# atlas-jj/ORB-SLAM-free-space-carving

Hardware: AMD Instinct MI355X
Metric: Mpix*KF/s fused (640x480xN_KF) (higher is better)
Workload: dtype f32

## Files before the change

include/sdm_c.h:

```cpp
#ifndef SDM_C_H
#define SDM_C_H

#include <stddef.h>
#include <stdint.h>

#ifdef __cplusplus
extern "C" {
#endif

#define SDM_OK 0
#define SDM_EINVAL 1
#define SDM_EHIP 2
#define SDM_ENODEV 3
#define SDM_ESTATE 4
#define SDM_ECOMM 5

#define SDM_MAX_NEIGHBOURS 64
#define SDM_MAX_OBSERVATIONS 8192

typedef struct sdm_ctx sdm_ctx;

typedef struct {
    float lambdaG;
    float lambdaL;
// ... 26 lines not shown
    long long table_stagings;
} sdm_stats;

void sdm_default_params(sdm_params *p);
void sdm_default_config(sdm_config *c);
size_t sdm_depth_pool_bytes(int W, int H, int max_keyframes);
int sdm_create(sdm_ctx **out, const sdm_config *cfg);
void sdm_destroy(sdm_ctx *ctx);
const char *sdm_last_error(void);
int sdm_set_params(sdm_ctx *ctx, const sdm_params *p);
int sdm_get_params(sdm_ctx *ctx, sdm_params *out);
int sdm_set_stream(sdm_ctx *ctx, void *hip_stream);
int sdm_synchronize(sdm_ctx *ctx);
int sdm_device_count(void);

int sdm_upload_keyframe(sdm_ctx *ctx, int slot, const uint8_t *im, const float *grad,
                        const float *theta, float I_stddev, const float K[4], const float Tcw[12]);
int sdm_upload_image(sdm_ctx *ctx, int slot, const uint8_t *im, const float K[4],
                     const float Tcw[12]);
#define SDM_ORDER_RGB 0
#define SDM_ORDER_BGR 1
#define SDM_ORDER_RGBA 2
#define SDM_ORDER_BGRA 3
#define SDM_ORDER_GRAY 4
int sdm_upload_image_rgb(sdm_ctx *ctx, int slot, const uint8_t *pixels, int order, const float K[4],
                         const float dist[5], const float Tcw[12]);
int sdm_upload_images_batch(sdm_ctx *ctx, int n, const int *slots, const uint8_t *const *images,
                            const float *K, const float *Tcw);
int sdm_upload_images_rgb_batch(sdm_ctx *ctx, int n, const int *slots, const uint8_t *const *pixels,
                                int order, const float *K, const float dist[5], const float *Tcw);
void *sdm_host_alloc(size_t bytes);
void sdm_host_free(void *p);
int sdm_upload_image_device(sdm_ctx *ctx, int slot, const void *d_im, const float K[4],
                            const float Tcw[12]);
int sdm_set_pose(sdm_ctx *ctx, int slot, const float Tcw[12]);
int sdm_download_inputs(sdm_ctx *ctx, int slot, uint8_t *im, float *grad, float *theta,
                        float *I_stddev);

int sdm_search_fuse(sdm_ctx *ctx, int n_ref, const int *ref_slots, int n, const int *nbr_slots,
                    const float *rot_deg, const float *min_depth,
                    const float *max_depth);
int sdm_intra_check(sdm_ctx *ctx, int n_ref, const int *ref_slots);
int sdm_intra_grow(sdm_ctx *ctx, int n_ref, const int *ref_slots);
int sdm_recon(sdm_ctx *ctx, int n_ref, const int *ref_slots, int n, const int *nbr_slots,
              const float *rot_deg, const float *min_depth, const float *max_depth);

int sdm_upload_observations(sdm_ctx *ctx, int slot, int n_kp, const int *map_point_ids, const float *angles,
                            int n_depths, const float *depths);
int sdm_upload_observations_batch(sdm_ctx *ctx, int n, const int *slots, const int *n_kp,
                                  const int *const *map_point_ids, const float *const *angles, const int *n_depths,
                                  const float *const *depths);
int sdm_search_priors(sdm_ctx *ctx, int n_ref, const int *ref_slots, int n, const int *nbr_slots, float *rot_deg,
                      float *min_depth, float *max_depth);
int sdm_recon_observed(sdm_ctx *ctx, int n_ref, const int *ref_slots, int n, const int *nbr_slots);

#define SDM_COVIS_MIN_WEIGHT 15

int sdm_covisibility(sdm_ctx *ctx, int n_ref, const int *ref_slots, int n_cand, const int *cand_slots, int *weights);

int sdm_covisible_neighbours(sdm_ctx *ctx, int n_ref, const int *ref_slots, int n_cand, const int *cand_slots,
                             int n, int min_weight, int *nbr_slots, int *nbr_weights, int *counts);

int sdm_recon_covisible(sdm_ctx *ctx, int n_ref, const int *ref_slots, int n_cand, const int *cand_slots,
                        int n, int min_weight, int *nbr_slots_out, unsigned char *done);

int sdm_inter_check(sdm_ctx *ctx, int n_ref, const int *ref_slots, int n, const int *nbr_slots,
                    int commit);


int sdm_pointset(sdm_ctx *ctx, int n_ref, const int *ref_slots, int source);
int sdm_inter_check_pointset(sdm_ctx *ctx, int n_ref, const int *ref_slots, int n, const int *nbr_slots,
                             int commit);

int sdm_upload_depth(sdm_ctx *ctx, int slot, const float *rho, const float *sigma);
int sdm_download_depth(sdm_ctx *ctx, int slot, float *rho, float *sigma);
int sdm_download_checked(sdm_ctx *ctx, int slot, float *rho);
int sdm_download_pointset(sdm_ctx *ctx, int slot, float *xyz);
typedef struct {
    float *xyz;
    unsigned *pixel;
    float *rho_sigma;
    uint8_t *intensity;
    long long capacity;
    int on_device;
} sdm_point_buffers;

int sdm_extract_points(sdm_ctx *ctx, int n, const int *slots, int source, double max_sigma, double min_rho,
                       sdm_point_buffers *out, long long *offsets);
int sdm_extract_points_support(sdm_ctx *ctx, int n, const int *slots, int n_nbr, const int *nbr_slots ,
                               int source, double max_sigma, double min_rho, sdm_point_buffers *out,
                               unsigned long long *support , long long *offsets);
typedef struct {
    unsigned *multiplicity;
    unsigned *source_index;
    unsigned *representative;
    long long rep_capacity;
    long long plain_total;
} sdm_voxel_buffers;
int sdm_extract_points_voxel(sdm_ctx *ctx, int n, const int *slots, int source, double max_sigma, double min_rho,
                             float voxel_size, sdm_point_buffers *out, sdm_voxel_buffers *vox ,
                             long long *offsets);
int sdm_extract_bound(sdm_ctx *ctx, int n, const int *slots, int source, double min_rho, long long *bound);
void *sdm_depth_pool_ptr(sdm_ctx *ctx);
int sdm_assume_pipeline_maps(sdm_ctx *ctx, int n, const int *slots);

int sdm_mark_depth_present(sdm_ctx *ctx, int n, const int *slots);

#define SDM_COMM_ID_BYTES 128
int sdm_comm_unique_id(unsigned char id[SDM_COMM_ID_BYTES]);
int sdm_comm_init(sdm_ctx *ctx, const unsigned char id[SDM_COMM_ID_BYTES], int world, int rank);
int sdm_comm_attach(sdm_ctx *ctx, void *nccl_comm);
int sdm_comm_destroy(sdm_ctx *ctx);
int sdm_comm_info(sdm_ctx *ctx, int *world, int *rank);
int sdm_exchange_halo_begin(sdm_ctx *ctx, int n_send, const int *send_peer, const int *send_slot,
                            int n_recv, const int *recv_peer, const int *recv_slot);
int sdm_exchange_wait(sdm_ctx *ctx);
int sdm_exchange_halo(sdm_ctx *ctx, int n_send, const int *send_peer, const int *send_slot,
                      int n_recv, const int *recv_peer, const int *recv_slot);
int sdm_allgather_depth(sdm_ctx *ctx, int first_slot, int count, int n_fetch, const int *fetch_index,
                        const int *dst_slot);
int sdm_allgather_begin(sdm_ctx *ctx, int maps_per_rank);
int sdm_allgather_piece(sdm_ctx *ctx, int count, const int *slots);
int sdm_allgather_finish(sdm_ctx *ctx, int n_fetch, const int *fetch_index, const int *dst_slot);
int sdm_exchange_compact(sdm_ctx *ctx, int entries_per_map);
int sdm_exchange_mismatches(sdm_ctx *ctx, int *count);
int sdm_compact_pack_host(sdm_ctx *ctx, int slot, float *out);
int sdm_compact_unpack_host(sdm_ctx *ctx, int slot, const float *in, int *refused);
int sdm_compact_sources_ready(sdm_ctx *ctx, int n, const int *slots, int *ready);
int sdm_active_count(sdm_ctx *ctx, int slot, int *count);
int sdm_download_active_list(sdm_ctx *ctx, int slot, unsigned *list, int capacity, int *count,
                             unsigned long long *hash);
int sdm_comm_all_ok(sdm_ctx *ctx, int local_ok, int *all_ok);
int sdm_comm_all_max(sdm_ctx *ctx, int local_value, int *all_max);

int sdm_intra_check_maps(sdm_ctx *ctx, float *rho, float *sigma, const float *grad);
int sdm_intra_grow_maps(sdm_ctx *ctx, float *rho, float *sigma, const float *grad);

int sdm_epipolar_search(sdm_ctx *ctx, int ref_slot, int nbr_slot, int x, int y, float min_depth,
                        float max_depth, float rot_deg, float out[5]);
int sdm_search_range(sdm_ctx *ctx, int ref_slot, int nbr_slot, int x, int y, float mind,
                     float maxd, float *umin, float *umax);
int sdm_fuse(sdm_ctx *ctx, const float *rho, const float *sigma, int n, float out[3]);
int sdm_pair_geometry(sdm_ctx *ctx, int ref_slot, int nbr_slot, float F12[9], float R21[9],
                      float t21[3]);

int sdm_stereo_search_constraints(const float *orb_depths, int n, float *min_depth,
                                  float *max_depth);
float sdm_median_rot_in_plane(const int *mp1, const float *angle1, int n1, const int *mp2,
                              const float *angle2, int n2);

int sdm_enable_stats(sdm_ctx *ctx, int on);
int sdm_get_stats(sdm_ctx *ctx, sdm_stats *out, int reset);
int sdm_set_scan_mode(sdm_ctx *ctx, int mode);
int sdm_set_ingest_overlap(sdm_ctx *ctx, int on);
#define SDM_STAGE_SEARCH_FUSE 0
#define SDM_STAGE_INTRA 1
#define SDM_STAGE_INTER 2
#define SDM_STAGE_POINTSET 3
#define SDM_NUM_STAGES 4
int sdm_enable_timing(sdm_ctx *ctx, int on);
int sdm_get_timing(sdm_ctx *ctx, double ms_total[SDM_NUM_STAGES], long long launches[SDM_NUM_STAGES],
                   int reset);
int sdm_selftest(sdm_ctx *ctx, int which, unsigned long long out[2]);
const char *sdm_device_arch(sdm_ctx *ctx);

#ifdef __cplusplus
}
#endif
#endif
```

orb-slam-free-space-carving_amd/binding.py:

```python
import ctypes as C
import os

import numpy as np

_HERE = os.path.dirname(os.path.abspath(__file__))
MAX_NEIGHBOURS = 64
MAX_OBSERVATIONS = 8192


class SdmError(RuntimeError):
    def __init__(self, code, msg):
        super().__init__("sdm error %d: %s" % (code, msg))
        self.code = code


class Params(C.Structure):
    _fields_ = [("lambdaG", C.c_float), ("lambdaL", C.c_float), ("lambdaTheta", C.c_float),
                ("lambdaN", C.c_int), ("theta_var", C.c_double)]


class Config(C.Structure):
    _fields_ = [("device", C.c_int), ("W", C.c_int), ("H", C.c_int), ("max_keyframes", C.c_int),
                ("max_neighbours", C.c_int), ("batch_capacity", C.c_int), ("with_pointset", C.c_int),
                ("ext_depth_pool", C.c_void_p), ("stream", C.c_void_p)]


class Stats(C.Structure):
    _fields_ = [("searches", C.c_longlong), ("candidates", C.c_longlong), ("gate_pass", C.c_longlong),
                ("hypotheses", C.c_longlong), ("fused", C.c_longlong), ("mask_waves", C.c_longlong),
                ("mask_steps", C.c_longlong), ("mask_row_mismatch", C.c_longlong), ("open_pixels", C.c_longlong),
                ("table_stagings", C.c_longlong)]


class PointBuffers(C.Structure):
    _fields_ = [("xyz", C.c_void_p), ("pixel", C.c_void_p), ("rho_sigma", C.c_void_p), ("intensity", C.c_void_p),
                ("capacity", C.c_longlong), ("on_device", C.c_int)]


class VoxelBuffers(C.Structure):
    _fields_ = [("multiplicity", C.c_void_p), ("source_index", C.c_void_p), ("representative", C.c_void_p),
                ("rep_capacity", C.c_longlong), ("plain_total", C.c_longlong)]


POINT_FIELDS = {"xyz": (np.float32, 3), "pixel": (np.uint32, 1), "rho_sigma": (np.float32, 2), "intensity": (np.uint8, 1)}


def lib_path():
    return os.environ.get("SDM_LIB_PATH") or os.path.join(_HERE, "lib", "libsdm_hip.so")


_lib = None

_f32p, _u8p, _ip = C.POINTER(C.c_float), C.POINTER(C.c_uint8), C.POINTER(C.c_int)
_ctx = C.c_void_p
SYMBOLS = [
    ("sdm_default_params", None, [C.POINTER(Params)]),
    ("sdm_default_config", None, [C.POINTER(Config)]),
    ("sdm_depth_pool_bytes", C.c_size_t, [C.c_int, C.c_int, C.c_int]),
    ("sdm_create", C.c_int, [C.POINTER(_ctx), C.POINTER(Config)]),
    ("sdm_destroy", None, [_ctx]),
    ("sdm_last_error", C.c_char_p, []),
    ("sdm_set_params", C.c_int, [_ctx, C.POINTER(Params)]),
    ("sdm_set_stream", C.c_int, [_ctx, C.c_void_p]),
    ("sdm_synchronize", C.c_int, [_ctx]),
    ("sdm_device_count", C.c_int, []),
    ("sdm_upload_keyframe", C.c_int, [_ctx, C.c_int, _u8p, _f32p, _f32p, C.c_float, _f32p, _f32p]),
    ("sdm_upload_image", C.c_int, [_ctx, C.c_int, _u8p, _f32p, _f32p]),
    ("sdm_upload_image_rgb", C.c_int, [_ctx, C.c_int, _u8p, C.c_int, _f32p, _f32p, _f32p]),
    ("sdm_upload_image_device", C.c_int, [_ctx, C.c_int, C.c_void_p, _f32p, _f32p]),
    ("sdm_upload_images_batch", C.c_int, [_ctx, C.c_int, _ip, C.POINTER(C.c_void_p), _f32p, _f32p]),
    ("sdm_upload_images_rgb_batch", C.c_int, [_ctx, C.c_int, _ip, C.POINTER(C.c_void_p), C.c_int, _f32p, _f32p, _f32p]),
    ("sdm_host_alloc", C.c_void_p, [C.c_size_t]),
    ("sdm_host_free", None, [C.c_void_p]),
    ("sdm_set_pose", C.c_int, [_ctx, C.c_int, _f32p]),
    ("sdm_download_inputs", C.c_int, [_ctx, C.c_int, _u8p, _f32p, _f32p, _f32p]),
    ("sdm_search_fuse", C.c_int, [_ctx, C.c_int, _ip, C.c_int, _ip, _f32p, _f32p, _f32p]),
    ("sdm_intra_check", C.c_int, [_ctx, C.c_int, _ip]),
    ("sdm_intra_grow", C.c_int, [_ctx, C.c_int, _ip]),
    ("sdm_recon", C.c_int, [_ctx, C.c_int, _ip, C.c_int, _ip, _f32p, _f32p, _f32p]),
    ("sdm_upload_observations", C.c_int, [_ctx, C.c_int, C.c_int, _ip, _f32p, C.c_int, _f32p]),
    ("sdm_upload_observations_batch", C.c_int, [_ctx, C.c_int, _ip, _ip, C.POINTER(C.c_void_p), C.POINTER(C.c_void_p), _ip,
                                                C.POINTER(C.c_void_p)]),
    ("sdm_search_priors", C.c_int, [_ctx, C.c_int, _ip, C.c_int, _ip, _f32p, _f32p, _f32p]),
    ("sdm_recon_observed", C.c_int, [_ctx, C.c_int, _ip, C.c_int, _ip]),
    ("sdm_covisibility", C.c_int, [_ctx, C.c_int, _ip, C.c_int, _ip, _ip]),
    ("sdm_covisible_neighbours", C.c_int, [_ctx, C.c_int, _ip, C.c_int, _ip, C.c_int, C.c_int, _ip, _ip, _ip]),
    ("sdm_recon_covisible", C.c_int, [_ctx, C.c_int, _ip, C.c_int, _ip, C.c_int, C.c_int, _ip, _u8p]),
    ("sdm_inter_check", C.c_int, [_ctx, C.c_int, _ip, C.c_int, _ip, C.c_int]),
    ("sdm_pointset", C.c_int, [_ctx, C.c_int, _ip, C.c_int]),
    ("sdm_inter_check_pointset", C.c_int, [_ctx, C.c_int, _ip, C.c_int, _ip, C.c_int]),
    ("sdm_upload_depth", C.c_int, [_ctx, C.c_int, _f32p, _f32p]),
    ("sdm_download_depth", C.c_int, [_ctx, C.c_int, _f32p, _f32p]),
    ("sdm_download_checked", C.c_int, [_ctx, C.c_int, _f32p]),
    ("sdm_download_pointset", C.c_int, [_ctx, C.c_int, _f32p]),
    ("sdm_extract_points", C.c_int, [_ctx, C.c_int, _ip, C.c_int, C.c_double, C.c_double, C.POINTER(PointBuffers),
                                     C.POINTER(C.c_longlong)]),
    ("sdm_extract_points_support", C.c_int, [_ctx, C.c_int, _ip, C.c_int, _ip, C.c_int, C.c_double, C.c_double,
                                             C.POINTER(PointBuffers), C.POINTER(C.c_ulonglong), C.POINTER(C.c_longlong)]),
    ("sdm_extract_points_voxel", C.c_int, [_ctx, C.c_int, _ip, C.c_int, C.c_double, C.c_double, C.c_float,
                                           C.POINTER(PointBuffers), C.POINTER(VoxelBuffers), C.POINTER(C.c_longlong)]),
    ("sdm_extract_bound", C.c_int, [_ctx, C.c_int, _ip, C.c_int, C.c_double, C.POINTER(C.c_longlong)]),
    ("sdm_depth_pool_ptr", C.c_void_p, [_ctx]),
    ("sdm_assume_pipeline_maps", C.c_int, [_ctx, C.c_int, _ip]),
    ("sdm_mark_depth_present", C.c_int, [_ctx, C.c_int, _ip]),
    ("sdm_comm_unique_id", C.c_int, [C.POINTER(C.c_ubyte)]),
    ("sdm_comm_init", C.c_int, [_ctx, C.POINTER(C.c_ubyte), C.c_int, C.c_int]),
    ("sdm_comm_attach", C.c_int, [_ctx, C.c_void_p]),
    ("sdm_comm_destroy", C.c_int, [_ctx]),
    ("sdm_comm_info", C.c_int, [_ctx, _ip, _ip]),
    ("sdm_exchange_halo_begin", C.c_int, [_ctx, C.c_int, _ip, _ip, C.c_int, _ip, _ip]),
    ("sdm_exchange_wait", C.c_int, [_ctx]),
    ("sdm_exchange_halo", C.c_int, [_ctx, C.c_int, _ip, _ip, C.c_int, _ip, _ip]),
    ("sdm_allgather_depth", C.c_int, [_ctx, C.c_int, C.c_int, C.c_int, _ip, _ip]),
    ("sdm_allgather_begin", C.c_int, [_ctx, C.c_int]),
    ("sdm_allgather_piece", C.c_int, [_ctx, C.c_int, _ip]),
    ("sdm_allgather_finish", C.c_int, [_ctx, C.c_int, _ip, _ip]),
    ("sdm_comm_all_ok", C.c_int, [_ctx, C.c_int, _ip]),
    ("sdm_comm_all_max", C.c_int, [_ctx, C.c_int, _ip]),
    ("sdm_exchange_compact", C.c_int, [_ctx, C.c_int]),
    ("sdm_exchange_mismatches", C.c_int, [_ctx, _ip]),
    ("sdm_compact_sources_ready", C.c_int, [_ctx, C.c_int, _ip, _ip]),
    ("sdm_compact_pack_host", C.c_int, [_ctx, C.c_int, _f32p]),
    ("sdm_compact_unpack_host", C.c_int, [_ctx, C.c_int, _f32p, _ip]),
    ("sdm_active_count", C.c_int, [_ctx, C.c_int, _ip]),
    ("sdm_download_active_list", C.c_int, [_ctx, C.c_int, C.POINTER(C.c_uint), C.c_int, _ip, C.POINTER(C.c_ulonglong)]),
    ("sdm_intra_check_maps", C.c_int, [_ctx, _f32p, _f32p, _f32p]),
    ("sdm_intra_grow_maps", C.c_int, [_ctx, _f32p, _f32p, _f32p]),
    ("sdm_epipolar_search", C.c_int, [_ctx, C.c_int, C.c_int, C.c_int, C.c_int, C.c_float, C.c_float,
                                      C.c_float, _f32p]),
    ("sdm_search_range", C.c_int, [_ctx, C.c_int, C.c_int, C.c_int, C.c_int, C.c_float, C.c_float,
                                   _f32p, _f32p]),
    ("sdm_fuse", C.c_int, [_ctx, _f32p, _f32p, C.c_int, _f32p]),
    ("sdm_pair_geometry", C.c_int, [_ctx, C.c_int, C.c_int, _f32p, _f32p, _f32p]),
    ("sdm_stereo_search_constraints", C.c_int, [_f32p, C.c_int, _f32p, _f32p]),
    ("sdm_median_rot_in_plane", C.c_float, [_ip, _f32p, C.c_int, _ip, _f32p, C.c_int]),
    ("sdm_enable_stats", C.c_int, [_ctx, C.c_int]),
    ("sdm_get_stats", C.c_int, [_ctx, C.POINTER(Stats), C.c_int]),
    ("sdm_set_scan_mode", C.c_int, [_ctx, C.c_int]),
    ("sdm_get_params", C.c_int, [_ctx, C.POINTER(Params)]),
    ("sdm_set_ingest_overlap", C.c_int, [_ctx, C.c_int]),
    ("sdm_selftest", C.c_int, [_ctx, C.c_int, C.POINTER(C.c_ulonglong)]),
    ("sdm_enable_timing", C.c_int, [_ctx, C.c_int]),
    ("sdm_get_timing", C.c_int, [_ctx, C.POINTER(C.c_double), C.POINTER(C.c_longlong), C.c_int]),
    ("sdm_device_arch", C.c_char_p, [_ctx]),
]


def load_library():
    global _lib
    if _lib is not None:
        return _lib
    p = lib_path()
    if not os.path.exists(p):
        raise OSError("%s not built: run `python orb-slam-free-space-carving_amd/build.py` "
                      "(there is no CPU fallback)" % p)
    lib = C.CDLL(p)
    for name, res, args in SYMBOLS:
        fn = getattr(lib, name)
        fn.restype = res
        fn.argtypes = args
    _lib = lib
    return lib


def _f32(a):
    a = np.ascontiguousarray(a, dtype=np.float32)
    return a, a.ctypes.data_as(_f32p)


def _i32(a):
    a = np.ascontiguousarray(a, dtype=np.int32)
    return a, a.ctypes.data_as(_ip)


def stereo_search_constraints(depths):
    lib = load_library()
    d, dp = _f32(depths)
    mn, mx = C.c_float(), C.c_float()
    rc = lib.sdm_stereo_search_constraints(dp, len(d), C.byref(mn), C.byref(mx))
    if rc:
        raise SdmError(rc, lib.sdm_last_error().decode())
    return float(mn.value), float(mx.value)


def median_rot_in_plane(mp1, ang1, mp2, ang2):
    lib = load_library()
    m1, m1p = _i32(mp1)
    m2, m2p = _i32(mp2)
    a1, a1p = _f32(ang1)
    a2, a2p = _f32(ang2)
    return float(lib.sdm_median_rot_in_plane(m1p, a1p, len(m1), m2p, a2p, len(m2)))


class Engine:

    def __init__(self, W, H, max_keyframes, max_neighbours=7, device=0, batch_capacity=0,
                 with_pointset=True, ext_depth_pool=None, stream=None):
        self.lib = load_library()
        cfg = Config()
        self.lib.sdm_default_config(C.byref(cfg))
        cfg.device, cfg.W, cfg.H = device, W, H
        cfg.max_keyframes, cfg.max_neighbours = max_keyframes, max_neighbours
        cfg.batch_capacity = batch_capacity
        cfg.with_pointset = 1 if with_pointset else 0
        cfg.ext_depth_pool = ext_depth_pool
        cfg.stream = stream
        self.W, self.H, self.max_keyframes, self.max_neighbours = W, H, max_keyframes, max_neighbours
        self.device = device
        self.ctx = _ctx()
        self._check(self.lib.sdm_create(C.byref(self.ctx), C.byref(cfg)))

    def _check(self, rc):
        if rc:
            raise SdmError(rc, self.lib.sdm_last_error().decode())

    def close(self):
        if getattr(self, "ctx", None):
            self.lib.sdm_destroy(self.ctx)
            self.ctx = None

    def __del__(self):
        try:
            self.close()
        except Exception:
            pass

    def arch(self):
        return self.lib.sdm_device_arch(self.ctx).decode()

    def set_params(self, **kw):
        p = Params()
        self.lib.sdm_default_params(C.byref(p))
        for k, v in kw.items():
            setattr(p, k, v)
        self._check(self.lib.sdm_set_params(self.ctx, C.byref(p)))

    def get_params(self):
        p = Params()
        self._check(self.lib.sdm_get_params(self.ctx, C.byref(p)))
        return {k: getattr(p, k) for k, _ in Params._fields_}

    def set_stream(self, stream_ptr):
        self._check(self.lib.sdm_set_stream(self.ctx, stream_ptr))

    def synchronize(self):
        self._check(self.lib.sdm_synchronize(self.ctx))

    def depth_pool_ptr(self):
        return self.lib.sdm_depth_pool_ptr(self.ctx)

    def upload_keyframe(self, slot, im, grad, theta, I_stddev, K, Tcw):
        im = np.ascontiguousarray(im, dtype=np.uint8)
        assert im.shape == (self.H, self.W)
        g, gp = _f32(grad)
        t, tp = _f32(theta)
        k, kp = _f32(K)
        T, Tp = _f32(np.asarray(Tcw).reshape(12))
        self._check(self.lib.sdm_upload_keyframe(self.ctx, slot, im.ctypes.data_as(_u8p), gp, tp,
                                                 float(I_stddev), kp, Tp))

    def upload_image(self, slot, im, K, Tcw):
        im = np.ascontiguousarray(im, dtype=np.uint8)
        assert im.shape == (self.H, self.W)
        k, kp = _f32(K)
        T, Tp = _f32(np.asarray(Tcw).reshape(12))
        self._check(self.lib.sdm_upload_image(self.ctx, slot, im.ctypes.data_as(_u8p), kp, Tp))

    ORDER = dict(rgb=0, bgr=1, rgba=2, bgra=3, gray=4)
    compact_entries = 0

    def upload_image_rgb(self, slot, pixels, order, K, dist, Tcw):
        px = np.ascontiguousarray(pixels, dtype=np.uint8)
        ch = {0: 3, 1: 3, 2: 4, 3: 4, 4: 1}[self.ORDER[order]]
        assert px.size == self.H * self.W * ch, (px.shape, ch)
        k, kp = _f32(K)
        T, Tp = _f32(np.asarray(Tcw).reshape(12))
        dp = None
        if dist is not None:
            d, dp = _f32(dist)
            assert len(d) == 5
        self._check(self.lib.sdm_upload_image_rgb(self.ctx, slot, px.ctypes.data_as(_u8p), self.ORDER[order], kp, dp, Tp))

    def _upload_args(self, slots, images, K, Tcw, nbytes):
        n = len(slots)
        assert len(images) == n
        ims = [np.ascontiguousarray(im, dtype=np.uint8) for im in images]
        for im in ims:
            assert im.size == nbytes, (im.shape, nbytes)
        ptrs = (C.c_void_p * n)(*[im.ctypes.data for im in ims])
        sl = (C.c_int * n)(*[int(x) for x in slots])
        k = np.ascontiguousarray(np.broadcast_to(np.asarray(K, np.float32).reshape(-1, 4), (n, 4)), dtype=np.float32)
# ... 363 lines not shown
    def comm_init(self, uid, world, rank):
        buf = (C.c_ubyte * self.COMM_ID_BYTES).from_buffer_copy(uid) if uid is not None else None
        self._check(self.lib.sdm_comm_init(self.ctx, buf, world, rank))

    def comm_destroy(self):
        self.compact_entries = 0
        self._check(self.lib.sdm_comm_destroy(self.ctx))

    def comm_info(self):
        w, r = C.c_int(), C.c_int()
        self._check(self.lib.sdm_comm_info(self.ctx, C.byref(w), C.byref(r)))
        return int(w.value), int(r.value)

    def _xchg_args(self, send, recv):
        sp, ss = _i32([p for p, _ in send]), _i32([s for _, s in send])
        rp, rs = _i32([p for p, _ in recv]), _i32([s for _, s in recv])
        return (len(send), sp[1], ss[1], len(recv), rp[1], rs[1]), (sp, ss, rp, rs)

    def exchange_halo_begin(self, send, recv):
        args, keep = self._xchg_args(send, recv)
        self._check(self.lib.sdm_exchange_halo_begin(self.ctx, *args))

    def exchange_wait(self):
        self._check(self.lib.sdm_exchange_wait(self.ctx))

    def exchange_halo(self, send, recv):
        args, keep = self._xchg_args(send, recv)
        self._check(self.lib.sdm_exchange_halo(self.ctx, *args))

    def allgather_depth(self, first_slot, count, fetch=None):
        if fetch is None:
            self._check(self.lib.sdm_allgather_depth(self.ctx, first_slot, count, -1, None, None))
            return
        fi, fip = _i32([i for i, _ in fetch])
        ds, dsp = _i32([s for _, s in fetch])
        self._check(self.lib.sdm_allgather_depth(self.ctx, first_slot, count, len(fetch), fip, dsp))

    def allgather_begin(self, maps_per_rank):
        self._check(self.lib.sdm_allgather_begin(self.ctx, maps_per_rank))

    def allgather_piece(self, slots):
        s, sp = _i32(np.asarray(slots).reshape(-1))
        self._check(self.lib.sdm_allgather_piece(self.ctx, len(s), sp))

    def allgather_finish(self, fetch):
        fi, fip = _i32([i for i, _ in fetch])
        ds, dsp = _i32([s for _, s in fetch])
        self._check(self.lib.sdm_allgather_finish(self.ctx, len(fetch), fip, dsp))

    def comm_all_max(self, value):
        out = C.c_int()
        self._check(self.lib.sdm_comm_all_max(self.ctx, int(value), C.byref(out)))
        return int(out.value)

    def exchange_compact(self, entries_per_map):
        self._check(self.lib.sdm_exchange_compact(self.ctx, int(entries_per_map)))
        self.compact_entries = int(entries_per_map)

    COMPACT_HEADER = 8

    def compact_pack_host(self, slot):
        out = np.empty((self.compact_entries + self.COMPACT_HEADER, 2), np.float32)
        self._check(self.lib.sdm_compact_pack_host(self.ctx, int(slot), out.ctypes.data_as(_f32p)))
        return out

    def compact_unpack_host(self, slot, payload):
        p = np.ascontiguousarray(payload, np.float32)
        assert p.size == 2 * (self.compact_entries + self.COMPACT_HEADER)
        ref = C.c_int()
        self._check(self.lib.sdm_compact_unpack_host(self.ctx, int(slot), p.ctypes.data_as(_f32p), C.byref(ref)))
        return bool(ref.value)

    def exchange_mismatches(self):
        out = C.c_int()
        self._check(self.lib.sdm_exchange_mismatches(self.ctx, C.byref(out)))
        return int(out.value)

    def compact_sources_ready(self, slots):
        arr = (C.c_int * max(len(slots), 1))(*[int(x) for x in slots])
        out = C.c_int()
        self._check(self.lib.sdm_compact_sources_ready(self.ctx, len(slots), arr, C.byref(out)))
        return bool(out.value)

    def active_count(self, slot):
        out = C.c_int()
        self._check(self.lib.sdm_active_count(self.ctx, int(slot), C.byref(out)))
        return int(out.value)

    def active_list(self, slot):
        n = self.active_count(slot)
        lst = np.empty(max(n, 1), np.uint32)
        cnt, h = C.c_int(), C.c_ulonglong()
        self._check(self.lib.sdm_download_active_list(self.ctx, int(slot), lst.ctypes.data_as(C.POINTER(C.c_uint)), int(lst.size),
                                                      C.byref(cnt), C.byref(h)))
        return lst[:cnt.value].copy(), int(h.value)

    def comm_all_ok(self, local_ok=True):
        out = C.c_int()
        self._check(self.lib.sdm_comm_all_ok(self.ctx, 1 if local_ok else 0, C.byref(out)))
        return bool(out.value)

    def assume_pipeline_maps(self, slots):
        r, rp = _i32(np.asarray(slots).reshape(-1))
        self._check(self.lib.sdm_assume_pipeline_maps(self.ctx, len(r), rp))

    def intra_check_maps(self, rho, sigma, grad=None):
        r = np.array(rho, dtype=np.float32, order="C")
        s = np.array(sigma, dtype=np.float32, order="C")
        gp = None
        if grad is not None:
            g, gp = _f32(grad)
        self._check(self.lib.sdm_intra_check_maps(self.ctx, r.ctypes.data_as(_f32p), s.ctypes.data_as(_f32p), gp))
        return r, s

    def intra_grow_maps(self, rho, sigma, grad):
        r = np.array(rho, dtype=np.float32, order="C")
        s = np.array(sigma, dtype=np.float32, order="C")
        g, gp = _f32(grad)
        self._check(self.lib.sdm_intra_grow_maps(self.ctx, r.ctypes.data_as(_f32p), s.ctypes.data_as(_f32p), gp))
        return r, s

    def epipolar_search(self, ref, nbr, x, y, min_depth, max_depth, rot=0.0):
        out = (C.c_float * 5)()
        self._check(self.lib.sdm_epipolar_search(self.ctx, ref, nbr, x, y, min_depth, max_depth, rot, out))
        return dict(rho=float(out[0]), sigma=float(out[1]), supported=int(out[2]), best_u=float(out[3]),
                    best_v=float(out[4]))

    def search_range(self, ref, nbr, x, y, mind, maxd):
        a, b = C.c_float(), C.c_float()
        self._check(self.lib.sdm_search_range(self.ctx, ref, nbr, x, y, mind, maxd, C.byref(a), C.byref(b)))
        return float(a.value), float(b.value)

    def fuse(self, rho, sigma):
        r, rp = _f32(rho)
        s, sp = _f32(sigma)
        out = (C.c_float * 3)()
        self._check(self.lib.sdm_fuse(self.ctx, rp, sp, len(r), out))
        return float(out[0]), float(out[1]), int(out[2])

    def pair_geometry(self, ref, nbr):
        F = np.empty(9, np.float32)
        R = np.empty(9, np.float32)
        t = np.empty(3, np.float32)
        self._check(self.lib.sdm_pair_geometry(self.ctx, ref, nbr, F.ctypes.data_as(_f32p),
                                               R.ctypes.data_as(_f32p), t.ctypes.data_as(_f32p)))
        return F, R, t

    def set_ingest_overlap(self, on=True):
        self._check(self.lib.sdm_set_ingest_overlap(self.ctx, 1 if on else 0))

    def set_scan_mode(self, mode):
        self._check(self.lib.sdm_set_scan_mode(self.ctx, int(mode)))

    def enable_stats(self, on=True):
        self._check(self.lib.sdm_enable_stats(self.ctx, 1 if on else 0))

    def selftest(self, which):
        out = (C.c_ulonglong * 2)()
        self._check(self.lib.sdm_selftest(self.ctx, which, out))
        return int(out[0]), int(out[1])

    STAGES = ("search_fuse", "intra", "inter", "pointset")

    def enable_timing(self, on=True):
        self._check(self.lib.sdm_enable_timing(self.ctx, 1 if on else 0))

    def get_timing(self, reset=True):
        ms = (C.c_double * 4)()
        cnt = (C.c_longlong * 4)()
        self._check(self.lib.sdm_get_timing(self.ctx, ms, cnt, 1 if reset else 0))
        return {s: (float(ms[i]), int(cnt[i])) for i, s in enumerate(self.STAGES)}

    def get_stats(self, reset=True):
        s = Stats()
        self._check(self.lib.sdm_get_stats(self.ctx, C.byref(s), 1 if reset else 0))
        return {k: int(getattr(s, k)) for k, _ in Stats._fields_}
```

orb-slam-free-space-carving_amd/csrc/sdm_device.h:

```cpp
#pragma once
#include <hip/hip_runtime.h>
#include <float.h>
#include <stddef.h>
#include <stdint.h>

#include "sdm_c.h"

namespace sdm {

struct KfMeta {
    float fx, fy, cx, cy;
    float Tcw[12];
    float I_stddev;
    int uploaded;
    int pad[2];
};

struct RefConst {
    int slot;
    float fx, fy, cx, cy;
    float mind, maxd;
    int act_count;
};

// ... 277 lines not shown
__device__ __forceinline__ float fast_atan2_deg_x1(float y)
{
    const float scale = (float)(180.0 / 3.14159265358979323846);
    const float p1 = 0.9997878412794807f * scale;
    const float p3 = -0.3258083974640975f * scale;
    const float p5 = 0.1555786518463281f * scale;
    const float p7 = -0.04432655554792128f * scale;
    float ay = fabsf(y);
    float a, c, c2;
    if (1.0f >= ay) {
        c = ay;
        c2 = c * c;
        a = (((p7 * c2 + p5) * c2 + p3) * c2 + p1) * c;
    } else {
#if SDM_K1_OPT_ATAN_RCP
        c = rcp_exact(ay + (float)DBL_EPSILON);
#else
        c = 1.0f / (ay + (float)DBL_EPSILON);
#endif
        c2 = c * c;
        a = 90.f - (((p7 * c2 + p5) * c2 + p3) * c2 + p1) * c;
    }
    if (y < 0) a = 360.f - a;
    return a;
}

#ifndef SDM_K1_OPT
#define SDM_K1_OPT 0x3a27f
#endif

constexpr int PCV_FLOATS = 20;
constexpr int CV_RX = 9, CV_RZ = 12, CV_TX = 15, CV_TZ = 16, CV_ROT = 17, CV_ISTD = 18;
static_assert(offsetof(PairConst, Rx) == 4 * CV_RX && offsetof(PairConst, Rz) == 4 * CV_RZ && offsetof(PairConst, tx) == 4 * CV_TX &&
                  offsetof(PairConst, tz) == 4 * CV_TZ && offsetof(PairConst, rot) == 4 * CV_ROT &&
                  offsetof(PairConst, istd) == 4 * CV_ISTD && offsetof(PairConst, Ry) == 4 * PCV_FLOATS,
              "the CV_* indices follow PairConst");

__device__ __forceinline__ float match_cost1(float pe2, float ge2, const DevParams& prm)
{
    double s = (double)pe2 + (double)ge2 * prm.inv_theta;
    const unsigned lo = (unsigned)__double2loint(s), hi = (unsigned)__double2hiint(s);
    const bool risky = (((lo & 0x1FFFFFFFu) - 0x0FFFFF00u) <= 0x200u) | ((hi - 0x39C00000u) >= (0x46200000u - 0x39C00000u));
    if (__builtin_expect(risky, 0)) s = (double)pe2 + (double)ge2 / prm.theta_var;
    return (float)s;
}

constexpr float INV_THETA_DEFAULT_F = (float)(1.0 / 0.23);
constexpr unsigned COST_BAND = 16u;
__device__ __forceinline__ float match_cost_ref(float pe2, float ge2, const DevParams& prm)
{
    return (float)((double)pe2 + (double)ge2 / prm.theta_var);
}
__device__ __forceinline__ float match_cost_approx(float pe2, float ge2) { return __builtin_fmaf(ge2, INV_THETA_DEFAULT_F, pe2); }

__device__ __forceinline__ float lerp_w0(float yf)
{
#if SDM_K1_OPT & 0x10
    return 1.0f - __builtin_amdgcn_fractf(yf);
#else
    return (floorf(yf) + 1.0f) - yf;
#endif
}
__device__ __forceinline__ float rec_lerp_im_w(const float4& r, float y0w)
{
    unsigned w = __float_as_uint(r.w);
    float y1w = 1.0f - y0w;
    float v0 = (float)(int)(w & 0xffu), v1 = (float)(int)((w >> 8) & 0xffu);
    return v0 * y0w + v1 * y1w;
}
__device__ __forceinline__ float rec_lerp_grad_w(const float4& r, float y0w)
{
    float y1w = 1.0f - y0w;
    return r.x * y0w + r.z * y1w;
}

__device__ __forceinline__ int cvt_i32_sat(float x)
{
    int r;
    asm("v_cvt_i32_f32 %0, %1" : "=v"(r) : "v"(x));
    return r;
}
__device__ __forceinline__ bool search_range_int1(float fx, float cx, float rxxp, float rzxp, float tx, float tz,
                                                  float mind, float maxd, int W, int& lo, int& hi)
{
    float x_min = rxxp * mind + tx, z_min = rzxp * mind + tz;
    float x_max = rxxp * maxd + tx, z_max = rzxp * maxd + tz;
    const float u1 = fx * x_min / z_min + cx;
    const float u2 = fx * x_max / z_max + cx;
    const float mn = __builtin_amdgcn_fmed3f(u1, u2, -__builtin_inff());
    const float mx = __builtin_amdgcn_fmed3f(u1, u2, __builtin_inff());
    lo = min(max(cvt_i32_sat(ceilf(mn)), 0), W);
    hi = min(max(cvt_i32_sat(floorf(mx)), 0), W - 1);
    return !__builtin_isunordered(u1, u2);
}

__device__ __forceinline__ float wrap_once_360_ref(float a)
{
    if (a >= 360) a -= 360;
    if (a < 0) a += 360;
    return a;
}
__device__ __forceinline__ float wrap_once_360(float a)
{
#if SDM_K1_OPT & 0x40
    a = a + 0.0f;
    const unsigned bits = __float_as_uint(a);
    const unsigned lt360 = (unsigned)((int)(bits - 0x43B40000u) >> 31);
    const unsigned neg = (unsigned)((int)bits >> 31);
    unsigned keep = lt360 | neg;
    asm("" : "+v"(keep));
    a = a + __uint_as_float(~keep & 0xC3B40000u);
    return wrap_neg360(a);
#else
    return wrap_once_360_ref(a);
#endif
}

constexpr unsigned QUOT_MAG_LO = 87u << 23;
constexpr unsigned QUOT_MAG_HI = (168u << 23) - 1u;
__device__ __forceinline__ unsigned absbits(float x) { return __float_as_uint(x) & 0x7FFFFFFFu; }
__device__ __forceinline__ float rcp_fast(float b)
{
    const float r = __builtin_amdgcn_rcpf(b);
    const float e = __builtin_fmaf(-b, r, 1.0f);
    return __builtin_fmaf(e, r, r);
}
__device__ __forceinline__ float quot_fast(float a, float b, float r)
{
    float q0 = a * r;
    float e0 = __builtin_fmaf(-q0, b, a);
    float q1 = __builtin_fmaf(e0, r, q0);
    float e1 = __builtin_fmaf(-q1, b, a);
    return __builtin_fmaf(e1, r, q1);
}
__device__ __forceinline__ bool quot_window_ok(float a, float b)
{
    const unsigned ua = absbits(a), ub = absbits(b);
    return (ua >= QUOT_MAG_LO) & (ua <= QUOT_MAG_HI) & (ub >= QUOT_MAG_LO) & (ub <= QUOT_MAG_HI);
}

__device__ __forceinline__ float sqrt_exact(float x)
{
#if SDM_K1_OPT & 0x10000
    if (__builtin_expect((__float_as_uint(x) - (27u << 23)) >= ((254u - 27u) << 23), 0)) return sqrtf(x);
    const float r = __builtin_amdgcn_rsqf(x);
    const float y0 = x * r, h = 0.5f * r;
    const float e = __builtin_fmaf(-y0, y0, x);
    return __builtin_fmaf(e, h, y0);
#else
    return sqrtf(x);
#endif
}

__device__ __forceinline__ bool line_quot_safe(const float* F)
{
    bool ok = true;
    for (int i = 0; i < 9; i++) {
        const unsigned u = __float_as_uint(F[i]), mag = u & 0x7FFFFFFFu;
        ok = ok && (u == 0u || (mag >= ((127u - 36u) << 23) && mag <= ((127u + 20u) << 23)));
    }
    return ok;
}

struct ScanState {
    float old_err, best_pe, best_ge;
    int best_pixel;
};

struct ScanConst {
    const char* nbase;
    unsigned W16;
    float hlim_b;
    float ab, cb, pixel, grad1, th_line, ang_pi_rot, gate_lim;
    int hi;
};
template <bool STATS, bool CLEAN>
__device__ __forceinline__ void scan_candidate(const ScanConst& q, int uj, float yf, const float4& r, const DevParams& prm,
                                               ScanState& S, SearchStats* st)
{
    if (r.x < prm.lambdaG) return;
#if SDM_ABLATE == 4
    if (r.z > S.old_err) { S.best_pixel = uj; S.old_err = r.z; }
    return;
#endif
    const float d2 = r.y - q.th_line;
    const float d3 = r.y - q.ang_pi_rot;
    bool fail;
    if (CLEAN) {
#if SDM_K1_OPT & 0x04
        fail = gate2_fails_fast1(d2) | gate3_fails_fast1(d3);
#else
        fail = gate2_fails_fast(d2) | gate3_fails_fast(d3);
#endif
    } else {
        fail = gate2_fails_k(d2, prm.g2c) | gate3_fails_k(d3, prm.g3lo, prm.g3span);
        if (__builtin_expect(!((d2 < q.gate_lim) & (d3 < q.gate_lim)), 0))
            fail = gate2_fails_ref(d2, prm.lambdaL) || gate3_fails_ref(d3, prm.lambdaTheta);
    }
    if (fail) return;
    if (STATS) st->gate_pass++;
#if SDM_ABLATE == 3 || SDM_ABLATE == 4
    if (r.z > S.old_err) { S.best_pixel = uj; S.old_err = r.z; }
    return;
#endif
    const float y0w = lerp_w0(yf);
    float pe = q.pixel - rec_lerp_im_w(r, y0w);
    float ge = q.grad1 - rec_lerp_grad_w(r, y0w);
#if SDM_K1_OPT & 0x2000
    if (CLEAN || prm.approx_ok) {
        const float e = CLEAN ? match_cost_approx(pe * pe, ge * ge) : __builtin_fmaf(ge * ge, prm.inv_theta_f, pe * pe);
        bool better = e < S.old_err;
        if (__builtin_expect((__float_as_uint(e) - __float_as_uint(S.old_err) + COST_BAND) <= 2u * COST_BAND, 0))
            better = match_cost_ref(pe * pe, ge * ge, prm) < match_cost_ref(S.best_pe * S.best_pe, S.best_ge * S.best_ge, prm);
        if (better) {
#if SDM_K1_OPT & 0x4000
            asm volatile("" ::: "memory");
#endif
            S.best_pixel = uj;
            S.old_err = e;
            S.best_pe = pe;
            S.best_ge = ge;
        }
        return;
    }
#endif
#if SDM_K1_OPT & 0x08
    float err = match_cost1(pe * pe, ge * ge, prm);
#else
    float err = match_cost(pe * pe, ge * ge, prm);
#endif
    if (err < S.old_err) {
        S.best_pixel = uj;
        S.old_err = err;
        S.best_pe = pe;
        S.best_ge = ge;
    }
}

template <bool STATS, bool CLEAN, int NB>
__device__ __forceinline__ void scan_batch(const ScanConst& q, int u0, float u0f, const DevParams& prm, ScanState& S,
                                           SearchStats* st)
{
    float yfs[NB];
    unsigned long long rowok[NB];
    v4f rs[NB];
    const unsigned c0 = (unsigned)u0 << 4;
#if !(SDM_K1_OPT & 0x01)
    const unsigned hi16 = (unsigned)max(q.hi, 0) << 4;
#endif
#pragma unroll
    for (int k = 0; k < NB; k++) {
        float yf = -(q.ab * (u0f + (float)k) + q.cb);
        float yc = __builtin_amdgcn_fmed3f(yf, 1.0f, q.hlim_b);
#if SDM_K1_OPT & 0x01
        const unsigned off = __umul24((unsigned)(int)yc, q.W16) + c0;
        const char* __restrict__ nb_k = q.nbase + 16 * k;
#else
        unsigned uc16 = min(c0 + 16u * k, hi16);
        unsigned off = __umul24((unsigned)(int)yc, q.W16) + uc16;
        const char* __restrict__ nb_k = q.nbase;
#endif
        yfs[k] = yf;
        rowok[k] = __builtin_amdgcn_fcmpf(yc, yf, 1 );
#if SDM_ABLATE == 5
        rs[k] = v4f{20.0f + (float)(off & 15u), 10.0f, 21.0f, __uint_as_float(0x6040u)};
#else
        rs[k] = *reinterpret_cast<const v4f*>(nb_k + off);
#endif
    }
#pragma unroll
    for (int k = 0; k < NB; k++)
        asm volatile("" : "+v"(rs[k]));
#pragma unroll
    for (int k = 0; k < NB; k++) {
        const int uj = u0 + k;
        if (STATS && uj <= q.hi) st->candidates++;
        const float4 r = make_float4(rs[k].x, rs[k].y, rs[k].z, rs[k].w);
        if (!((uj <= q.hi) & __builtin_amdgcn_inverse_ballot_w64(rowok[k]))) continue;
        scan_candidate<STATS, CLEAN>(q, uj, yfs[k], r, prm, S, st);
    }
}

template <bool STATS, bool CLEAN>
__device__ __forceinline__ void scan_segment(const ScanConst& q, int lo, const DevParams& prm, ScanState& S, SearchStats* st)
{
    float u0f = (float)lo;
    for (int u0 = lo; u0 <= q.hi; u0 += SCAN_UNROLL, u0f += (float)SCAN_UNROLL)
        scan_batch<STATS, CLEAN, SCAN_UNROLL>(q, u0, u0f, prm, S, st);
}

#ifndef SDM_MASK_MIN_L
#define SDM_MASK_MIN_L 24
#endif
#ifndef SDM_MASK_MIN_L_UNION
#define SDM_MASK_MIN_L_UNION 48
#endif
#ifndef SDM_MASK_MAX_SLOPE
#define SDM_MASK_MAX_SLOPE 0.25f
#endif
#ifndef SDM_MASK_NB
#define SDM_MASK_NB 2
#endif
#ifndef SDM_MASK_BINS
#define SDM_MASK_BINS 1
#endif
constexpr int MASK_BINS = 16;
constexpr int MASK_WINDOW = 6;
constexpr int MASK_UNION = MASK_BINS + MASK_WINDOW - 1;
constexpr int MASK_PLANES = MASK_UNION + 1;
constexpr unsigned MASK_WORD_BYTES = 4u * MASK_PLANES;
constexpr float MASK_EPS = 0x1p-6f;
constexpr int MASK_HINT_L = SDM_MASK_MIN_L * 3 / 4;
#ifndef SDM_MASK_CALL_MEAN_L
#define SDM_MASK_CALL_MEAN_L 32
#endif
constexpr int MASK_CALL_MEAN_L = SDM_MASK_CALL_MEAN_L;
constexpr float MASK_ANG_MARGIN = 0.01f;
constexpr float MASK_MAX_LAMBDA_THETA = 56.0f;
constexpr float MASK_BIN_SCALE = (float)MASK_BINS / 360.0f;
__host__ __device__ __forceinline__ int mask_bin(float t)
{
    const int b = (int)(t * MASK_BIN_SCALE);
    return b < MASK_BINS - 1 ? b : MASK_BINS - 1;
}
struct MaskStats {
    unsigned long long waves, steps, row_mismatch;
};
struct MaskView {
    const char* base;
    unsigned row_pitch;
};
template <bool STATS, bool CLEAN, bool BINNED>
__device__ __forceinline__ void scan_masked(const ScanConst& q, const MaskView& mv, int lo, const DevParams& prm, ScanState& S,
                                            SearchStats* st, MaskStats* ms)
{
    const float yh = -(q.ab * (float)q.hi + q.cb);
    const float inv_s = __builtin_amdgcn_rcpf(fabsf(q.ab)) * 0.998046875f;
    const bool falling = q.ab > 0.0f;
    unsigned pl0 = 4u * (unsigned)MASK_UNION;
    if (BINNED) {
        float w0 = q.ang_pi_rot - (prm.lambdaTheta + MASK_ANG_MARGIN);
        if (w0 < 0.0f) w0 += 360.0f;
        pl0 = 4u * (unsigned)mask_bin(w0);
    }
    for (int base = lo; base <= q.hi; base += 64) {
        const int chi = min(q.hi, base + 63);
        unsigned long long cand = 0ull;
        bool ended = false;
        int u = base;
        while (u <= chi) {
            const float yf = -(q.ab * (float)u + q.cb);
            const float yc = __builtin_amdgcn_fmed3f(yf, 1.0f, q.hlim_b);
            if (!(yc == yf)) {
                const bool out_lo = (yf < 1.0f) & (yh < 1.0f), out_hi = (yf > q.hlim_b) & (yh > q.hlim_b);
                if (!(yf == yf) | out_lo | out_hi) {
                    if (STATS) st->candidates += (unsigned long long)(q.hi - u + 1);
                    ended = true;
                    break;
                }
                if (STATS) st->candidates++;
                u++;
                continue;
            }
            const float fr = __builtin_amdgcn_fractf(yf);
            const float room = (falling ? fr : 1.0f - fr) - MASK_EPS;
            const int n = max(cvt_i32_sat(room * inv_s), 0);
            const int cover = min(min(n, chi - u), 32);
            const char* __restrict__ mp = mv.base + (__umul24((unsigned)(int)yc, mv.row_pitch) + __umul24((unsigned)u >> 5, MASK_WORD_BYTES) + pl0);
            unsigned mlo, mhi;
            if (BINNED) {
                typedef unsigned mword4 __attribute__((ext_vector_type(4), aligned(4)));
                typedef unsigned mword2 __attribute__((ext_vector_type(2), aligned(4)));
                const mword4 a0 = *reinterpret_cast<const mword4*>(mp);
                const mword2 a1 = *reinterpret_cast<const mword2*>(mp + 16);
                const mword4 b0 = *reinterpret_cast<const mword4*>(mp + MASK_WORD_BYTES);
                const mword2 b1 = *reinterpret_cast<const mword2*>(mp + MASK_WORD_BYTES + 16);
                mlo = (a0.x | a0.y | a0.z) | (a0.w | a1.x | a1.y);
                mhi = (b0.x | b0.y | b0.z) | (b0.w | b1.x | b1.y);
            } else {
                mlo = *reinterpret_cast<const unsigned*>(mp);
                mhi = *reinterpret_cast<const unsigned*>(mp + MASK_WORD_BYTES);
            }
            unsigned long long bits = (((unsigned long long)mhi << 32) | (unsigned long long)mlo) >> ((unsigned)u & 31u);
            bits &= (2ull << cover) - 1ull;
            cand |= bits << (unsigned)(u - base);
            if (STATS) {
                st->candidates += (unsigned long long)(cover + 1);
                ms->steps++;
            }
            u += cover + 1;
        }
        if (STATS) {
            for (int k = 0; base + k <= (ended ? u - 1 : chi); k++) {
                const float yk = -(q.ab * (float)(base + k) + q.cb);
                if (!(__builtin_amdgcn_fmed3f(yk, 1.0f, q.hlim_b) == yk)) continue;
                const v4f r = *reinterpret_cast<const v4f*>(q.nbase + (__umul24((unsigned)(int)yk, q.W16) + ((unsigned)(base + k) << 4)));
                if (r.x < prm.lambdaG) continue;
                const bool fail = gate2_fails_ref(r.y - q.th_line, prm.lambdaL) || gate3_fails_ref(r.y - q.ang_pi_rot, prm.lambdaTheta);
                if (!fail && !((cand >> k) & 1ull)) ms->row_mismatch++;
            }
        }
        while (cand != 0ull) {
            int ujs[SDM_MASK_NB];
            float yfs[SDM_MASK_NB];
            v4f rs[SDM_MASK_NB];
            unsigned long long okm[SDM_MASK_NB];
#pragma unroll
            for (int k = 0; k < SDM_MASK_NB; k++) {
                okm[k] = __builtin_amdgcn_ballot_w64(cand != 0ull);
                const int uj = base + (cand != 0ull ? (int)__builtin_ctzll(cand) : 0);
                cand &= cand - 1ull;
                const float yfj = -(q.ab * (float)uj + q.cb);
                const float ycj = __builtin_amdgcn_fmed3f(yfj, 1.0f, q.hlim_b);
                ujs[k] = uj;
                yfs[k] = yfj;
                rs[k] = *reinterpret_cast<const v4f*>(q.nbase + (__umul24((unsigned)(int)ycj, q.W16) + ((unsigned)uj << 4)));
            }
#pragma unroll
            for (int k = 0; k < SDM_MASK_NB; k++)
                asm volatile("" : "+v"(rs[k]));
#pragma unroll
            for (int k = 0; k < SDM_MASK_NB; k++) {
                if (!__builtin_amdgcn_inverse_ballot_w64(okm[k])) continue;
                scan_candidate<STATS, CLEAN>(q, ujs[k], yfs[k], make_float4(rs[k].x, rs[k].y, rs[k].z, rs[k].w), prm, S, st);
            }
        }
        if (ended) break;
    }
}

__device__ __forceinline__ int wave_max_nonneg(int v)
{
    v = max(v, __builtin_amdgcn_update_dpp(0, v, 0x111, 0xf, 0xf, false));
    v = max(v, __builtin_amdgcn_update_dpp(0, v, 0x112, 0xf, 0xf, false));
    v = max(v, __builtin_amdgcn_update_dpp(0, v, 0x114, 0xf, 0xf, false));
    v = max(v, __builtin_amdgcn_update_dpp(0, v, 0x118, 0xf, 0xf, false));
    v = max(v, __builtin_amdgcn_update_dpp(0, v, 0x142, 0xa, 0xf, false));
    v = max(v, __builtin_amdgcn_update_dpp(0, v, 0x143, 0xc, 0xf, false));
    return __builtin_amdgcn_readlane(v, 63);
}
template <bool STATS, bool CLEAN>
__device__ __forceinline__ void scan_planned(const ScanConst& q, int lo, int Lmax, const DevParams& prm, ScanState& S,
                                             SearchStats* st)
{
    int n3 = (-Lmax) & 3;
    if (Lmax <= 3) n3 = 1;
    if (Lmax == 5) n3 = 2;
    const int n4 = max(Lmax - 3 * n3, 0) >> 2;
    int u0 = lo;
    float u0f = (float)lo;
    for (int i = 0; i < n4; i++, u0 += 4, u0f += 4.0f)
        if (u0 <= q.hi) scan_batch<STATS, CLEAN, 4>(q, u0, u0f, prm, S, st);
    for (int i = 0; i < n3; i++, u0 += 3, u0f += 3.0f)
        if (u0 <= q.hi) scan_batch<STATS, CLEAN, 3>(q, u0, u0f, prm, S, st);
}

template <bool STATS, bool PLAN = false, bool MASK = false>
__device__ __forceinline__ bool epipolar_search(const float4* __restrict__ nrec, int W, int H,
                                                const float* __restrict__ cv, const float* __restrict__ rcv, int clean,
                                                bool on, int x, int y, float pixel, float grad1,
                                                float th_pi, float xp0, float xp1, const DevParams& prm, float& rho_o,
                                                float& sigma_o, float& best_u, float& best_v,
                                                SearchStats* st, const MaskView mv = MaskView{nullptr, 0u}, MaskStats* ms = nullptr)
{
    float fx = rcv[0], cx = rcv[1];
    const float mind = rcv[2], maxd = rcv[3];
    rho_o = 0.f;
    sigma_o = 0.f;
    best_u = 0.f;
    best_v = 0.f;
    if (STATS && on) st->searches++;
    const float* F = cv;
    float a = (float)x * F[0] + (float)y * F[3] + F[6];
    float b = (float)x * F[1] + (float)y * F[4] + F[7];
    float c = (float)x * F[2] + (float)y * F[5] + F[8];
#if SDM_K1_OPT & 0x8000
    float ab, cb;
    if (clean & 2) {
        const float rb = rcp_fast(b);
        ab = quot_fast(a, b, rb);
        cb = quot_fast(c, b, rb);
    } else {
        ab = a / b;
        cb = c / b;
    }
    bool live = on & (ab >= -4) & (ab <= 4);
    if (!PLAN && !live) return false;
#else
    float ab = a / b;
    bool live = on & (ab >= -4) & (ab <= 4);
    if (!PLAN && !live) return false;
    float cb = c / b;
#endif

    float rxxp = row_dot_xp(cv + CV_RX, xp0, xp1);
    float rzxp = row_dot_xp(cv + CV_RZ, xp0, xp1);
    float tx = cv[CV_TX], tz = cv[CV_TZ];
    int lo, hi;
#if SDM_K1_OPT & 0x20
    live &= search_range_int1(fx, cx, rxxp, rzxp, tx, tz, mind, maxd, W, lo, hi);
#else
    live &= search_range_int(fx, cx, rxxp, rzxp, tx, tz, mind, maxd, W, lo, hi);
    if (hi > W - 1) hi = W - 1;
#endif
    if (!PLAN && !live) return false;

    float th_line = fast_atan2_deg_x1(-ab);
    float ang_pi_rot = wrap_once_360(th_pi + cv[CV_ROT]);

    const float gate_lim = prm.closed_ok ? 360.0f : -__builtin_inff();
    ScanState S = {1000000.0f, 1000.0f, 0.f, -1};
    const float hlim2 = (float)(H - 2);
    const char* __restrict__ nbase = reinterpret_cast<const char*>(nrec);
#if SDM_ABLATE == 10
    if (ang_pi_rot + th_line + (float)(hi - lo) != 12345.678f) live = false;
#endif
#if SDM_ABLATE == 11
    if (ab + cb + rxxp + rzxp != 12345.678f) live = false;
#endif
#if SDM_ABLATE == 6
    hi = lo - 1;
    S.old_err = ab;
    S.best_pixel = lo + 2;
#endif
    if (PLAN && !live) hi = lo - 1;
    ScanConst sc;
    sc.nbase = nbase;
    sc.W16 = (unsigned)W << 4;
    sc.hlim_b = __uint_as_float(__float_as_uint((float)(H - 1)) - 1u);
    sc.ab = ab;
    sc.cb = cb;
    sc.pixel = pixel;
    sc.grad1 = grad1;
    sc.th_line = th_line;
    sc.ang_pi_rot = ang_pi_rot;
    sc.gate_lim = gate_lim;
    sc.hi = hi;
    if (PLAN) {
        const int Lmax = wave_max_nonneg(max(hi - lo + 1, 0));
        if (Lmax > 0) {
#if SDM_K1_OPT & 0x02
            if ((clean & 1) && prm.default_gates && prm.fast_theta_div)
                scan_planned<STATS, true>(sc, lo, Lmax, prm, S, st);
            else
#endif
                scan_planned<STATS, false>(sc, lo, Lmax, prm, S, st);
        }
        if (!live) return false;
    } else {
        bool masked = false;
        const unsigned long long here = __builtin_amdgcn_ballot_w64(true);
#ifndef SDM_MASK_DISABLE
        if (MASK && mv.base != nullptr && prm.scan_mode != 1 && ((clean & 4) || prm.scan_mode == 2)) {
            const bool binned = (clean & 1) && prm.bins_ok && SDM_MASK_BINS;
            const int min_l = binned ? SDM_MASK_MIN_L : SDM_MASK_MIN_L_UNION;
            const unsigned long long lng = __builtin_amdgcn_ballot_w64(hi - lo + 1 >= min_l);
            const unsigned long long steep = __builtin_amdgcn_ballot_w64(fabsf(ab) > SDM_MASK_MAX_SLOPE);
            masked = prm.scan_mode == 2 || (2 * __popcll(lng) >= __popcll(here) && steep == 0ull);
        }
#endif
        if (MASK && masked) {
            if (STATS && (int)__builtin_amdgcn_mbcnt_hi(~0u, __builtin_amdgcn_mbcnt_lo(~0u, 0u)) == (int)__builtin_ctzll(here)) ms->waves++;
#if SDM_K1_OPT & 0x02
            if ((clean & 1) && prm.default_gates && prm.fast_theta_div)
                scan_masked<STATS, true, SDM_MASK_BINS != 0>(sc, mv, lo, prm, S, st, ms);
            else
#endif
                if ((clean & 1) && prm.bins_ok && SDM_MASK_BINS)
                scan_masked<STATS, false, true>(sc, mv, lo, prm, S, st, ms);
            else
                scan_masked<STATS, false, false>(sc, mv, lo, prm, S, st, ms);
        } else {
#if SDM_K1_OPT & 0x02
            if ((clean & 1) && prm.default_gates && prm.fast_theta_div)
                scan_segment<STATS, true>(sc, lo, prm, S, st);
            else
#endif
                scan_segment<STATS, false>(sc, lo, prm, S, st);
        }
    }
    const float best_pe = S.best_pe, best_ge = S.best_ge;
    const int best_pixel = S.best_pixel;
    if (best_pixel < 0) return false;
#if SDM_ABLATE == 2
    rho_o = S.old_err + best_pe + (float)best_pixel;
    sigma_o = best_ge + 1.0f;
    return true;
#endif


    int up = best_pixel + 1, um = best_pixel - 1;
    if (um < 0 || up > W - 1) return false;
    float yfp = -(ab * (float)up + cb);
    float yfm = -(ab * (float)um + cb);
    float fyp = floorf(yfp), fym = floorf(yfm);
    if (!(fyp >= 0.0f && fyp <= hlim2)) return false;
    if (!(fym >= 0.0f && fym <= hlim2)) return false;
    int y0p = (int)fyp, y0m = (int)fym;
#if SDM_K1_OPT & 0x20000
    v4f vp = *reinterpret_cast<const v4f*>(nbase + ((__umul24((unsigned)y0p, (unsigned)W) + (unsigned)up) << 4));
    v4f vm = *reinterpret_cast<const v4f*>(nbase + ((__umul24((unsigned)y0m, (unsigned)W) + (unsigned)um) << 4));
    asm volatile("" : "+v"(vp));
    asm volatile("" : "+v"(vm));
    const float4 rp = make_float4(vp.x, vp.y, vp.z, vp.w), rm = make_float4(vm.x, vm.y, vm.z, vm.w);
#else
    float4 rp = *reinterpret_cast<const float4*>(nbase + ((__umul24((unsigned)y0p, (unsigned)W) + (unsigned)up) << 4));
    float4 rm = *reinterpret_cast<const float4*>(nbase + ((__umul24((unsigned)y0m, (unsigned)W) + (unsigned)um) << 4));
#endif
    const float y1p = fyp + 1.0f, y1m = fym + 1.0f;
    float g = (rec_lerp_im(rp, y1p, yfp) - rec_lerp_im(rm, y1m, yfm)) / 2;
    float q = (rec_lerp_grad(rp, y1p, yfp) - rec_lerp_grad(rm, y1m, yfm)) / 2;
    const double inv_theta = prm.inv_theta;
    float gg = g * g;
    float denom = (float)((double)gg + inv_theta * (double)q * (double)q);
    float gpe = g * best_pe;
    float ustar = (float)((double)best_pixel +
                          ((double)gpe + inv_theta * (double)q * (double)best_ge) / (double)denom);
    float ustar_var = 2 * cv[CV_ISTD] * cv[CV_ISTD] / denom;
    best_u = ustar;
    best_v = -(ab * ustar + cb);

    float d0 = pixel_depth(ustar, fx, cx, rzxp, rxxp, tx, tz);
    float s = sqrt_exact(ustar_var);
    float dmin = pixel_depth(ustar - s, fx, cx, rzxp, rxxp, tx, tz);
    float dmax = pixel_depth(ustar + s, fx, cx, rzxp, rxxp, tx, tz);
    float e1 = fabsf(dmax - d0), e2 = fabsf(dmin - d0);
    rho_o = d0;
    sigma_o = (e1 < e2) ? e2 : e1;
    return true;
}

__device__ __forceinline__ bool chi_test(float a, float b, float sa, float sb)
{
    float d = a - b;
    float num = d * d;
    float chi = num / (sa * sa) + num / (sb * sb);
    return (double)chi < 5.99;
}

__device__ __forceinline__ double div_by_with_rcp(double a, double b, double r)
{
    double q0 = a * r;
    double e0 = __builtin_fma(-q0, b, a);
    double q1 = __builtin_fma(e0, r, q0);
    double e1 = __builtin_fma(-q1, b, a);
    return __builtin_fma(e1, r, q1);
}
__device__ __forceinline__ void fusion_terms(float rho, float sg, double& t_rho, double& t_one)
{
    double s2 = (double)sg * (double)sg;
    const float ar = fabsf(rho);
#if SDM_K1_OPT & 512
    const unsigned hi = (unsigned)__double2hiint(s2);
    const bool safe = ((hi - 0x39B00000u) < (0x46400000u - 0x39B00000u)) & (ar > 1.0e-30f) & (ar < 1.0e30f);
    if (safe) {
        double y = (double)__builtin_amdgcn_rcpf(sg * sg);
        double e = __builtin_fma(-s2, y, 1.0);
        y = __builtin_fma(e, y, y);
        e = __builtin_fma(-s2, y, 1.0);
        y = __builtin_fma(e, y, y);
        e = __builtin_fma(-s2, y, 1.0);
        t_one = __builtin_fma(e, y, y);
        t_rho = div_by_with_rcp((double)rho, s2, t_one);
    } else {
        t_one = 1.0 / s2;
        t_rho = (double)rho / s2;
    }
#else
    t_one = 1.0 / s2;
    const bool safe = (s2 > 1.0e-60) & (s2 < 1.0e60) & (ar > 1.0e-30f) & (ar < 1.0e30f);
    t_rho = safe ? div_by_with_rcp((double)rho, s2, t_one) : (double)rho / s2;
#endif
}
__device__ __forceinline__ void fusion_accum(float rho, float sg, float& pjsj, float& rsj)
{
    double t_rho, t_one;
    fusion_terms(rho, sg, t_rho, t_one);
    pjsj = (float)((double)pjsj + t_rho);
    rsj = (float)((double)rsj + t_one);
}

__device__ __forceinline__ bool gt_1em6(float x) { return x > __uint_as_float(0x358637bdu); }
__device__ __forceinline__ bool lt_1em6(float x) { return x <= __uint_as_float(0x358637bdu); }

__device__ __forceinline__ float safe_rcp_sq(float s)
{
    float s2 = s * s;
    bool ok = (s2 >= 1.0e-30f) && (s2 <= 1.0e30f);
    return ok ? __builtin_amdgcn_rcpf(s2) : __builtin_nanf("");
}

// ... 53 lines not shown
```

orb-slam-free-space-carving_amd/csrc/sdm_engine.hip:

```cpp
#include <hip/hip_runtime.h>

#include <algorithm>
#include <atomic>
#include <chrono>
#include <cmath>
#include <condition_variable>
#include <cstdio>
#include <cstdlib>
#include <cstring>
#include <limits>
#include <map>
#include <mutex>
#include <string>
#include <thread>
#include <vector>

#include "sdm_c.h"
#include "sdm_kernels.h"
#include "sdm_extract.h"
#include "sdm_support.h"
#include "sdm_priors.h"
#include "sdm_covis.h"
#include "sdm_voxel.h"

using namespace sdm;

namespace {

thread_local std::string g_err;

int fail(int code, const std::string& msg)
{
    g_err = msg;
    return code;
}

#define HIP_TRY(expr)                                                                         \
    do {                                                                                      \
        hipError_t e__ = (expr);                                                              \
        if (e__ != hipSuccess)                                                                \
            return fail(SDM_EHIP, std::string(#expr) + ": " + hipGetErrorString(e__));        \
    } while (0)

}

struct sdm_ctx {
    sdm_config cfg{};
    int W = 0, H = 0;
    long long P = 0;
    TileGeom geom{};
    hipStream_t stream = nullptr;
    bool own_stream = false;
    std::string arch;

    float4* rec = nullptr;
    float2* pool = nullptr;
    bool own_pool = false;
    float2* scratch = nullptr;
    float* chk = nullptr;
    float* xyz = nullptr;

    KfMeta* d_meta = nullptr;
    std::vector<KfMeta> h_meta;
    std::vector<char> has_depth, has_chk;
    unsigned* d_act = nullptr;
    int* d_act_count = nullptr;
    int* d_theta_bad = nullptr;
    unsigned* d_open_ctr = nullptr;
    long long* d_open_pix = nullptr;
    unsigned long long* d_open_vm = nullptr;
    float2* d_open_hyp = nullptr;
    unsigned open_capacity = 0;
    unsigned open_quota = 512;
    unsigned open_inplace_min = 40;
    unsigned open_grid = 2048;
    unsigned open_launch = 0;
    unsigned* d_grow_ctr = nullptr;
    long long* d_grow_pix = nullptr;
    float2* d_grow_val = nullptr;
    unsigned grow_capacity = 0;
    unsigned grow_launch = 0;
    unsigned k4_lds_pad = 0;
    int* h_act_count = nullptr;
    std::vector<float> act_lambdaG;
    std::vector<char> chk_sparse, xyz_sparse;
    std::vector<float> recon_lambdaG;

    uint8_t* d_im = nullptr;
    int ing_cap = 0;
    struct IngestBuf {
        uint8_t* d_img = nullptr;
        uint8_t* h_ring = nullptr;
        uint8_t* d_src = nullptr;
        uint8_t* h_src = nullptr;
        IngestItem* h_items = nullptr;
        IngestItem* d_items = nullptr;
        hipEvent_t copied = nullptr;
        hipEvent_t consumed = nullptr;
        bool copied_pending = false, consumed_pending = false;
        int consumed_from = -1;
    } ing[12];
    static constexpr int ING_BUFS_MAX = 12;
    int ing_bufs = 4;
    int ing_next = 0;
    size_t src_bytes = 0;
    hipStream_t up_stream = nullptr;
    static constexpr int ING_GROUP = 4;
    static_assert(ING_GROUP == CHUNK_TABLES, "one merged launch covers a group");
    unsigned long long* d_part = nullptr;
    unsigned long long* d_seg_mask = nullptr;
    int* d_seg_off = nullptr;
    IngestItem* d_gitems = nullptr;
    int nseg = 0;
    unsigned long long* d_act_hash = nullptr;
    unsigned* d_gmask = nullptr;
    int mrow = 0;
    int scan_mode = 0;
    bool ingest_overlap = false;
    static constexpr int CNT_RING = 16;
    hipEvent_t cnt_ev[CNT_RING] = {};
    unsigned long long cnt_next = 1, cnt_done = 0;
    std::vector<unsigned long long> slot_cnt;
    bool validated = false;
    sdm_params validated_prm{};
    int validated_closed = 0, validated_approx = 0;
    float* d_grad = nullptr;
    float* d_theta = nullptr;
    float* d_small = nullptr;

    int cap_refs = 0;
    size_t tab_bytes = 0;
    struct TableKey {
        bool valid = false, has_consts = false;
        bool long_ranges = false;
        int n_ref = 0, n = 0;
        unsigned long long epoch = 0;
        std::vector<int> refs, nbrs;
        std::vector<float> rot, mind, maxd;
    };
    static constexpr int TABLE_SETS = 8;
    struct TableSet {
        unsigned char *d_tab = nullptr, *h_tab = nullptr;
        RefConst* d_refs = nullptr;
        PairConst* d_pairs = nullptr;
        TableKey key;
        hipEvent_t free_ev = nullptr;
        bool pending = false;
        unsigned long long last_use = 0;
    } sets[TABLE_SETS];
    int cur_set = 0;
    unsigned long long use_tick = 0;
    unsigned char *d_tab = nullptr, *h_tab = nullptr;
    int *d_ref_slots = nullptr, *d_nbr_slots = nullptr;
    float *d_rot = nullptr, *d_mind = nullptr, *d_maxd = nullptr;
    long long *d_off = nullptr, *h_off = nullptr;
    unsigned long long epoch = 1;
    long long table_stagings = 0;
    RefConst* d_refs = nullptr;
    PairConst* d_pairs = nullptr;

    float2* h_f2 = nullptr;

    sdm_params prm{};
    DevParams dprm{};
    bool stats_on = false;
    unsigned long long* d_stats = nullptr;

    struct Span {
        hipEvent_t a, b;
        int stage;
    };
    bool timing_on = false;
    std::vector<Span> spans;
    size_t spans_used = 0;

    void* comm = nullptr;
    bool own_comm = false;
    int world = 1, rank = 0;
    hipStream_t comm_stream = nullptr;
    hipEvent_t ev_maps_ready = nullptr, ev_xchg_done = nullptr;
    bool xchg_pending = false;
    float2* gather_buf = nullptr;
    long long gather_slots = 0;
    struct AgPiece {
        int offset, count;
    };
    bool ag_open = false;
    int ag_count = 0, ag_covered = 0;
    std::vector<AgPiece> ag_pieces;
    std::vector<char> ag_contributed;
    float2* stage_buf = nullptr;
    int stage_slots = 0;
    int* d_agree = nullptr;
    int xchg_entries = 0;
    unsigned* d_xchg_mismatch = nullptr;

    unsigned char* d_ext = nullptr;
    size_t ext_bytes = 0;
    unsigned char* h_ext = nullptr;
    size_t ext_host_bytes = 0;
    unsigned char* d_ext_stage = nullptr;
    size_t ext_stage_bytes = 0;
    unsigned char* d_vox = nullptr;
    size_t vox_bytes = 0;
    unsigned char* d_vox_out = nullptr;
    size_t vox_out_bytes = 0;

    ObsStore obs{};
    std::vector<char> has_obs;
    std::vector<int> obs_kp, obs_nd;
    unsigned char *d_obs_stage = nullptr, *h_obs_stage = nullptr;
    size_t obs_dev_bytes = 0, obs_host_bytes = 0;
    unsigned char *d_pri = nullptr, *h_pri = nullptr;
    size_t pri_dev_bytes = 0, pri_host_bytes = 0;
    unsigned char *d_cov = nullptr, *h_cov = nullptr;
    size_t cov_dev_bytes = 0, cov_host_bytes = 0;
};

namespace {

void set_dev_params(sdm_ctx* c)
{
    c->dprm.lambdaG = c->prm.lambdaG;
    c->dprm.lambdaL = c->prm.lambdaL;
    c->dprm.lambdaTheta = c->prm.lambdaTheta;
    c->dprm.lambdaN = c->prm.lambdaN;
    c->dprm.theta_var = c->prm.theta_var;
    c->dprm.inv_theta = 1 / c->prm.theta_var;
    c->dprm.fast_theta_div = (c->prm.theta_var == 0.23) ? 1 : 0;
    c->dprm.default_gates = (c->prm.lambdaL == 80.0f && c->prm.lambdaTheta == 45.0f) ? 1 : 0;
    c->dprm.scan_mode = c->scan_mode;
    auto round_up = [](double v) {
        float f = (float)v;
        if ((double)f < v) f = std::nextafterf(f, std::numeric_limits<float>::infinity());
        return f;
    };
    const float lL = c->prm.lambdaL, lT = c->prm.lambdaTheta;
    c->dprm.g2c = (lL == lL) ? round_up(90.0 - (double)lL) : 0.0f;
    if (lT >= 0.0f && lT < 180.0f) {
        unsigned lo, hi;
        const float t_up = round_up(360.0 - (double)lT);
        memcpy(&lo, &lT, 4);
        memcpy(&hi, &t_up, 4);
        c->dprm.g3lo = lo + 1u;
        c->dprm.g3span = hi - (lo + 1u);
    } else if (lT < 0.0f) {
        c->dprm.g3lo = 0u;
        c->dprm.g3span = 0x7F800001u;
    } else {
        c->dprm.g3lo = 0u;
        c->dprm.g3span = 0u;
    }
    c->dprm.inv_theta_f = (float)(1.0 / c->prm.theta_var);
    c->dprm.bins_ok = (lT >= 0.0f && lT <= MASK_MAX_LAMBDA_THETA) ? 1 : 0;
    const bool defaults = c->dprm.default_gates && c->dprm.fast_theta_div;
    c->dprm.closed_ok = c->dprm.default_gates;
    c->dprm.approx_ok = defaults ? 1 : 0;
}

int validate_params(sdm_ctx* c)
{
    if (c->dprm.default_gates && c->dprm.fast_theta_div) return SDM_OK;
    if (c->validated && memcmp(&c->validated_prm, &c->prm, sizeof(sdm_params)) == 0) {
        c->dprm.closed_ok = c->validated_closed;
        c->dprm.approx_ok = c->validated_approx;
        return SDM_OK;
    }
    HIP_TRY(hipSetDevice(c->cfg.device));
    unsigned long long out[4] = {0, 0, 0, 0};
    HIP_TRY(hipMemsetAsync(c->d_stats, 0, sizeof(unsigned long long) * STATS_WORDS, c->stream));
    hipLaunchKernelGGL(k_selftest_gates, dim3(4096), dim3(BLOCK), 0, c->stream, c->dprm, c->d_stats + 4, c->d_stats + 5);
    hipLaunchKernelGGL(k_selftest_cost, dim3(256), dim3(BLOCK), 0, c->stream, c->dprm, 256, c->d_stats + 6, c->d_stats + 7);
    HIP_TRY(hipGetLastError());
    HIP_TRY(hipMemcpyAsync(out, c->d_stats + 4, sizeof(out), hipMemcpyDeviceToHost, c->stream));
    HIP_TRY(hipMemsetAsync(c->d_stats, 0, sizeof(unsigned long long) * STATS_WORDS, c->stream));
    HIP_TRY(hipStreamSynchronize(c->stream));
    const double th = c->prm.theta_var;
    c->validated_closed = (out[0] == 0 && out[1] > 0) ? 1 : 0;
    c->validated_approx = (out[2] == 0 && th >= 1.0e-6 && th <= 1.0e6) ? 1 : 0;
    c->validated_prm = c->prm;
    c->validated = true;
    c->dprm.closed_ok = c->validated_closed;
    c->dprm.approx_ok = c->validated_approx;
    return SDM_OK;
}

int blocks_for(long long n) { return (int)((n + BLOCK - 1) / BLOCK); }

int ingest_acquire(sdm_ctx* c, int b, hipStream_t copy_stream)
{
    sdm_ctx::IngestBuf& B = c->ing[b];
    if (B.copied_pending) {
        HIP_TRY(hipEventSynchronize(B.copied));
        B.copied_pending = false;
    }
    if (B.consumed_pending) {
        HIP_TRY(hipStreamWaitEvent(copy_stream, B.consumed_from >= 0 ? c->ing[B.consumed_from].consumed : B.consumed, 0));
        B.consumed_pending = false;
    }
    return SDM_OK;
}
int ingest_publish(sdm_ctx* c, int b, int m, hipStream_t copy_stream, bool compute_waits = true)
{
    const hipStream_t ks = c->stream;
    sdm_ctx::IngestBuf& B = c->ing[b];
    HIP_TRY(hipMemcpyAsync(B.d_items, B.h_items, sizeof(IngestItem) * (size_t)m, hipMemcpyHostToDevice, copy_stream));
    HIP_TRY(hipEventRecord(B.copied, copy_stream));
    B.copied_pending = true;
    if (copy_stream != ks && compute_waits) HIP_TRY(hipStreamWaitEvent(ks, B.copied, 0));
    return SDM_OK;
}
int counts_queued(sdm_ctx* c, int n, const int* slots)
{
    const unsigned long long g = c->cnt_next++;
    HIP_TRY(hipEventRecord(c->cnt_ev[g % sdm_ctx::CNT_RING], c->stream));
    for (int i = 0; i < n; i++) c->slot_cnt[(size_t)slots[i]] = g;
    return SDM_OK;
}
int ingest_launch_chunk(sdm_ctx* c, int b, int m, int kf0, bool from_images, const IngestParams* q)
{
    const hipStream_t ks = c->stream;
    sdm_ctx::IngestBuf& B = c->ing[b];
    const int tiles_x = c->geom.tiles_x, ntiles = c->geom.ntiles;
    if (kf0 < 0 || kf0 + m > sdm_ctx::ING_GROUP * c->ing_cap) return fail(SDM_EINVAL, "ingest group overflow (internal)");
    if (q) hipLaunchKernelGGL(k_ingest_batch, dim3(blocks_for(c->P), m), dim3(BLOCK), 0, ks, B.d_items, c->W, c->H, *q);
    if (from_images) {
        ChunkTables tabs;
        for (int i = 0; i < CHUNK_TABLES; i++) tabs.p[i] = B.d_items;
        tabs.per = std::max(m, 1);
        hipLaunchKernelGGL(k_prepass_batch<true>, dim3(ntiles, m), dim3(BLOCK), 0, ks, tabs, c->W, c->H, tiles_x, c->P, c->rec,
                           c->pool, c->chk, c->xyz, c->dprm.lambdaG, c->d_part, c->d_seg_mask, c->nseg, c->d_gmask, c->mrow, kf0,
                           c->d_gitems);
    } else {
        hipLaunchKernelGGL(k_gate_batch, dim3(ntiles, m), dim3(BLOCK), 0, ks, B.d_items, c->W, c->H, tiles_x, c->P, c->rec,
                           c->dprm.lambdaG, c->d_part, c->d_seg_mask, c->nseg, c->d_gmask, c->mrow, kf0, c->d_gitems);
    }
    HIP_TRY(hipGetLastError());
    HIP_TRY(hipEventRecord(B.consumed, ks));
    B.consumed_pending = true;
    B.consumed_from = -1;
    return SDM_OK;
}
int ingest_launch_chunks_merged(sdm_ctx* c, int n_chunks, const int* bufs, int per, int total)
{
    const hipStream_t ks = c->stream;
    if (n_chunks < 1 || n_chunks > CHUNK_TABLES || total > sdm_ctx::ING_GROUP * c->ing_cap || per < 1 ||
        total <= (n_chunks - 1) * per || total > n_chunks * per)
        return fail(SDM_EINVAL, "merged ingest launch: bad chunk shape (internal)");
    ChunkTables tabs;
    for (int i = 0; i < CHUNK_TABLES; i++) tabs.p[i] = c->ing[bufs[std::min(i, n_chunks - 1)]].d_items;
    tabs.per = per;
    HIP_TRY(hipStreamWaitEvent(ks, c->ing[bufs[n_chunks - 1]].copied, 0));
    hipLaunchKernelGGL(k_prepass_batch<true>, dim3(c->geom.ntiles, total), dim3(BLOCK), 0, ks, tabs, c->W, c->H, c->geom.tiles_x,
                       c->P, c->rec, c->pool, c->chk, c->xyz, c->dprm.lambdaG, c->d_part, c->d_seg_mask, c->nseg, c->d_gmask,
                       c->mrow, 0, c->d_gitems);
    HIP_TRY(hipGetLastError());
    HIP_TRY(hipEventRecord(c->ing[bufs[n_chunks - 1]].consumed, ks));
    for (int i = 0; i < n_chunks; i++) {
        c->ing[bufs[i]].consumed_pending = true;
        c->ing[bufs[i]].consumed_from = i == n_chunks - 1 ? -1 : bufs[n_chunks - 1];
    }
    return SDM_OK;
}
int ingest_launch_group(sdm_ctx* c, int n_kf, bool from_images)
{
    if (n_kf <= 0) return SDM_OK;
    const hipStream_t ks = c->stream;
    hipLaunchKernelGGL(k_prepass_finish, dim3(n_kf), dim3(FIN_BLOCK), 0, ks, c->d_gitems, c->W, c->H, c->geom.ntiles, c->nseg,
                       c->d_part, c->d_seg_mask, c->d_seg_off, c->d_meta, c->d_act_count, c->h_act_count, c->d_theta_bad,
                       c->d_act_hash, from_images ? 1 : 0);
    const int waves = (c->nseg + LIST_SEGS - 1) / LIST_SEGS;
    hipLaunchKernelGGL(k_list_write, dim3((waves + BLOCK / 64 - 1) / (BLOCK / 64), n_kf), dim3(BLOCK), 0, ks, c->d_gitems,
                       c->geom.tiles_x, c->nseg, c->P, c->d_seg_mask, c->d_seg_off, c->d_act);
    HIP_TRY(hipGetLastError());
    return SDM_OK;
}

int rebuild_lists(sdm_ctx* c, int n, const int* slots)
{
    int rc;
    int group_kfs = 0, group_chunks = 0;
    for (int i0 = 0; i0 < n; i0 += c->ing_cap) {
        const int m = std::min(c->ing_cap, n - i0);
        const int b = c->ing_next;
        c->ing_next = (c->ing_next + 1) % c->ing_bufs;
        if ((rc = ingest_acquire(c, b, c->stream))) return rc;
        for (int i = 0; i < m; i++) {
            IngestItem& it = c->ing[b].h_items[i];
            memset(&it, 0, sizeof(it));
            it.slot = slots[i0 + i];
        }
        if ((rc = ingest_publish(c, b, m, c->stream))) return rc;
        if ((rc = ingest_launch_chunk(c, b, m, group_kfs, false, nullptr))) return rc;
        group_kfs += m;
        if (++group_chunks == sdm_ctx::ING_GROUP || i0 + m >= n) {
            if ((rc = ingest_launch_group(c, group_kfs, false))) return rc;
            group_kfs = group_chunks = 0;
        }
    }
    if ((rc = counts_queued(c, n, slots))) return rc;
    for (int i = 0; i < n; i++) {
        const int slot = slots[i];
        if (c->act_lambdaG[slot] == c->act_lambdaG[slot]) {
            c->chk_sparse[slot] = 0;
            c->xyz_sparse[slot] = 0;
        }
        c->act_lambdaG[slot] = c->dprm.lambdaG;
    }
    c->epoch++;
    return SDM_OK;
}
int build_active(sdm_ctx* c, int slot) { return rebuild_lists(c, 1, &slot); }

int sync_counts(sdm_ctx* c)
{
    if (c->cnt_done + 1 < c->cnt_next) {
        HIP_TRY(hipEventSynchronize(c->cnt_ev[(c->cnt_next - 1) % sdm_ctx::CNT_RING]));
        c->cnt_done = c->cnt_next - 1;
    }
    return SDM_OK;
}
int sync_counts_for(sdm_ctx* c, int n_a, const int* a, size_t n_b, const int* b)
{
    unsigned long long g = 0;
    for (int i = 0; i < n_a; i++) g = std::max(g, c->slot_cnt[(size_t)a[i]]);
    for (size_t i = 0; i < n_b; i++) g = std::max(g, c->slot_cnt[(size_t)b[i]]);
    if (g > c->cnt_done) {
        if (c->cnt_next - g >= (unsigned long long)sdm_ctx::CNT_RING) g = c->cnt_next - 1;
        HIP_TRY(hipEventSynchronize(c->cnt_ev[g % sdm_ctx::CNT_RING]));
        c->cnt_done = g;
    }
    return SDM_OK;
}

int check_slot(sdm_ctx* c, int slot, bool need_upload)
{
    if (!c) return fail(SDM_EINVAL, "null context");
    if (slot < 0 || slot >= c->cfg.max_keyframes) return fail(SDM_EINVAL, "slot out of range");
    if (need_upload && !c->h_meta[slot].uploaded) return fail(SDM_ESTATE, "slot has no keyframe uploaded");
    return SDM_OK;
}

int wait_tables(sdm_ctx* c)
{
    sdm_ctx::TableSet& s = c->sets[c->cur_set];
    if (s.pending) {
        HIP_TRY(hipEventSynchronize(s.free_ev));
        s.pending = false;
    }
    return SDM_OK;
}

size_t select_set(sdm_ctx* c, int si, int n_ref, size_t np)
{
    sdm_ctx::TableSet& s = c->sets[si];
    c->cur_set = si;
    c->d_tab = s.d_tab;
    c->h_tab = s.h_tab;
    c->d_refs = s.d_refs;
    c->d_pairs = s.d_pairs;
    size_t words = (size_t)n_ref * 3 + np * 2;
    words = (words + 1) & ~(size_t)1;
    c->h_off = reinterpret_cast<long long*>(c->h_tab + words * 4);
    c->d_ref_slots = reinterpret_cast<int*>(c->d_tab);
    c->d_nbr_slots = c->d_ref_slots + n_ref;
    c->d_rot = reinterpret_cast<float*>(c->d_nbr_slots + np);
    c->d_mind = c->d_rot + np;
    c->d_maxd = c->d_mind + n_ref;
    c->d_off = reinterpret_cast<long long*>(c->d_tab + words * 4);
    return words;
}

template <typename F>
void for_ref_slices(int n_ref, long long blocks_per_ref, int threads, F&& fn)
{
    static const int lg = [] {
        int v = 31;
        if (const char* e = getenv("SDM_MAX_DISPATCH_LOG2")) {
#ifdef SDM_DEBUG_KNOBS
            v = std::max(20, std::min(40, atoi(e)));
#else
            v = std::max(20, std::min(31, atoi(e)));
#endif
        }
        return v;
    }();
    const long long max_blocks = (1ll << lg) / threads;
    const int per = (int)std::max<long long>(1, std::min<long long>(n_ref, max_blocks / std::max<long long>(blocks_per_ref, 1)));
    for (int first = 0; first < n_ref; first += per) fn(first, std::min(per, n_ref - first));
}

struct StageTimer {
    sdm_ctx* c;
    sdm_ctx::Span* sp = nullptr;
    StageTimer(sdm_ctx* ctx, int stage) : c(ctx)
    {
        if (!c->timing_on) return;
        if (c->spans_used == c->spans.size()) {
            if (c->spans.size() >= 65536) return;
            sdm_ctx::Span n{};
            if (hipEventCreate(&n.a) != hipSuccess || hipEventCreate(&n.b) != hipSuccess) return;
            c->spans.push_back(n);
        }
        sp = &c->spans[c->spans_used++];
        sp->stage = stage;
        (void)hipEventRecord(sp->a, c->stream);
    }
    ~StageTimer()
    {
        if (sp) (void)hipEventRecord(sp->b, c->stream);
    }
};

int stage_tables(sdm_ctx* c, int n_ref, const int* ref_slots, int n, const int* nbr_slots, const float* rot,
                 const float* mind, const float* maxd, bool need_consts = false, bool rebuild_stale = true)
{
    if (n_ref <= 0 || !ref_slots) return fail(SDM_EINVAL, "n_ref <= 0 or null ref_slots");
    if (n_ref > c->cap_refs) return fail(SDM_EINVAL, "n_ref exceeds max_keyframes");
    if (n < 0 || n > c->cfg.max_neighbours) return fail(SDM_EINVAL, "n exceeds max_neighbours");
    if (n > 0 && !nbr_slots) return fail(SDM_EINVAL, "null nbr_slots");
    for (int r = 0; r < n_ref; r++) {
        int rc = check_slot(c, ref_slots[r], true);
        if (rc) return rc;
        for (int j = 0; j < n; j++) {
            rc = check_slot(c, nbr_slots[r * n + j], true);
            if (rc) return rc;
        }
    }
    HIP_TRY(hipSetDevice(c->cfg.device));
    int rc;
    if (rebuild_stale) {
        std::vector<int> stale;
        std::vector<char> seen((size_t)c->cfg.max_keyframes, 0);
        auto look = [&](int slot) {
            if (!(c->act_lambdaG[slot] == c->dprm.lambdaG) && !seen[slot]) {
                seen[slot] = 1;
                stale.push_back(slot);
            }
        };
        for (int r = 0; r < n_ref; r++) look(ref_slots[r]);
        if (need_consts)
            for (size_t i = 0; i < (size_t)n_ref * (size_t)n; i++) look(nbr_slots[i]);
        if (!stale.empty() && (rc = rebuild_lists(c, (int)stale.size(), stale.data()))) return rc;
    }
    static const bool dbg_st = getenv("SDM_DEBUG_STAGE_TIMING") != nullptr;
    auto now_ms = [] { return std::chrono::duration<double, std::milli>(std::chrono::steady_clock::now().time_since_epoch()).count(); };
    const double t_s0 = dbg_st ? now_ms() : 0.0;
    if ((rc = sync_counts_for(c, n_ref, ref_slots, (size_t)n_ref * (size_t)n, nbr_slots))) return rc;
    if (dbg_st && now_ms() - t_s0 > 0.2)
        fprintf(stderr, "[sdm stage] waited %.3f ms for list lengths (slot %d: read-back %llu, done %llu, next %llu)\n",
                now_ms() - t_s0, ref_slots[0], c->slot_cnt[(size_t)ref_slots[0]], c->cnt_done, c->cnt_next);

    const size_t np = (size_t)n_ref * (size_t)n;
    auto matches = [&](const sdm_ctx::TableKey& k) {
        bool hit = k.valid && k.epoch == c->epoch && k.n_ref == n_ref &&
                   memcmp(k.refs.data(), ref_slots, sizeof(int) * n_ref) == 0;
        if (hit && n > 0) hit = (k.n == n) && memcmp(k.nbrs.data(), nbr_slots, sizeof(int) * np) == 0;
        if (hit && need_consts) {
            hit = k.has_consts && memcmp(k.mind.data(), mind, sizeof(float) * n_ref) == 0 &&
                  memcmp(k.maxd.data(), maxd, sizeof(float) * n_ref) == 0;
            if (hit) {
                if (rot)
                    hit = memcmp(k.rot.data(), rot, sizeof(float) * np) == 0;
                else
                    for (size_t i = 0; i < np && hit; i++) hit = (k.rot[i] == 0.0f);
            }
        }
        return hit;
    };
    for (int si = 0; si < sdm_ctx::TABLE_SETS; si++) {
        if (!matches(c->sets[si].key)) continue;
        select_set(c, si, n_ref, (size_t)n_ref * (size_t)c->sets[si].key.n);
        c->sets[si].last_use = ++c->use_tick;
        return SDM_OK;
    }
    int victim = 0;
    for (int si = 0; si < sdm_ctx::TABLE_SETS; si++) {
        if (!c->sets[si].key.valid) {
            victim = si;
            break;
        }
        if (c->sets[si].last_use < c->sets[victim].last_use) victim = si;
    }
    const size_t words = select_set(c, victim, n_ref, np);
    c->table_stagings++;
    const double t_w0 = dbg_st ? now_ms() : 0.0;
    if ((rc = wait_tables(c))) return rc;
    if (dbg_st && now_ms() - t_w0 > 0.2) fprintf(stderr, "[sdm stage] waited %.3f ms for table set %d\n", now_ms() - t_w0, victim);
    sdm_ctx::TableKey& k = c->sets[victim].key;
    k.valid = false;
    const size_t bytes = words * 4 + sizeof(long long) * 3 * (size_t)n_ref;
    if (bytes > c->tab_bytes) return fail(SDM_EINVAL, "table staging overflow");
    int* h_refs = reinterpret_cast<int*>(c->h_tab);
    int* h_nbrs = h_refs + n_ref;
    float* h_rot = reinterpret_cast<float*>(h_nbrs + np);
    float* h_mind = h_rot + np;
    float* h_maxd = h_mind + n_ref;
    memcpy(h_refs, ref_slots, sizeof(int) * n_ref);
    if (np) memcpy(h_nbrs, nbr_slots, sizeof(int) * np);
    for (size_t i = 0; i < np; i++) h_rot[i] = rot ? rot[i] : 0.0f;
    const int cap = c->cfg.batch_capacity;
    for (int r = 0; r < n_ref; r++) {
        h_mind[r] = mind ? mind[r] : 0.f;
        h_maxd[r] = maxd ? maxd[r] : 0.f;
        c->h_off[r] = (long long)ref_slots[r] * c->P;
        c->h_off[n_ref + r] = (long long)(r % cap) * c->P;
        c->h_off[2 * n_ref + r] = (long long)ref_slots[r] * c->P * 4;
    }
    HIP_TRY(hipMemcpyAsync(c->d_tab, c->h_tab, bytes, hipMemcpyHostToDevice, c->stream));
    if (n > 0) {
        hipLaunchKernelGGL(k_pair_setup, dim3(blocks_for((long long)np)), dim3(BLOCK), 0, c->stream, c->d_meta,
                           c->d_ref_slots, c->d_nbr_slots, c->d_rot, c->d_mind, c->d_maxd, c->d_act_count, c->d_theta_bad,
                           n_ref, n, c->W, c->H, c->d_refs, c->d_pairs);
    } else {
        hipLaunchKernelGGL(k_ref_setup, dim3(blocks_for(n_ref)), dim3(BLOCK), 0, c->stream, c->d_meta, c->d_ref_slots,
                           c->d_act_count, n_ref, c->d_refs);
    }
    HIP_TRY(hipGetLastError());
    k.valid = true;
    k.has_consts = (n > 0) && mind && maxd;
    k.n_ref = n_ref;
    k.n = n;
    k.epoch = c->epoch;
    k.refs.assign(ref_slots, ref_slots + n_ref);
    k.nbrs.assign(nbr_slots, nbr_slots + np);
    k.rot.assign(h_rot, h_rot + np);
    k.mind.assign(h_mind, h_mind + n_ref);
    k.maxd.assign(h_maxd, h_maxd + n_ref);
    k.long_ranges = false;
    if (k.has_consts) {
        double sum = 0.0;
        for (size_t i = 0; i < np; i++) {
            const KfMeta& m1 = c->h_meta[ref_slots[i / (size_t)n]];
            const KfMeta& m2 = c->h_meta[nbr_slots[i]];
            float F[9], R21[9], t21[3];
            pair_geometry(m1, m2, F, R21, t21);
            const float d0 = h_mind[i / (size_t)n], d1 = h_maxd[i / (size_t)n];
            float u0 = m1.fx * (R21[2] * d0 + t21[0]) / (R21[8] * d0 + t21[2]) + m1.cx;
            float u1 = m1.fx * (R21[2] * d1 + t21[0]) / (R21[8] * d1 + t21[2]) + m1.cx;
            const float cols = (float)c->W;
            u0 = u0 < 0 ? 0 : (u0 > cols ? cols : u0);
            u1 = u1 < 0 ? 0 : (u1 > cols ? cols : u1);
            const float len = std::fabs(u1 - u0);
            sum += (len == len) ? (double)len : (double)cols;
        }
        k.long_ranges = np > 0 && sum / (double)np >= (double)MASK_CALL_MEAN_L;
    }
    HIP_TRY(hipEventRecord(c->sets[victim].free_ev, c->stream));
    c->sets[victim].pending = true;
    c->sets[victim].last_use = ++c->use_tick;
    return SDM_OK;
}

int tables_staged(sdm_ctx* c)
{
    (void)c;
    return SDM_OK;
}

int push_meta(sdm_ctx* c, int slot, bool keep_istd)
{
    c->epoch++;
    hipLaunchKernelGGL(k_set_meta, dim3(1), dim3(1), 0, c->stream, c->d_meta + slot, c->h_meta[slot], keep_istd ? 1 : 0);
    HIP_TRY(hipGetLastError());
    return SDM_OK;
}

void reset_slot_state(sdm_ctx* c, int slot)
{
    c->epoch++;
    c->has_depth[slot] = 0;
    c->has_chk[slot] = 0;
    c->recon_lambdaG[slot] = std::nanf("");
    c->act_lambdaG[slot] = std::nanf("");
    c->chk_sparse[slot] = 1;
    c->xyz_sparse[slot] = 1;
    if (!c->has_obs.empty()) c->has_obs[slot] = 0;
}
int reset_slot(sdm_ctx* c, int slot)
{
    reset_slot_state(c, slot);
    HIP_TRY(hipMemsetAsync(c->pool + (long long)slot * c->P, 0, sizeof(float2) * c->P, c->stream));
    HIP_TRY(hipMemsetAsync(c->chk + (long long)slot * c->P, 0, sizeof(float) * c->P, c->stream));
    HIP_TRY(hipMemsetAsync(c->d_theta_bad + slot, 0, sizeof(int), c->stream));
    if (c->xyz) HIP_TRY(hipMemsetAsync(c->xyz + (long long)slot * c->P * 3, 0, sizeof(float) * 3 * c->P, c->stream));
    return SDM_OK;
}

void fill_meta(KfMeta& m, const float K[4], const float Tcw[12])
{
    m.fx = K[0];
    m.fy = K[1];
    m.cx = K[2];
    m.cy = K[3];
    memcpy(m.Tcw, Tcw, sizeof(float) * 12);
}

int pack_staged(sdm_ctx* c, int slot)
{
    hipLaunchKernelGGL(k_pack, dim3(blocks_for(c->P)), dim3(BLOCK), 0, c->stream, c->d_im, c->d_grad, c->d_theta,
                       c->W, c->H, c->rec + (long long)slot * c->P, c->d_theta_bad + slot);
    HIP_TRY(hipGetLastError());
    return SDM_OK;
}

template <typename T>
int dev_alloc(T** p, size_t count)
{
    HIP_TRY(hipMalloc((void**)p, sizeof(T) * std::max<size_t>(count, 1)));
    return SDM_OK;
}
template <typename T>
int host_alloc(T** p, size_t count)
{
    HIP_TRY(hipHostMalloc((void**)p, sizeof(T) * std::max<size_t>(count, 1), hipHostMallocDefault));
    return SDM_OK;
}

int alloc_ingest_bufs(sdm_ctx* c, int want)
{
    int rc;
    for (int b = 0; b < want; b++) {
        sdm_ctx::IngestBuf& B = c->ing[b];
        if (B.d_img) continue;
        if ((rc = dev_alloc(&B.d_img, (size_t)c->ing_cap * c->P)) || (rc = host_alloc(&B.h_ring, (size_t)c->ing_cap * c->P)) ||
            (rc = dev_alloc(&B.d_items, (size_t)c->ing_cap)) || (rc = host_alloc(&B.h_items, (size_t)c->ing_cap)))
            return rc;
        if (hipEventCreateWithFlags(&B.copied, hipEventDisableTiming) != hipSuccess ||
            hipEventCreateWithFlags(&B.consumed, hipEventDisableTiming) != hipSuccess)
            return fail(SDM_EHIP, "hipEventCreate failed");
    }
    return SDM_OK;
}

}

#include "sdm_comm.h"

extern "C" {

void sdm_default_params(sdm_params* p)
{
    p->lambdaG = 8.0f;
    p->lambdaL = 80.0f;
    p->lambdaTheta = 45.0f;
    p->lambdaN = 3;
    p->theta_var = 0.23;
}

void sdm_default_config(sdm_config* c)
{
    memset(c, 0, sizeof(*c));
    c->W = 640;
    c->H = 480;
    c->max_keyframes = 16;
    c->max_neighbours = 7;
    c->with_pointset = 1;
}

size_t sdm_depth_pool_bytes(int W, int H, int max_keyframes)
{
    return sizeof(float2) * (size_t)W * (size_t)H * (size_t)max_keyframes;
}

const char* sdm_last_error(void) { return g_err.c_str(); }

int sdm_device_count(void)
{
    int n = 0;
    if (hipGetDeviceCount(&n) != hipSuccess) return 0;
    return n;
}

int sdm_create(sdm_ctx** out, const sdm_config* cfg)
{
    if (!out || !cfg) return fail(SDM_EINVAL, "null argument");
    *out = nullptr;
    if (cfg->W < 8 || cfg->H < 8 || cfg->W > 16384 || cfg->H > 16384) return fail(SDM_EINVAL, "bad image size");
    if ((long long)cfg->W * cfg->H > (1ll << 27)) return fail(SDM_EINVAL, "image too large (more than 2^27 pixels)");
    if (cfg->max_keyframes < 1) return fail(SDM_EINVAL, "max_keyframes < 1");
    if (cfg->max_neighbours < 1 || cfg->max_neighbours > SDM_MAX_NEIGHBOURS)
        return fail(SDM_EINVAL, "max_neighbours out of range");
    int ndev = 0;
    if (hipGetDeviceCount(&ndev) != hipSuccess || ndev <= 0)
        return fail(SDM_ENODEV, "no HIP device visible: this engine has no CPU fallback");
    if (cfg->device < 0 || cfg->device >= ndev) return fail(SDM_EINVAL, "device ordinal out of range");
    HIP_TRY(hipSetDevice(cfg->device));
    hipDeviceProp_t prop;
    HIP_TRY(hipGetDeviceProperties(&prop, cfg->device));

    sdm_ctx* c = new sdm_ctx();
    c->cfg = *cfg;
    c->arch = prop.gcnArchName;
    c->W = cfg->W;
    c->H = cfg->H;
    c->P = (long long)cfg->W * cfg->H;
    c->geom = make_geom(cfg->W, cfg->H);
    if (c->cfg.batch_capacity <= 0) c->cfg.batch_capacity = std::min(cfg->max_keyframes, 64);
    c->cfg.batch_capacity = std::max(2, std::min(c->cfg.batch_capacity, std::max(cfg->max_keyframes, 2)));
    sdm_default_params(&c->prm);
    set_dev_params(c);
    const int K = cfg->max_keyframes;
    c->cap_refs = K;
    c->h_meta.assign(K, KfMeta{});
    c->has_depth.assign(K, 0);
    c->has_chk.assign(K, 0);
    c->act_lambdaG.assign(K, std::nanf(""));
    c->recon_lambdaG.assign(K, std::nanf(""));
    c->chk_sparse.assign(K, 1);
    c->xyz_sparse.assign(K, 1);
    c->slot_cnt.assign(K, 0);

    int rc = SDM_OK;
    auto bail = [&](int code) {
        std::string keep = g_err;
        sdm_destroy(c);
        g_err = keep;
        return code;
    };
    if (cfg->stream) {
        c->stream = (hipStream_t)cfg->stream;
    } else {
        if (hipStreamCreateWithFlags(&c->stream, hipStreamNonBlocking) != hipSuccess)
            return bail(fail(SDM_EHIP, "hipStreamCreate failed"));
        c->own_stream = true;
    }
    if ((rc = dev_alloc(&c->rec, (size_t)c->P * K))) return bail(rc);
    if (cfg->ext_depth_pool) {
        c->pool = (float2*)cfg->ext_depth_pool;
    } else {
        if ((rc = dev_alloc(&c->pool, (size_t)c->P * K))) return bail(rc);
        c->own_pool = true;
    }
    if ((rc = dev_alloc(&c->scratch, (size_t)c->P * c->cfg.batch_capacity))) return bail(rc);
    if ((rc = dev_alloc(&c->chk, (size_t)c->P * K))) return bail(rc);

    if (cfg->with_pointset)
        if ((rc = dev_alloc(&c->xyz, (size_t)c->P * 3 * K))) return bail(rc);
    if ((rc = dev_alloc(&c->d_meta, (size_t)K))) return bail(rc);
    if ((rc = dev_alloc(&c->d_act, (size_t)c->P * K))) return bail(rc);
    if ((rc = dev_alloc(&c->d_act_count, (size_t)K))) return bail(rc);
    if ((rc = dev_alloc(&c->d_theta_bad, (size_t)K))) return bail(rc);
    {
        long long cap = std::min<long long>(1ll << 20, std::max<long long>(K1_PX, c->P * K / 4));
        if (const char* e = getenv("SDM_K4_PAD")) c->k4_lds_pad = (unsigned)atoi(e);
        if (const char* e = getenv("SDM_OPEN_QUOTA")) c->open_quota = (unsigned)atoll(e);
        if (const char* e = getenv("SDM_OPEN_INPLACE")) c->open_inplace_min = (unsigned)atoll(e);
        if (const char* e = getenv("SDM_OPEN_GRID")) c->open_grid = (unsigned)std::max(1ll, atoll(e));
        if (const char* e = getenv("SDM_OPEN_CAPACITY"))
            cap = std::max<long long>(K1_PX, std::min<long long>(cap, atoll(e)));
        c->open_capacity = (unsigned)(cap / K1_PX * K1_PX);
        if ((rc = dev_alloc(&c->d_open_ctr, 8)) || (rc = dev_alloc(&c->d_open_pix, (size_t)c->open_capacity)) ||
            (rc = dev_alloc(&c->d_open_vm, (size_t)c->open_capacity)) ||
            (rc = dev_alloc(&c->d_open_hyp, (size_t)c->open_capacity * cfg->max_neighbours)))
            return bail(rc);
        const unsigned init[8] = {0u, 0xFFFFFFFFu, 0u, 0u, 0u, 0xFFFFFFFFu, 0u, 0u};
        if (hipMemcpy(c->d_open_ctr, init, sizeof(init), hipMemcpyHostToDevice) != hipSuccess)
            return bail(fail(SDM_EHIP, "open-list counter initialisation failed"));
        long long gcap = std::min<long long>(1ll << 18, c->P);
        if (const char* e = getenv("SDM_GROW_CAPACITY")) gcap = std::max<long long>(1, std::min<long long>(gcap, atoll(e)));
        c->grow_capacity = (unsigned)gcap;
        if ((rc = dev_alloc(&c->d_grow_ctr, 2)) || (rc = dev_alloc(&c->d_grow_pix, (size_t)gcap)) ||
            (rc = dev_alloc(&c->d_grow_val, (size_t)gcap)))
            return bail(rc);
        if (hipMemset(c->d_grow_ctr, 0, 2 * sizeof(unsigned)) != hipSuccess)
            return bail(fail(SDM_EHIP, "grow-list counter initialisation failed"));
    }
    {
        c->nseg = c->H * c->geom.tiles_x;
        c->ing_cap = (int)std::max<long long>(1, std::min<long long>(std::min(64, K), ((long long)32 << 20) / c->P));
        c->src_bytes = (size_t)std::max<long long>((long long)c->ing_cap * c->P, 4 * c->P);
        {
            int lo_p = 0, hi_p = 0;
            (void)hipDeviceGetStreamPriorityRange(&lo_p, &hi_p);
            if (hipStreamCreateWithPriority(&c->up_stream, hipStreamNonBlocking, hi_p) != hipSuccess)
                return bail(fail(SDM_EHIP, "hipStreamCreate failed"));
        }
        for (int i = 0; i < sdm_ctx::CNT_RING; i++)
            if (hipEventCreateWithFlags(&c->cnt_ev[i], hipEventDisableTiming) != hipSuccess)
                return bail(fail(SDM_EHIP, "hipEventCreate failed"));
        if ((rc = alloc_ingest_bufs(c, c->ing_bufs))) return bail(rc);
        const size_t gcap = (size_t)sdm_ctx::ING_GROUP * c->ing_cap;
        if ((rc = dev_alloc(&c->d_part, gcap * c->geom.ntiles * PART_WORDS)) || (rc = dev_alloc(&c->d_seg_mask, gcap * c->nseg)) ||
            (rc = dev_alloc(&c->d_seg_off, gcap * c->nseg)) || (rc = dev_alloc(&c->d_gitems, gcap)) ||
            (rc = dev_alloc(&c->d_act_hash, (size_t)K)))
            return bail(rc);
        c->mrow = 2 * (c->geom.tiles_x + 1);
        if ((rc = dev_alloc(&c->d_gmask, (size_t)K * c->H * MASK_PLANES * c->mrow))) return bail(rc);
        if (const char* e = getenv("SDM_SCAN_MODE")) c->scan_mode = std::max(0, std::min(2, atoi(e)));
        set_dev_params(c);
    }
    if ((rc = dev_alloc(&c->d_im, (size_t)c->P))) return bail(rc);
    if ((rc = dev_alloc(&c->d_grad, (size_t)c->P))) return bail(rc);
    if ((rc = dev_alloc(&c->d_theta, (size_t)c->P))) return bail(rc);
    if ((rc = dev_alloc(&c->d_small, 16))) return bail(rc);
    if ((rc = dev_alloc(&c->d_stats, STATS_WORDS))) return bail(rc);
    const size_t np = (size_t)K * cfg->max_neighbours;
    c->tab_bytes = 4 * ((size_t)K * 3 + np * 2 + 2) + sizeof(long long) * 3 * (size_t)K;
    for (int si = 0; si < sdm_ctx::TABLE_SETS; si++) {
        sdm_ctx::TableSet& s = c->sets[si];
        if ((rc = dev_alloc(&s.d_tab, c->tab_bytes)) || (rc = host_alloc(&s.h_tab, c->tab_bytes))) return bail(rc);
        if ((rc = dev_alloc(&s.d_refs, K)) || (rc = dev_alloc(&s.d_pairs, np))) return bail(rc);
        if (hipEventCreateWithFlags(&s.free_ev, hipEventDisableTiming) != hipSuccess)
            return bail(fail(SDM_EHIP, "hipEventCreate failed"));
    }
    select_set(c, 0, 1, 0);
    if ((rc = host_alloc(&c->h_f2, (size_t)c->P))) return bail(rc);
    if ((rc = host_alloc(&c->h_act_count, (size_t)K))) return bail(rc);
    memset(c->h_act_count, 0, sizeof(int) * (size_t)K);

    if (hipMemsetAsync(c->rec, 0, sizeof(float4) * c->P * K, c->stream) != hipSuccess ||
        hipMemsetAsync(c->pool, 0, sizeof(float2) * c->P * K, c->stream) != hipSuccess ||
        hipMemsetAsync(c->chk, 0, sizeof(float) * c->P * K, c->stream) != hipSuccess ||
        hipMemsetAsync(c->d_meta, 0, sizeof(KfMeta) * K, c->stream) != hipSuccess ||
        hipMemsetAsync(c->d_act_count, 0, sizeof(int) * K, c->stream) != hipSuccess ||
        hipMemsetAsync(c->d_theta_bad, 0, sizeof(int) * K, c->stream) != hipSuccess ||
        hipMemsetAsync(c->d_act_hash, 0, sizeof(unsigned long long) * K, c->stream) != hipSuccess ||
        hipMemsetAsync(c->d_gmask, 0, sizeof(unsigned) * (size_t)K * c->H * MASK_PLANES * c->mrow, c->stream) != hipSuccess ||
        hipMemsetAsync(c->d_stats, 0, sizeof(unsigned long long) * STATS_WORDS, c->stream) != hipSuccess ||
        (c->xyz && hipMemsetAsync(c->xyz, 0, sizeof(float) * 3 * c->P * K, c->stream) != hipSuccess) ||
        hipStreamSynchronize(c->stream) != hipSuccess)
        return bail(fail(SDM_EHIP, "initial memset failed"));

    const int max_lds = (int)k1_lds_bytes(cfg->max_neighbours);
    if (hipFuncSetAttribute((const void*)k_search_fuse<false, false>, hipFuncAttributeMaxDynamicSharedMemorySize, max_lds) != hipSuccess ||
        hipFuncSetAttribute((const void*)k_search_fuse<true, false>, hipFuncAttributeMaxDynamicSharedMemorySize, max_lds) != hipSuccess ||
        hipFuncSetAttribute((const void*)k_search_fuse<false, true>, hipFuncAttributeMaxDynamicSharedMemorySize, max_lds) != hipSuccess ||
        hipFuncSetAttribute((const void*)k_search_fuse<true, true>, hipFuncAttributeMaxDynamicSharedMemorySize, max_lds) != hipSuccess)
        return bail(fail(SDM_EHIP, "hipFuncSetAttribute(max dynamic LDS) failed"));
    *out = c;
    return SDM_OK;
}

void sdm_destroy(sdm_ctx* c)
{
    if (!c) return;
    (void)hipSetDevice(c->cfg.device);
    if (c->stream) (void)hipStreamSynchronize(c->stream);
    comm_release(c);
    (void)hipFree(c->rec);
    if (c->own_pool) (void)hipFree(c->pool);
    (void)hipFree(c->scratch);
    (void)hipFree(c->chk);

    (void)hipFree(c->xyz);
    (void)hipFree(c->d_meta);
    (void)hipFree(c->d_act);
    (void)hipFree(c->d_act_count);
    (void)hipFree(c->d_theta_bad);
    (void)hipFree(c->d_open_ctr);
    (void)hipFree(c->d_open_pix);
    (void)hipFree(c->d_open_vm);
    (void)hipFree(c->d_open_hyp);
    (void)hipFree(c->d_grow_ctr);
    (void)hipFree(c->d_grow_pix);
    (void)hipFree(c->d_grow_val);
    if (c->up_stream) (void)hipStreamSynchronize(c->up_stream);
    for (int b = 0; b < sdm_ctx::ING_BUFS_MAX; b++) {
        sdm_ctx::IngestBuf& B = c->ing[b];
        (void)hipFree(B.d_img);
        (void)hipFree(B.d_src);
        (void)hipFree(B.d_items);
        (void)hipHostFree(B.h_ring);
        (void)hipHostFree(B.h_src);
        (void)hipHostFree(B.h_items);
        if (B.copied) (void)hipEventDestroy(B.copied);
        if (B.consumed) (void)hipEventDestroy(B.consumed);
    }
    if (c->up_stream) (void)hipStreamDestroy(c->up_stream);
    for (int i = 0; i < sdm_ctx::CNT_RING; i++)
        if (c->cnt_ev[i]) (void)hipEventDestroy(c->cnt_ev[i]);
    (void)hipFree(c->d_part);
    (void)hipFree(c->d_seg_mask);
    (void)hipFree(c->d_seg_off);
    (void)hipFree(c->d_gitems);
    (void)hipFree(c->d_act_hash);
    (void)hipFree(c->d_gmask);
    (void)hipFree(c->d_im);
    (void)hipFree(c->d_grad);
    (void)hipFree(c->d_theta);
    (void)hipFree(c->d_small);
    (void)hipFree(c->d_stats);
    for (int si = 0; si < sdm_ctx::TABLE_SETS; si++) {
        sdm_ctx::TableSet& s = c->sets[si];
        (void)hipFree(s.d_tab);
        (void)hipFree(s.d_refs);
        (void)hipFree(s.d_pairs);
        (void)hipHostFree(s.h_tab);
        if (s.free_ev) (void)hipEventDestroy(s.free_ev);
    }
    (void)hipHostFree(c->h_f2);
    (void)hipHostFree(c->h_act_count);
    (void)hipFree(c->d_ext);
    (void)hipFree(c->d_ext_stage);
    (void)hipFree(c->d_vox);
    (void)hipFree(c->d_vox_out);
    (void)hipHostFree(c->h_ext);
    (void)hipFree(c->obs.ids);
    (void)hipFree(c->obs.ang);
    (void)hipFree(c->obs.depth);
    (void)hipFree(c->obs.cnt);
    (void)hipFree(c->obs.nd);
    (void)hipFree(c->d_obs_stage);
    (void)hipHostFree(c->h_obs_stage);
    (void)hipFree(c->d_pri);
    (void)hipHostFree(c->h_pri);
    (void)hipFree(c->obs.cov_ids);
    (void)hipFree(c->obs.cov_cnt);
    (void)hipFree(c->d_cov);
    (void)hipHostFree(c->h_cov);
    for (auto& sp : c->spans) {
        (void)hipEventDestroy(sp.a);
        (void)hipEventDestroy(sp.b);
    }
    if (c->own_stream && c->stream) (void)hipStreamDestroy(c->stream);
    delete c;
}

int sdm_set_params(sdm_ctx* c, const sdm_params* p)
{
    if (!c || !p) return fail(SDM_EINVAL, "null argument");
    if (!(p->theta_var > 0) || p->lambdaN < 0) return fail(SDM_EINVAL, "bad parameter value");
    c->prm = *p;
    set_dev_params(c);
    return validate_params(c);
}

int sdm_get_params(sdm_ctx* c, sdm_params* out)
{
    if (!c || !out) return fail(SDM_EINVAL, "null argument");
    *out = c->prm;
    return SDM_OK;
}

int sdm_set_stream(sdm_ctx* c, void* s)
{
    if (!c) return fail(SDM_EINVAL, "null context");
    HIP_TRY(hipStreamSynchronize(c->stream));
    c->cnt_done = c->cnt_next - 1;
    if (c->own_stream) {
        (void)hipStreamDestroy(c->stream);
        c->own_stream = false;
    }
    c->stream = (hipStream_t)s;
    return SDM_OK;
}

int sdm_synchronize(sdm_ctx* c)
{
    if (!c) return fail(SDM_EINVAL, "null context");
    HIP_TRY(hipStreamSynchronize(c->stream));
    return SDM_OK;
}

const char* sdm_device_arch(sdm_ctx* c) { return c ? c->arch.c_str() : ""; }

int sdm_upload_keyframe(sdm_ctx* c, int slot, const uint8_t* im, const float* grad, const float* theta, float I_stddev,
                        const float K[4], const float Tcw[12])
{
    int rc = check_slot(c, slot, false);
    if (rc) return rc;
    if (!im || !grad || !theta || !K || !Tcw) return fail(SDM_EINVAL, "null input plane");
    HIP_TRY(hipSetDevice(c->cfg.device));
    if ((rc = reset_slot(c, slot))) return rc;
    HIP_TRY(hipMemcpyAsync(c->d_im, im, (size_t)c->P, hipMemcpyHostToDevice, c->stream));
    HIP_TRY(hipMemcpyAsync(c->d_grad, grad, sizeof(float) * c->P, hipMemcpyHostToDevice, c->stream));
    HIP_TRY(hipMemcpyAsync(c->d_theta, theta, sizeof(float) * c->P, hipMemcpyHostToDevice, c->stream));
    if ((rc = pack_staged(c, slot))) return rc;
    KfMeta& m = c->h_meta[slot];
    fill_meta(m, K, Tcw);
    m.I_stddev = I_stddev;
    m.uploaded = 1;
    if ((rc = push_meta(c, slot, false))) return rc;
    if ((rc = build_active(c, slot))) return rc;
    return sync_counts(c);
}

namespace {

std::mutex g_pinned_mutex;
std::map<const uint8_t*, size_t> g_pinned_blocks;
bool host_pinned(const void* p, size_t bytes)
{
    std::lock_guard<std::mutex> lock(g_pinned_mutex);
    const uint8_t* q = (const uint8_t*)p;
    auto it = g_pinned_blocks.upper_bound(q);
    if (it == g_pinned_blocks.begin()) return false;
    --it;
    return q >= it->first && q + bytes <= it->first + it->second;
}

struct Stager {
    struct Plan {
        uint8_t* dst = nullptr;
        const uint8_t* const* src = nullptr;
        int m = 0;
        size_t bytes = 0;
    };
    int nt = 1;
    std::vector<std::thread> th;
    std::vector<Plan> plans;
    std::vector<std::atomic<int> > done;
    std::mutex mu;
    std::condition_variable cv;
    int posted = 0;
    bool quit = false;

    Stager(int threads, int chunks) noexcept
    {
        try {
            plans.resize((size_t)chunks);
            done = std::vector<std::atomic<int> >((size_t)chunks);
            for (auto& d : done) d.store(0);
            th.reserve((size_t)std::max(0, threads - 1));
            for (int t = 1; t < threads; t++)
                th.emplace_back([this, t] {
                    for (size_t k = 0; k < plans.size(); k++) {
                        {
                            std::unique_lock<std::mutex> lock(mu);
                            cv.wait(lock, [&] { return quit || posted > (int)k; });
                            if (quit) return;
                        }
                        share(plans[k], t);
                        done[k].fetch_add(1, std::memory_order_release);
                    }
                });
        } catch (...) {
        }
        nt = 1 + (int)th.size();
    }
    bool usable() const { return !plans.empty() && done.size() == plans.size(); }
    void share(const Plan& p, int t) const
    {
        for (int i = t; i < p.m; i += nt) memcpy(p.dst + (size_t)i * p.bytes, p.src[i], p.bytes);
    }
    void stage(int k, uint8_t* dst, const uint8_t* const* src, int m, size_t bytes)
    {
        Plan p;
        p.dst = dst;
        p.src = src;
        p.m = m;
        p.bytes = bytes;
        if (!usable() || nt == 1) {
            for (int i = 0; i < m; i++) memcpy(dst + (size_t)i * bytes, src[i], bytes);
            return;
// ... 1 lines not shown
        plans[(size_t)k] = p;
        {
            std::lock_guard<std::mutex> lock(mu);
            posted = k + 1;
        }
        cv.notify_all();
        share(p, 0);
        while (done[(size_t)k].load(std::memory_order_acquire) < nt - 1) std::this_thread::yield();
    }
    ~Stager()
    {
        {
            std::lock_guard<std::mutex> lock(mu);
            quit = true;
        }
        cv.notify_all();
        for (auto& x : th)
            if (x.joinable()) x.join();
    }
};

int check_batch_slots(sdm_ctx* c, int n, const int* slots)
{
    if (!c) return fail(SDM_EINVAL, "null context");
    if (n < 0 || (n > 0 && !slots)) return fail(SDM_EINVAL, "bad slot list");
    std::vector<char> seen((size_t)c->cfg.max_keyframes, 0);
    for (int i = 0; i < n; i++) {
        int rc = check_slot(c, slots[i], false);
        if (rc) return rc;
        if (seen[slots[i]]) return fail(SDM_EINVAL, "duplicate slot in one upload batch");
        seen[slots[i]] = 1;
    }
    return SDM_OK;
}

int ensure_src_buffers(sdm_ctx* c)
{
    if (c->ing[0].d_src && c->ing[c->ing_bufs - 1].d_src) return SDM_OK;
    int rc;
    for (int b = 0; b < c->ing_bufs; b++) {
        if (c->ing[b].d_src) continue;
        if ((rc = dev_alloc(&c->ing[b].d_src, c->src_bytes))) return rc;
        if ((rc = host_alloc(&c->ing[b].h_src, c->src_bytes))) return rc;
    }
    return SDM_OK;
}

int ingest_images_impl(sdm_ctx* c, int n, const int* slots, const uint8_t* const* images, bool on_device, const IngestParams* q,
                  const float* K, const float* Tcw)
{
    static const bool dbg = getenv("SDM_DEBUG_INGEST_TIMING") != nullptr;
    static const double dbg_ms = dbg && atof(getenv("SDM_DEBUG_INGEST_TIMING")) > 0 ? atof(getenv("SDM_DEBUG_INGEST_TIMING")) : 2.0;
    auto now = [] { return std::chrono::duration<double, std::milli>(std::chrono::steady_clock::now().time_since_epoch()).count(); };
    const double t_entry = dbg ? now() : 0.0;
    int rc = check_batch_slots(c, n, slots);
    if (rc) return rc;
    if (n == 0) return SDM_OK;
    if (!images || !K || !Tcw) return fail(SDM_EINVAL, "null input");
    for (int i = 0; i < n; i++)
        if (!images[i]) return fail(SDM_EINVAL, "null image");
    HIP_TRY(hipSetDevice(c->cfg.device));
    if (q && (rc = ensure_src_buffers(c))) return rc;
    const size_t bytes = (size_t)c->P * (q ? q->channels : 1);
    int cap = q ? (int)std::max<size_t>(1, std::min<size_t>((size_t)c->ing_cap, c->src_bytes / bytes)) : c->ing_cap;
    cap = std::max(1, std::min(cap, std::max(4, (n + 3) / 4)));
    bool direct = false;
    int last = -1;
    std::vector<char> pinned((size_t)n, 0);
    size_t pageable_bytes = 0;
    for (int i = 0; i < n && !on_device; i++) {
        pinned[i] = host_pinned(images[i], bytes) ? 1 : 0;
        if (!pinned[i]) pageable_bytes += bytes;
    }
    const int hw = (int)std::thread::hardware_concurrency();
    const int n_chunks = (n + cap - 1) / cap;
    static const int max_stagers = [] {
        const char* e = getenv("SDM_STAGER_THREADS");
        return e ? std::max(1, std::min(16, atoi(e))) : 4;
    }();
    Stager stager((pageable_bytes >= ((size_t)2 << 20) && hw >= 4) ? std::min(max_stagers, hw / 2) : 1, n_chunks);
    const hipStream_t cs = n_chunks > 1 ? c->up_stream : c->stream;
    double tdbg[5] = {0, 0, 0, 0, 0};
    const double t_loop = dbg ? now() : 0.0;
    int failed_from = n;
    int group_kfs = 0, group_chunks = 0;
    int group_first = 0;
    const bool merge = c->ingest_overlap && n_chunks > 1 && !q && !on_device && cs != c->stream;
    int merged_bufs[CHUNK_TABLES] = {0, 0, 0, 0};
    auto finish_group = [&]() -> int {
        const int g = group_kfs, nch = group_chunks;
        group_kfs = group_chunks = 0;
        int r = SDM_OK;
        if (merge && nch > 0) r = ingest_launch_chunks_merged(c, nch, merged_bufs, cap, g);
        if (!r) r = ingest_launch_group(c, g, true);
        return r;
    };
    auto bail = [&](int code) {
        const std::string keep = g_err;
        if (direct) (void)hipStreamSynchronize(cs);
        (void)finish_group();
        (void)counts_queued(c, failed_from, slots);
        for (int i = failed_from; i < n; i++) {
            reset_slot_state(c, slots[i]);
            c->h_meta[slots[i]].uploaded = 0;
        }
        g_err = keep;
        return code;
    };
    for (int i0 = 0, chunk = 0; i0 < n; i0 += cap, chunk++) {
        const int m = std::min(cap, n - i0);
        failed_from = i0;
        const int b = c->ing_next;
        c->ing_next = (c->ing_next + 1) % c->ing_bufs;
        sdm_ctx::IngestBuf& B = c->ing[b];
        if (dbg) tdbg[0] = now();
        if ((rc = ingest_acquire(c, b, cs))) return bail(rc);
        if (dbg) tdbg[1] = now();
        uint8_t* d_dst = q ? B.d_src : B.d_img;
        uint8_t* h_dst = q ? B.h_src : B.h_ring;
        for (int i = 0; i < m; i++) {
            IngestItem& it = B.h_items[i];
            memset(&it, 0, sizeof(it));
            it.slot = slots[i0 + i];
            it.img = on_device ? images[i0 + i] : B.d_img + (size_t)i * c->P;
            it.src = q ? B.d_src + (size_t)i * bytes : nullptr;
            fill_meta(it.meta, K + 4 * (size_t)(i0 + i), Tcw + 12 * (size_t)(i0 + i));
            it.meta.uploaded = 1;
        }
        if (!on_device) {
            int n_pinned = 0;
            for (int i = 0; i < m; i++) n_pinned += pinned[i0 + i];
            if (n_pinned == m) {
                for (int i = 0; i < m;) {
                    int r = 1;
                    while (i + r < m && images[i0 + i + r] == images[i0 + i + r - 1] + bytes) r++;
                    if (hipMemcpyAsync(d_dst + (size_t)i * bytes, images[i0 + i], (size_t)r * bytes, hipMemcpyHostToDevice, cs) != hipSuccess)
                        return bail(fail(SDM_EHIP, "hipMemcpyAsync (pinned image) failed"));
                    direct = true;
                    i += r;
                }
                direct = true;
            } else {
                stager.stage(chunk, h_dst, images + i0, m, bytes);
                if (hipMemcpyAsync(d_dst, h_dst, (size_t)m * bytes, hipMemcpyHostToDevice, cs) != hipSuccess)
                    return bail(fail(SDM_EHIP, "hipMemcpyAsync (staged images) failed"));
            }
        }
        if (dbg) tdbg[2] = now();
        if ((rc = ingest_publish(c, b, m, cs, !merge))) return bail(rc);
        if (dbg) tdbg[3] = now();
        for (int i = 0; i < m; i++) {
            const int slot = slots[i0 + i];
            reset_slot_state(c, slot);
            c->h_meta[slot] = B.h_items[i].meta;
            c->act_lambdaG[slot] = c->dprm.lambdaG;
            c->recon_lambdaG[slot] = c->dprm.lambdaG;
        }
        if (merge)
            merged_bufs[group_chunks] = b;
        else if ((rc = ingest_launch_chunk(c, b, m, group_kfs, true, q)))
            return bail(rc);
        group_kfs += m;
        group_chunks++;
        failed_from = i0 + m;
        if (group_chunks == sdm_ctx::ING_GROUP || i0 + m >= n) {
            if ((rc = finish_group())) {
                failed_from = group_first;
                return bail(rc);
            }
            group_first = i0 + m;
        }
        if (dbg) {
            tdbg[4] = now();
            if (tdbg[4] - tdbg[0] > dbg_ms)
                fprintf(stderr, "[sdm ingest] slow chunk: acquire %.3f  images %.3f  publish %.3f  launch %.3f ms\n",
                        tdbg[1] - tdbg[0], tdbg[2] - tdbg[1], tdbg[3] - tdbg[2], tdbg[4] - tdbg[3]);
        }
        last = b;
    }
    if ((rc = counts_queued(c, n, slots))) return rc;
    const double t_tail = dbg ? now() : 0.0;
    if (direct && last >= 0) {
        HIP_TRY(hipEventSynchronize(c->ing[last].copied));
        c->ing[last].copied_pending = false;
    }
    if (dbg && now() - t_entry > dbg_ms)
        fprintf(stderr, "[sdm ingest] slow call (%d keyframes): set-up %.3f  chunks %.3f  final wait %.3f ms\n", n, t_loop - t_entry,
                t_tail - t_loop, now() - t_tail);
    return SDM_OK;
}

int ingest_images(sdm_ctx* c, int n, const int* slots, const uint8_t* const* images, bool on_device, const IngestParams* q,
                  const float* K, const float* Tcw)
{
    try {
        return ingest_images_impl(c, n, slots, images, on_device, q, K, Tcw);
    } catch (const std::exception& e) {
        return fail(SDM_EHIP, std::string("ingest: ") + e.what());
    } catch (...) {
        return fail(SDM_EHIP, "ingest: unknown exception");
    }
}

int colour_order(int order, IngestParams& q)
{
    switch (order) {
        case SDM_ORDER_RGB: q.channels = 3; q.r_idx = 0; q.g_idx = 1; q.b_idx = 2; break;
        case SDM_ORDER_BGR: q.channels = 3; q.r_idx = 2; q.g_idx = 1; q.b_idx = 0; break;
        case SDM_ORDER_RGBA: q.channels = 4; q.r_idx = 0; q.g_idx = 1; q.b_idx = 2; break;
        case SDM_ORDER_BGRA: q.channels = 4; q.r_idx = 2; q.g_idx = 1; q.b_idx = 0; break;
        case SDM_ORDER_GRAY: q.channels = 1; break;
        default: return fail(SDM_EINVAL, "unknown colour order");
    }
    return SDM_OK;
}

}

int sdm_upload_images_batch(sdm_ctx* c, int n, const int* slots, const uint8_t* const* images, const float* K, const float* Tcw)
{
    return ingest_images(c, n, slots, images, false, nullptr, K, Tcw);
}

int sdm_upload_image(sdm_ctx* c, int slot, const uint8_t* im, const float K[4], const float Tcw[12])
{
    return ingest_images(c, 1, &slot, &im, false, nullptr, K, Tcw);
}

int sdm_upload_images_rgb_batch(sdm_ctx* c, int n, const int* slots, const uint8_t* const* pixels, int order, const float* K,
                                const float dist[5], const float* Tcw)
{
    if (!c) return fail(SDM_EINVAL, "null context");
    if (n > 0 && !K) return fail(SDM_EINVAL, "null input");
    IngestParams q{};
    int rc = colour_order(order, q);
    if (rc) return rc;
    if (n > 0) {
        q.fx = K[0]; q.fy = K[1]; q.cx = K[2]; q.cy = K[3];
        for (int i = 1; i < n && dist; i++)
            if (memcmp(K, K + 4 * (size_t)i, sizeof(float) * 4) != 0)
                return fail(SDM_EINVAL, "one batch undistorts with one camera: the K of its frames differ");
    }
    q.undistort = dist != nullptr;
    if (dist) { q.k1 = dist[0]; q.k2 = dist[1]; q.p1 = dist[2]; q.p2 = dist[3]; q.k3 = dist[4]; }
    if (dist && n > 0 && !(K[0] != 0.0f && K[1] != 0.0f)) return fail(SDM_EINVAL, "zero focal length");
    return ingest_images(c, n, slots, pixels, false, &q, K, Tcw);
}

int sdm_upload_image_rgb(sdm_ctx* c, int slot, const uint8_t* pixels, int order, const float K[4], const float dist[5],
                         const float Tcw[12])
{
    return sdm_upload_images_rgb_batch(c, 1, &slot, &pixels, order, K, dist, Tcw);
}

int sdm_upload_image_device(sdm_ctx* c, int slot, const void* d_im, const float K[4], const float Tcw[12])
{
    const uint8_t* im = (const uint8_t*)d_im;
    int rc = ingest_images(c, 1, &slot, &im, true, nullptr, K, Tcw);
    if (rc) return rc;
    return sync_counts(c);
}

void* sdm_host_alloc(size_t bytes)
{
    void* p = nullptr;
    if (hipHostMalloc(&p, std::max<size_t>(bytes, 1), hipHostMallocDefault) != hipSuccess) {
        (void)hipGetLastError();
        return nullptr;
    }
    std::lock_guard<std::mutex> lock(g_pinned_mutex);
    g_pinned_blocks[(const uint8_t*)p] = std::max<size_t>(bytes, 1);
    return p;
}

void sdm_host_free(void* p)
{
    if (!p) return;
    {
        std::lock_guard<std::mutex> lock(g_pinned_mutex);
        g_pinned_blocks.erase((const uint8_t*)p);
    }
    (void)hipHostFree(p);
}

int sdm_set_pose(sdm_ctx* c, int slot, const float Tcw[12])
{
    int rc = check_slot(c, slot, true);
    if (rc) return rc;
    if (!Tcw) return fail(SDM_EINVAL, "null pose");
    if (memcmp(c->h_meta[slot].Tcw, Tcw, sizeof(float) * 12) == 0) return SDM_OK;
    memcpy(c->h_meta[slot].Tcw, Tcw, sizeof(float) * 12);
    return push_meta(c, slot, true);
}

int sdm_download_inputs(sdm_ctx* c, int slot, uint8_t* im, float* grad, float* theta, float* I_stddev)
{
    int rc = check_slot(c, slot, true);
    if (rc) return rc;
    HIP_TRY(hipSetDevice(c->cfg.device));
    hipLaunchKernelGGL(k_unpack, dim3(blocks_for(c->P)), dim3(BLOCK), 0, c->stream, c->rec + (long long)slot * c->P,
                       (int)c->P, c->d_im, c->d_grad, c->d_theta);
    HIP_TRY(hipGetLastError());
    if (im) HIP_TRY(hipMemcpyAsync(im, c->d_im, (size_t)c->P, hipMemcpyDeviceToHost, c->stream));
    if (grad) HIP_TRY(hipMemcpyAsync(grad, c->d_grad, sizeof(float) * c->P, hipMemcpyDeviceToHost, c->stream));
    if (theta) HIP_TRY(hipMemcpyAsync(theta, c->d_theta, sizeof(float) * c->P, hipMemcpyDeviceToHost, c->stream));
    if (I_stddev)
        HIP_TRY(hipMemcpyAsync(I_stddev, &c->d_meta[slot].I_stddev, sizeof(float), hipMemcpyDeviceToHost, c->stream));
    HIP_TRY(hipStreamSynchronize(c->stream));
    return SDM_OK;
}

static bool all_pipeline_maps(sdm_ctx* c, int n_ref, const int* ref_slots);

static int launch_search_fuse(sdm_ctx* c, int n_ref, int n, const int* ref_slots)
{
    if (!all_pipeline_maps(c, n_ref, ref_slots)) {
        for_ref_slices(n_ref, blocks_for(c->P), BLOCK, [&](int first, int count) {
            hipLaunchKernelGGL(k_zero_maps, dim3(blocks_for(c->P * count)), dim3(BLOCK), 0, c->stream, c->pool, c->P,
                               c->d_ref_slots + first, count);
        });
        HIP_TRY(hipGetLastError());
    }
    StageTimer tm(c, SDM_STAGE_SEARCH_FUSE);
    int max_chunks = 0;
    for (int r = 0; r < n_ref; r++) max_chunks = std::max(max_chunks, (c->h_act_count[ref_slots[r]] + K1_PX - 1) / K1_PX);
    if (max_chunks == 0) return SDM_OK;
    const size_t lds = k1_lds_bytes(n);
    const int blocks_per_ref = 8 * ((max_chunks + 7) / 8);
    OpenList ol;
    ol.count = c->d_open_ctr + 4 * (c->open_launch & 1u);
    ol.next = c->d_open_ctr + 4 * ((c->open_launch + 1u) & 1u);
    ol.capacity = c->open_capacity;
    ol.quota = c->open_quota;
    ol.inplace_min = c->open_inplace_min;
    ol.pix = c->d_open_pix;
    ol.vm = c->d_open_vm;
    ol.hyp = c->d_open_hyp;
    c->open_launch++;
    const size_t lds_open = (sizeof(float2) + sizeof(float)) * (size_t)K1_PX * n + sizeof(unsigned) * (size_t)K1_PX * ((n + 3) / 4);
    const int grid_open = (int)std::min<unsigned>(c->open_capacity / K1_PX, c->open_grid);
    const bool mask = c->scan_mode == 2 || (c->scan_mode == 0 && c->sets[c->cur_set].key.long_ranges);
    auto k1 = c->stats_on ? (mask ? k_search_fuse<true, true> : k_search_fuse<true, false>)
                          : (mask ? k_search_fuse<false, true> : k_search_fuse<false, false>);
    for_ref_slices(n_ref, blocks_per_ref, K1_BLOCK, [&](int first, int count) {
        hipLaunchKernelGGL(k1, dim3(blocks_per_ref * count), dim3(K1_BLOCK), lds, c->stream, c->rec, c->P, c->d_refs + first,
                           c->d_pairs + (size_t)first * n, count, n, c->W, c->H, max_chunks, c->dprm, c->d_act, c->pool, c->d_stats,
                           ol, c->d_gmask, c->mrow);
    });
    if (c->stats_on)
        hipLaunchKernelGGL(k_fuse_open<true>, dim3(grid_open), dim3(K1_BLOCK), lds_open, c->stream, ol, n, c->dprm, c->pool,
                           c->P * c->cfg.max_keyframes, c->d_stats);
    else
        hipLaunchKernelGGL(k_fuse_open<false>, dim3(grid_open), dim3(K1_BLOCK), lds_open, c->stream, ol, n, c->dprm, c->pool,
                           c->P * c->cfg.max_keyframes, c->d_stats);
    HIP_TRY(hipGetLastError());
    return SDM_OK;
}

int sdm_active_count(sdm_ctx* c, int slot, int* count)
{
    int rc = check_slot(c, slot, true);
    if (rc) return rc;
    if (!count) return fail(SDM_EINVAL, "null argument");
    HIP_TRY(hipSetDevice(c->cfg.device));
    if (!(c->act_lambdaG[slot] == c->dprm.lambdaG))
        if ((rc = build_active(c, slot))) return rc;
    if ((rc = sync_counts(c))) return rc;
    *count = c->h_act_count[slot];
    return SDM_OK;
}

int sdm_download_active_list(sdm_ctx* c, int slot, unsigned* list, int capacity, int* count, unsigned long long* hash)
{
    int n = 0;
    int rc = sdm_active_count(c, slot, &n);
    if (rc) return rc;
    if (count) *count = n;
    if (list && capacity < n) return fail(SDM_EINVAL, "list buffer too small");
    HIP_TRY(hipStreamSynchronize(c->stream));
    if (list && n > 0)
        HIP_TRY(hipMemcpy(list, c->d_act + (long long)slot * c->P, sizeof(unsigned) * (size_t)n, hipMemcpyDeviceToHost));
    if (hash) HIP_TRY(hipMemcpy(hash, c->d_act_hash + slot, sizeof(unsigned long long), hipMemcpyDeviceToHost));
    return SDM_OK;
}

int sdm_search_fuse(sdm_ctx* c, int n_ref, const int* ref_slots, int n, const int* nbr_slots, const float* rot,
                    const float* mind, const float* maxd)
{
    if (!c) return fail(SDM_EINVAL, "null context");
    if (n < 1) return fail(SDM_EINVAL, "need at least one neighbour");
    if (!mind || !maxd) return fail(SDM_EINVAL, "null depth bounds");
    int rc = stage_tables(c, n_ref, ref_slots, n, nbr_slots, rot, mind, maxd, true);
    if (rc) return rc;
    if ((rc = launch_search_fuse(c, n_ref, n, ref_slots))) return rc;
    for (int r = 0; r < n_ref; r++) {
        c->has_depth[ref_slots[r]] = 1;
        c->recon_lambdaG[ref_slots[r]] = c->dprm.lambdaG;
    }
    return tables_staged(c);
}

static int launch_intra(sdm_ctx* c, int n_ref, int first, int count, bool check, bool grow)
{
    const int K = n_ref;
    if (check) {
        for_ref_slices(count, grid_blocks(c->geom, 1), BLOCK, [&](int f, int cn) {
            hipLaunchKernelGGL(k_intra_check, dim3(grid_blocks(c->geom, cn)), dim3(BLOCK), 0, c->stream, c->pool, c->scratch,
                               c->d_off + first + f, c->d_off + K + first + f, cn, c->geom);
        });
        HIP_TRY(hipGetLastError());
    }
    if (grow) {
        for_ref_slices(count, grid_blocks(c->geom, 1), BLOCK, [&](int f, int cn) {
            hipLaunchKernelGGL(k_intra_grow, dim3(grid_blocks(c->geom, cn)), dim3(BLOCK), 0, c->stream, c->scratch, c->pool,
                               c->d_off + K + first + f, c->d_off + first + f, (const float*)c->rec,
                               c->d_off + 2 * K + first + f, 4, cn, c->geom, c->dprm.lambdaG);
        });
        HIP_TRY(hipGetLastError());
    }
    return SDM_OK;
}

static int run_intra_lists(sdm_ctx* c, int n_ref, const int* ref_slots, bool check, bool grow)
{
    int rc = SDM_OK;
    StageTimer tm(c, SDM_STAGE_INTRA);
    const int K = n_ref, cap = c->cfg.batch_capacity;
    for (int first = 0; first < n_ref; first += cap) {
        const int count = std::min(cap, n_ref - first);
        int max_chunks = 0;
        for (int r = 0; r < count; r++)
            max_chunks = std::max(max_chunks, (c->h_act_count[ref_slots[first + r]] + BLOCK - 1) / BLOCK);
        if (max_chunks == 0) continue;
        const int per_ref = band_grid_per_ref(max_chunks, SDM_K23_GROUP, SDM_K23_BAND);
#if SDM_INTRA_COMPACT
        GrowList gl;
        gl.count = c->d_grow_ctr + (c->grow_launch & 1u);
        gl.next = c->d_grow_ctr + ((c->grow_launch + 1u) & 1u);
        gl.capacity = c->grow_capacity;
        gl.pix = c->d_grow_pix;
        gl.val = c->d_grow_val;
        for_ref_slices(count, per_ref, BLOCK, [&](int f, int cn) {
            if (check && grow)
                hipLaunchKernelGGL((k_intra_compact<true, true>), dim3(per_ref * cn), dim3(BLOCK), 0, c->stream, c->pool,
                                   c->scratch, c->d_off, c->d_off + K, c->d_refs, first + f, cn, c->W, max_chunks, c->P,
                                   c->d_act, gl);
            else if (check)
                hipLaunchKernelGGL((k_intra_compact<true, false>), dim3(per_ref * cn), dim3(BLOCK), 0, c->stream, c->pool,
                                   c->scratch, c->d_off, c->d_off + K, c->d_refs, first + f, cn, c->W, max_chunks, c->P,
                                   c->d_act, gl);
            else
                hipLaunchKernelGGL((k_intra_compact<false, true>), dim3(per_ref * cn), dim3(BLOCK), 0, c->stream, c->pool,
                                   c->scratch, c->d_off, c->d_off + K, c->d_refs, first + f, cn, c->W, max_chunks, c->P,
                                   c->d_act, gl);
        });
        HIP_TRY(hipGetLastError());
        if (check) {
            for_ref_slices(count, per_ref, BLOCK, [&](int f, int cn) {
                hipLaunchKernelGGL(k_intra_commit, dim3(per_ref * cn), dim3(BLOCK), 0, c->stream, c->pool, c->scratch, c->d_off,
                                   c->d_off + K, c->d_refs, first + f, cn, c->W, max_chunks, c->P, c->d_act);
            });
            HIP_TRY(hipGetLastError());
        }
        if (grow) {
            hipLaunchKernelGGL(k_grow, dim3(1), dim3(GROW_BLOCK), 0, c->stream, c->pool, gl, c->W, c->P, c->scratch, c->d_off,
                               c->d_off + K, c->d_refs, first, count, c->d_act);
            HIP_TRY(hipGetLastError());
            c->grow_launch++;
        }
#else
        if (check) {
            if (!grow) HIP_TRY(hipMemsetAsync(c->scratch, 0, sizeof(float2) * c->P * count, c->stream));
            for_ref_slices(count, per_ref, BLOCK, [&](int f, int cn) {
                hipLaunchKernelGGL(k_intra_list<false>, dim3(per_ref * cn), dim3(BLOCK), 0, c->stream, c->pool, c->scratch,
                                   c->d_off, c->d_off + K, c->d_refs, first + f, cn, c->W, max_chunks, c->P, c->d_act, c->rec,
                                   c->H, c->dprm.lambdaG);
            });
            HIP_TRY(hipGetLastError());
        } else {
            for (int r = 0; r < count; r++)
                HIP_TRY(hipMemcpyAsync(c->scratch + (long long)r * c->P, c->pool + c->h_off[first + r],
                                       sizeof(float2) * c->P, hipMemcpyDeviceToDevice, c->stream));
        }
        if (grow) {
            for_ref_slices(count, per_ref, BLOCK, [&](int f, int cn) {
                hipLaunchKernelGGL(k_intra_list<true>, dim3(per_ref * cn), dim3(BLOCK), 0, c->stream, c->scratch, c->pool,
                                   c->d_off + K, c->d_off, c->d_refs, first + f, cn, c->W, max_chunks, c->P, c->d_act, c->rec,
                                   c->H, c->dprm.lambdaG);
            });
            HIP_TRY(hipGetLastError());
        } else {
            for (int r = 0; r < count; r++)
                HIP_TRY(hipMemcpyAsync(c->pool + c->h_off[first + r], c->scratch + (long long)r * c->P,
                                       sizeof(float2) * c->P, hipMemcpyDeviceToDevice, c->stream));
        }
#endif
// ... 1130 lines not shown
    }
}

int sdm_covisible_neighbours(sdm_ctx* c, int n_ref, const int* ref_slots, int n_cand, const int* cand_slots, int n,
                             int min_weight, int* nbr_slots, int* nbr_weights, int* counts)
{
    try {
        if (c && !nbr_slots) return fail(SDM_EINVAL, "null nbr_slots");
        if (c && n < 1) return fail(SDM_EINVAL, "n out of [1, max_neighbours]");
        return covis_impl(c, n_ref, ref_slots, n_cand, cand_slots, n, min_weight, nullptr, nbr_slots, nbr_weights, counts);
    } catch (const std::exception& e) {
        return fail(SDM_EHIP, std::string("covisible neighbours: ") + e.what());
    }
}

int sdm_recon_covisible(sdm_ctx* c, int n_ref, const int* ref_slots, int n_cand, const int* cand_slots, int n, int min_weight,
                        int* nbr_slots_out, unsigned char* done)
{
    try {
        if (c && !done) return fail(SDM_EINVAL, "null done");
        if (c && n < 1) return fail(SDM_EINVAL, "n out of [1, max_neighbours]");
        if (c && n_ref <= 0) return fail(SDM_EINVAL, "n_ref <= 0 or null ref_slots");
        std::vector<int> nbrs((size_t)std::max(n_ref, 0) * n), counts((size_t)std::max(n_ref, 0));
        int rc = covis_impl(c, n_ref, ref_slots, n_cand, cand_slots, n, min_weight, nullptr, nbrs.data(), nullptr, counts.data());
        if (rc) return rc;
        std::vector<int> refs2, nbrs2;
        for (int r = 0; r < n_ref; r++)
            if (counts[r] == n) {
                refs2.push_back(ref_slots[r]);
                nbrs2.insert(nbrs2.end(), nbrs.begin() + (size_t)r * n, nbrs.begin() + (size_t)(r + 1) * n);
            }
        if (!refs2.empty() && (rc = sdm_recon_observed(c, (int)refs2.size(), refs2.data(), n, nbrs2.data()))) return rc;
        for (int r = 0; r < n_ref; r++) done[r] = counts[r] == n;
        if (nbr_slots_out) memcpy(nbr_slots_out, nbrs.data(), sizeof(int) * nbrs.size());
        return SDM_OK;
    } catch (const std::exception& e) {
        return fail(SDM_EHIP, std::string("recon covisible: ") + e.what());
    }
}

int sdm_enable_stats(sdm_ctx* c, int on)
{
    if (!c) return fail(SDM_EINVAL, "null context");
    c->stats_on = on != 0;
    return SDM_OK;
}

int sdm_selftest(sdm_ctx* c, int which, unsigned long long out[2])
{
    if (!c || !out) return fail(SDM_EINVAL, "null argument");
    HIP_TRY(hipSetDevice(c->cfg.device));
    HIP_TRY(hipMemsetAsync(c->d_stats, 0, sizeof(unsigned long long) * STATS_WORDS, c->stream));
    if (which == 0) {
        hipLaunchKernelGGL(k_selftest_div, dim3(4096), dim3(BLOCK), 0, c->stream, c->dprm.theta_var, c->dprm.inv_theta,
                           c->d_stats + 5);
    } else if (which == 1) {
        hipLaunchKernelGGL(k_selftest_chi, dim3(1024), dim3(BLOCK), 0, c->stream, 1024, c->d_stats + 5,
                           c->d_stats + 6);
    } else if (which == 2) {
        hipLaunchKernelGGL(k_selftest_cost, dim3(1024), dim3(BLOCK), 0, c->stream, c->dprm, 2048, c->d_stats + 5,
                           c->d_stats + 6);
    } else if (which == 4) {
        hipLaunchKernelGGL(k_selftest_fusion_terms, dim3(4096), dim3(BLOCK), 0, c->stream, 2048, c->d_stats + 5,
                           c->d_stats + 6);
    } else if (which == 5) {
        hipLaunchKernelGGL(k_selftest_quot, dim3(4096), dim3(BLOCK), 0, c->stream, 8192, c->d_stats + 5,
                           c->d_stats + 6);
    } else if (which == 7 || which == 9) {
        const int blocks = 1024;
        float2* d_patch = nullptr;
        PairConst* d_pc = nullptr;
        HIP_TRY(hipMalloc(&d_patch, sizeof(float2) * 6 * blocks * BLOCK));
        if (hipMalloc(&d_pc, sizeof(PairConst) * blocks * BLOCK) != hipSuccess) {
            (void)hipFree(d_patch);
            return fail(SDM_EHIP, "selftest scratch allocation failed");
        }
        hipLaunchKernelGGL(k_selftest_k4, dim3(blocks), dim3(BLOCK), 0, c->stream, 2048, d_patch, d_pc, c->d_stats + 5,
                           c->d_stats + 6, which == 9 ? 1 : 0);
        hipError_t e = hipGetLastError();
        if (e == hipSuccess) e = hipMemcpyAsync(out, c->d_stats + 5, sizeof(unsigned long long) * 2, hipMemcpyDeviceToHost, c->stream);
        if (e == hipSuccess) e = hipStreamSynchronize(c->stream);
        (void)hipFree(d_patch);
        (void)hipFree(d_pc);
        if (e != hipSuccess) return fail(SDM_EHIP, hipGetErrorString(e));
        HIP_TRY(hipMemsetAsync(c->d_stats, 0, sizeof(unsigned long long) * STATS_WORDS, c->stream));
        return SDM_OK;
    } else if (which == 6) {
        hipLaunchKernelGGL(k_selftest_rcp, dim3(4096), dim3(BLOCK), 0, c->stream, c->d_stats + 5, c->d_stats + 6);
    } else if (which == 8) {
        hipLaunchKernelGGL(k_selftest_scan_ids, dim3(4096), dim3(BLOCK), 0, c->stream, c->d_stats + 5, c->d_stats + 6);
    } else if (which == 10) {
        hipLaunchKernelGGL(k_selftest_atan_x1, dim3(4096), dim3(BLOCK), 0, c->stream, c->d_stats + 5, c->d_stats + 6);
    } else if (which == 3) {
        hipLaunchKernelGGL(k_selftest_gates, dim3(4096), dim3(BLOCK), 0, c->stream, c->dprm, c->d_stats + 5, c->d_stats + 6);
    } else {
        return fail(SDM_EINVAL, "unknown selftest");
    }
    HIP_TRY(hipGetLastError());
    HIP_TRY(hipMemcpyAsync(out, c->d_stats + 5, sizeof(unsigned long long) * 2, hipMemcpyDeviceToHost, c->stream));
    HIP_TRY(hipStreamSynchronize(c->stream));
    HIP_TRY(hipMemsetAsync(c->d_stats, 0, sizeof(unsigned long long) * STATS_WORDS, c->stream));
    return SDM_OK;
}

int sdm_enable_timing(sdm_ctx* c, int on)
{
    if (!c) return fail(SDM_EINVAL, "null context");
    c->timing_on = on != 0;
    return SDM_OK;
}

int sdm_get_timing(sdm_ctx* c, double ms_total[SDM_NUM_STAGES], long long launches[SDM_NUM_STAGES], int reset)
{
    if (!c || !ms_total || !launches) return fail(SDM_EINVAL, "null argument");
    HIP_TRY(hipStreamSynchronize(c->stream));
    for (int i = 0; i < SDM_NUM_STAGES; i++) {
        ms_total[i] = 0.0;
        launches[i] = 0;
    }
    for (size_t i = 0; i < c->spans_used; i++) {
        float ms = 0.f;
        HIP_TRY(hipEventElapsedTime(&ms, c->spans[i].a, c->spans[i].b));
        ms_total[c->spans[i].stage] += (double)ms;
        launches[c->spans[i].stage]++;
    }
    if (reset) c->spans_used = 0;
    return SDM_OK;
}

int sdm_set_ingest_overlap(sdm_ctx* c, int on)
{
    if (!c) return fail(SDM_EINVAL, "null context");
    HIP_TRY(hipSetDevice(c->cfg.device));
    if (on && c->ing_bufs < sdm_ctx::ING_BUFS_MAX) {
        HIP_TRY(hipStreamSynchronize(c->stream));
        if (c->up_stream) HIP_TRY(hipStreamSynchronize(c->up_stream));
        const int rc = alloc_ingest_bufs(c, sdm_ctx::ING_BUFS_MAX);
        if (rc) return rc;
        c->ing_bufs = sdm_ctx::ING_BUFS_MAX;
    }
    c->ingest_overlap = on != 0;
    return SDM_OK;
}

int sdm_set_scan_mode(sdm_ctx* c, int mode)
{
    if (!c) return fail(SDM_EINVAL, "null context");
    if (mode < 0 || mode > 2) return fail(SDM_EINVAL, "scan mode must be 0, 1 or 2");
    c->scan_mode = mode;
    set_dev_params(c);
    return SDM_OK;
}

int sdm_get_stats(sdm_ctx* c, sdm_stats* out, int reset)
{
    if (!c || !out) return fail(SDM_EINVAL, "null argument");
    unsigned long long v[STATS_WORDS];
    HIP_TRY(hipMemcpyAsync(v, c->d_stats, sizeof(v), hipMemcpyDeviceToHost, c->stream));
    HIP_TRY(hipStreamSynchronize(c->stream));
    out->searches = (long long)v[0];
    out->candidates = (long long)v[1];
    out->gate_pass = (long long)v[2];
    out->hypotheses = (long long)v[3];
    out->fused = (long long)v[4];
    out->mask_waves = (long long)v[5];
    out->mask_steps = (long long)v[6];
    out->mask_row_mismatch = (long long)v[7];
    out->open_pixels = (long long)v[8];
    out->table_stagings = c->table_stagings;
    if (reset) c->table_stagings = 0;
    if (reset) HIP_TRY(hipMemsetAsync(c->d_stats, 0, sizeof(v), c->stream));
    return SDM_OK;
}

}
```

orb-slam-free-space-carving_amd/csrc/sdm_ingest.h:

```cpp
#pragma once
#include "sdm_device.h"

namespace sdm {

constexpr int TILE_W = 64;
constexpr int TILE_H = 16;
constexpr int TILE_PX = TILE_W * TILE_H;
constexpr int BLOCK = 256;
constexpr int PX_PER_THREAD = TILE_PX / BLOCK;

struct IngestItem {
    const uint8_t* img;
    const uint8_t* src;
    int slot;
    int keep_istd;
    KfMeta meta;
};
constexpr int CHUNK_TABLES = 4;
struct ChunkTables {
    const IngestItem* p[CHUNK_TABLES];
    int per;
};
__device__ __forceinline__ const IngestItem& chunk_item(const ChunkTables& t, int kf)
{
// ... 131 lines not shown
    const unsigned long long G = __builtin_amdgcn_ballot_w64(sgate);
    const unsigned long long R = __builtin_amdgcn_ballot_w64(sgate & in_range);
    unsigned long long mine = R;
#pragma unroll
    for (int k = 0; k < 4; k++) {
        const unsigned long long Bk = __builtin_amdgcn_ballot_w64((bin >> k) & 1);
        const unsigned long long flip = ((mybin >> k) & 1) ? 0ull : ~0ull;
        mine &= Bk ^ flip;
    }
    mine |= G & ~R;
    if (lane == MASK_UNION) mine = G;
    if (store && lane < MASK_PLANES) {
        gmask[row_dword0 + (long long)(2 * tx) * MASK_PLANES + lane] = (unsigned)mine;
        gmask[row_dword0 + (long long)(2 * tx + 1) * MASK_PLANES + lane] = (unsigned)(mine >> 32);
    }
}

template <bool ZERO>
__global__ __launch_bounds__(BLOCK) void k_prepass_batch(const ChunkTables tabs, int W, int H, int tiles_x,
                                                         long long plane, float4* __restrict__ rec,
                                                         float2* __restrict__ pool, float* __restrict__ chk,
                                                         float* __restrict__ xyz, float lambdaG,
                                                         unsigned long long* __restrict__ part,
                                                         unsigned long long* __restrict__ seg_mask, int nseg,
                                                         unsigned* __restrict__ gmask, int mrow, int kf0,
                                                         IngestItem* __restrict__ gitems)
{
    __shared__ uint8_t t[PRE_HALO_H][PRE_HALO_W];
    __shared__ float gm[TILE_H + 1][TILE_W];
    __shared__ unsigned long long red[PART_WORDS * (BLOCK / 64)];
    const int kf = blockIdx.y, tile = blockIdx.x, tid = threadIdx.x;
    const int gkf = kf0 + kf;
    const IngestItem& item = chunk_item(tabs, kf);
    const uint8_t* __restrict__ im = item.img;
    const int slot = item.slot;
    if (tile == 0 && tid == 0) gitems[gkf] = item;
    const int tx = tile % tiles_x, ty = tile / tiles_x;
    const int tx0 = tx * TILE_W, ty0 = ty * TILE_H;
    const int lx = tid & (TILE_W - 1), wv = __builtin_amdgcn_readfirstlane(tid >> 6);
    for (int hy = wv; hy < PRE_HALO_H; hy += BLOCK / 64) {
        const uint8_t* __restrict__ row = im + (long long)min(max(ty0 + hy - 1, 0), H - 1) * W;
        t[hy][lx] = row[min(max(tx0 + lx - 1, 0), W - 1)];
        if (lx < PRE_HALO_W - TILE_W) t[hy][TILE_W + lx] = row[min(max(tx0 + TILE_W + lx - 1, 0), W - 1)];
    }
    __syncthreads();
    float th[PX_PER_THREAD];
    unsigned s1 = 0u, s2 = 0u;
    unsigned long long hsum = 0ull;
    bool bad = false;
#pragma unroll
    for (int i = 0; i < PX_PER_THREAD; i++) {
        const int ly = i * (BLOCK / 64) + wv;
        float gx, gy;
        int centre;
        scharr32(t, lx, ly, gx, gy, centre);
        const float xx = gx * gx, yy = gy * gy;
        gm[ly][lx] = sqrt_grad(xx + yy);
        th[i] = fast_atan2_deg(gy, gx);
        if (tx0 + lx < W && ty0 + ly < H) {
            s1 += (unsigned)centre;
            s2 += (unsigned)(centre * centre);
        }
    }
    if (wv == 0) {
        float gx, gy;
        int centre;
        scharr32(t, lx, TILE_H, gx, gy, centre);
        const float xx = gx * gx, yy = gy * gy;
        gm[TILE_H][lx] = sqrt_grad(xx + yy);
    }
    __syncthreads();
    const long long base = (long long)slot * plane;
#pragma unroll
    for (int i = 0; i < PX_PER_THREAD; i++) {
        const int ly = i * (BLOCK / 64) + wv;
        const int x = tx0 + lx, y = ty0 + ly;
        const bool in = x < W && y < H;
        bool gate = false, sgate = false, odd = false;
        if (in) {
            const bool below = y + 1 < H;
            const unsigned bits = (unsigned)t[ly + 1][lx + 1] | ((below ? (unsigned)t[ly + 2][lx + 1] : 0u) << 8);
            float4 r;
            r.x = gm[ly][lx];
            r.y = th[i];
            r.z = below ? gm[ly + 1][lx] : 0.0f;
            r.w = __uint_as_float(bits);
            const long long o = base + (long long)y * W + x;
            rec[o] = r;
            if (ZERO) {
                pool[o] = make_float2(0.f, 0.f);
                chk[o] = 0.f;
            }
            gate = act_gate(r.x, x, y, W, H, lambdaG);
            sgate = !(r.x < lambdaG);
            odd = !(r.y >= 0.0f && r.y <= 360.0f);
        }
        bad = bad || __builtin_amdgcn_ballot_w64(odd) != 0ull;
        if (ZERO && xyz && y < H) {
            float* __restrict__ z = xyz + (base + (long long)y * W + tx0) * 3;
            const int nz = 3 * min(TILE_W, W - tx0);
#pragma unroll
            for (int k = 0; k < 3; k++)
                if (lx + TILE_W * k < nz) z[lx + TILE_W * k] = 0.f;
        }
        const unsigned long long m = __builtin_amdgcn_ballot_w64(gate);
        hsum += seg_hash_term(m, (unsigned)y, (unsigned)tx0);
        if (lx == 0 && y < H) seg_mask[(long long)gkf * nseg + (long long)y * tiles_x + tx] = m;
        write_gate_planes(gmask, ((long long)slot * H + y) * MASK_PLANES * mrow, tx, sgate, th[i], y < H);
    }
    tile_partials(s1, s2, hsum, bad, red, part + ((long long)gkf * gridDim.x + tile) * PART_WORDS);
}

__global__ __launch_bounds__(BLOCK) void k_gate_batch(const IngestItem* __restrict__ items, int W, int H, int tiles_x,
                                                      long long plane, const float4* __restrict__ rec, float lambdaG,
                                                      unsigned long long* __restrict__ part,
                                                      unsigned long long* __restrict__ seg_mask, int nseg,
                                                      unsigned* __restrict__ gmask, int mrow, int kf0,
                                                      IngestItem* __restrict__ gitems)
{
    __shared__ unsigned long long red[PART_WORDS * (BLOCK / 64)];
    const int kf = blockIdx.y, tile = blockIdx.x, tid = threadIdx.x;
    const int gkf = kf0 + kf;
    const int slot = items[kf].slot;
    if (tile == 0 && tid == 0) gitems[gkf] = items[kf];
    const int tx = tile % tiles_x, ty = tile / tiles_x;
    const int lx = tid & (TILE_W - 1), wv = __builtin_amdgcn_readfirstlane(tid >> 6);
    const float4* __restrict__ r = rec + (long long)slot * plane;
    unsigned long long hsum = 0ull;
#pragma unroll
    for (int i = 0; i < PX_PER_THREAD; i++) {
        const int x = tx * TILE_W + lx, y = ty * TILE_H + i * (BLOCK / 64) + wv;
        bool gate = false, sgate = false;
        float theta = 0.0f;
        if (x < W && y < H) {
            const float4 rr = r[(long long)y * W + x];
            gate = act_gate(rr.x, x, y, W, H, lambdaG);
            sgate = !(rr.x < lambdaG);
            theta = rr.y;
        }
        const unsigned long long m = __builtin_amdgcn_ballot_w64(gate);
        hsum += seg_hash_term(m, (unsigned)y, (unsigned)(tx * TILE_W));
        if (lx == 0 && y < H) seg_mask[(long long)gkf * nseg + (long long)y * tiles_x + tx] = m;
        write_gate_planes(gmask, ((long long)slot * H + y) * MASK_PLANES * mrow, tx, sgate, theta, y < H);
    }
    tile_partials(0u, 0u, hsum, false, red, part + ((long long)gkf * gridDim.x + tile) * PART_WORDS);
}

constexpr int FIN_BLOCK = 1024;
__global__ __launch_bounds__(FIN_BLOCK) void k_prepass_finish(const IngestItem* __restrict__ items, int W, int H, int ntiles,
                                                              int nseg, const unsigned long long* __restrict__ part,
                                                              const unsigned long long* __restrict__ seg_mask,
                                                              int* __restrict__ seg_off, KfMeta* __restrict__ meta,
                                                              int* __restrict__ act_count, int* __restrict__ host_count,
                                                              int* __restrict__ theta_bad,
                                                              unsigned long long* __restrict__ act_hash, int full)
{
    __shared__ unsigned long long red[PART_WORDS][FIN_BLOCK / 64];
    __shared__ int wtot[FIN_BLOCK / 64];
    const int kf = blockIdx.x, tid = threadIdx.x, lane = tid & 63, wv = tid >> 6;
    const IngestItem it = items[kf];
    unsigned long long v[PART_WORDS] = {0ull, 0ull, 0ull, 0ull};
    for (int i = tid; i < ntiles; i += FIN_BLOCK)
#pragma unroll
        for (int k = 0; k < PART_WORDS; k++) v[k] += part[((long long)kf * ntiles + i) * PART_WORDS + k];
#pragma unroll
    for (int k = 0; k < PART_WORDS; k++) {
        for (int o = 32; o > 0; o >>= 1) v[k] += __shfl_down(v[k], o);
        if (lane == 0) red[k][wv] = v[k];
    }
    const unsigned long long* __restrict__ sm = seg_mask + (long long)kf * nseg;
    int* __restrict__ so = seg_off + (long long)kf * nseg;
    const int per = (nseg + FIN_BLOCK - 1) / FIN_BLOCK;
    const int s0 = tid * per, s1 = min(s0 + per, nseg);
    int mine = 0;
    for (int s = s0; s < s1; s++) mine += __popcll(sm[s]);
    int incl = mine;
    for (int o = 1; o < 64; o <<= 1) {
        const int up = __shfl_up(incl, o);
        if (lane >= o) incl += up;
    }
    if (lane == 63) wtot[wv] = incl;
    __syncthreads();
    int wbase = 0, total = 0;
    for (int w = 0; w < FIN_BLOCK / 64; w++) {
        if (w == wv) wbase = total;
        total += wtot[w];
    }
    int run = wbase + incl - mine;
    for (int s = s0; s < s1; s++) {
        so[s] = run;
        run += __popcll(sm[s]);
    }
    if (tid == 0) {
        unsigned long long tot[PART_WORDS];
        for (int k = 0; k < PART_WORDS; k++) {
            tot[k] = 0;
            for (int w = 0; w < FIN_BLOCK / 64; w++) tot[k] += red[k][w];
        }
        act_count[it.slot] = total;
        host_count[it.slot] = total;
        act_hash[it.slot] = tot[2];
        if (full) {
            KfMeta m = it.meta;
            if (it.keep_istd) {
                m.I_stddev = meta[it.slot].I_stddev;
            } else {
                const double n = (double)W * (double)H;
                const double mean = (double)tot[0] / n;
                double var = (double)tot[1] / n - mean * mean;
                if (var < 0) var = 0;
                m.I_stddev = (float)sqrt(var);
            }
            meta[it.slot] = m;
            theta_bad[it.slot] = tot[3] ? 1 : 0;
        }
    }
}

constexpr int LIST_SEGS = 16;
__global__ __launch_bounds__(BLOCK) void k_list_write(const IngestItem* __restrict__ items, int tiles_x, int nseg,
                                                      long long plane, const unsigned long long* __restrict__ seg_mask,
                                                      const int* __restrict__ seg_off, unsigned* __restrict__ act)
{
    const int kf = blockIdx.y;
    const int s0 = (blockIdx.x * (BLOCK / 64) + (int)(threadIdx.x >> 6)) * LIST_SEGS, lane = threadIdx.x & 63;
    if (s0 >= nseg) return;
    const int mine = min(s0 + (lane & (LIST_SEGS - 1)), nseg - 1);
    const unsigned long long mm = seg_mask[(long long)kf * nseg + mine];
    const int mo = seg_off[(long long)kf * nseg + mine];
    unsigned* __restrict__ out = act + (long long)items[kf].slot * plane;
    int y = s0 / tiles_x, tx = s0 - y * tiles_x;
#pragma unroll
    for (int j = 0; j < LIST_SEGS; j++) {
        if (s0 + j < nseg) {
            const unsigned long long m = ((unsigned long long)(unsigned)__builtin_amdgcn_readlane((int)(mm >> 32), j) << 32) |
                                         (unsigned)__builtin_amdgcn_readlane((int)mm, j);
            const int off = __builtin_amdgcn_readlane(mo, j);
            if ((m >> lane) & 1ull)
                out[off + __popcll(m & ((1ull << lane) - 1ull))] = ((unsigned)y << 16) | (unsigned)(tx * TILE_W + lane);
        }
        if (++tx == tiles_x) {
            tx = 0;
            y++;
        }
    }
}

__global__ __launch_bounds__(BLOCK) void k_pack(const uint8_t* __restrict__ im, const float* __restrict__ grad,
                                                const float* __restrict__ theta, int W, int H,
                                                float4* __restrict__ rec, int* __restrict__ theta_bad)
{
    int idx = blockIdx.x * BLOCK + threadIdx.x;
    bool bad = false;
    if (idx < W * H) {
        int y = idx / W;
        bool below = (y + 1 < H);
        unsigned bits = (unsigned)im[idx] | ((below ? (unsigned)im[idx + W] : 0u) << 8);
        float4 r;
        r.x = grad[idx];
        r.y = theta[idx];
        r.z = below ? grad[idx + W] : 0.0f;
        r.w = __uint_as_float(bits);
        rec[idx] = r;
        bad = !(r.y >= 0.0f && r.y <= 360.0f);
    }
    if (__builtin_amdgcn_ballot_w64(bad) != 0ull && (threadIdx.x & 63) == 0) atomicOr(theta_bad, 1);
}

__global__ __launch_bounds__(BLOCK) void k_unpack(const float4* __restrict__ rec, int n, uint8_t* __restrict__ im,
                                                  float* __restrict__ grad, float* __restrict__ theta)
{
    int idx = blockIdx.x * BLOCK + threadIdx.x;
    if (idx >= n) return;
    float4 r = rec[idx];
    im[idx] = (uint8_t)(__float_as_uint(r.w) & 0xffu);
    grad[idx] = r.x;
    theta[idx] = r.y;
}

__global__ void k_set_meta(KfMeta* __restrict__ dst, KfMeta m, int keep_istd)
{
    if (keep_istd) m.I_stddev = dst->I_stddev;
    *dst = m;
}

}
```

orb-slam-free-space-carving_amd/csrc/sdm_kernels.h:

```cpp
#pragma once
#include "sdm_device.h"
#include "sdm_ingest.h"

namespace sdm {

#ifndef SDM_INTRA_COMPACT
#define SDM_INTRA_COMPACT 1
#endif

struct TileGeom {
    int W, H, tiles_x, tiles_y, ntiles;
};

__host__ __device__ inline TileGeom make_geom(int W, int H)
{
    TileGeom g;
    g.W = W;
    g.H = H;
    g.tiles_x = (W + TILE_W - 1) / TILE_W;
    g.tiles_y = (H + TILE_H - 1) / TILE_H;
    g.ntiles = g.tiles_x * g.tiles_y;
    return g;
}
__host__ inline int grid_blocks(const TileGeom& g, int n_ref) { return 8 * ((g.ntiles + 7) / 8) * n_ref; }
// ... 110 lines not shown
    int r = idx / n, j = idx - r * n;
    KfMeta m1 = meta[ref_slots[r]];
    KfMeta m2 = meta[nbr_slots[idx]];
    PairConst pc;
    float R21[9], t21[3];
    pair_geometry(m1, m2, pc.F, R21, t21);
    for (int i = 0; i < 3; i++) {
        pc.Rx[i] = R21[i];
        pc.Ry[i] = R21[3 + i];
        pc.Rz[i] = R21[6 + i];
    }
    pc.tx = t21[0];
    pc.ty = t21[1];
    pc.tz = t21[2];
    pc.rot = rot ? rot[idx] : 0.0f;
    pc.istd = m2.I_stddev;
    pc.nbr_slot = nbr_slots[idx];
    pc.nfx = m2.fx;
    pc.nfy = m2.fy;
    pc.ncx = m2.cx;
    pc.ncy = m2.cy;
    pc.clean = ((theta_bad[ref_slots[r]] == 0 && theta_bad[nbr_slots[idx]] == 0 && pc.rot >= -360.0f && pc.rot <= 360.0f) ? 1 : 0) |
               (line_quot_safe(pc.F) ? 2 : 0);
    {
        float umin, umax;
        search_range(m1.fx, m1.cx, pc.Rx[2], pc.Rz[2], pc.tx, pc.tz, mind ? mind[r] : 0.f, maxd ? maxd[r] : 0.f, W, umin, umax);
        if (!(umax - umin < (float)MASK_HINT_L)) pc.clean |= 4;
    }
    {
        const float s = 1.0f + 0x1p-20f;
        const float X0 = fmaxf(fabsf(m1.cx), fabsf((float)(W - 1) - m1.cx)) / fabsf(m1.fx) * s;
        const float X1 = fmaxf(fabsf(m1.cy), fabsf((float)(H - 1) - m1.cy)) / fabsf(m1.fy) * s;
        k4_proj_bounds(pc, X0, X1);
    }
    pairs[idx] = pc;
    if (j == 0) {
        RefConst rc;
        rc.slot = ref_slots[r];
        rc.fx = m1.fx;
        rc.fy = m1.fy;
        rc.cx = m1.cx;
        rc.cy = m1.cy;
        rc.mind = mind ? mind[r] : 0.f;
        rc.maxd = maxd ? maxd[r] : 0.f;
        rc.act_count = act_counts[ref_slots[r]];
        refs[r] = rc;
    }
}

__global__ void k_ref_setup(const KfMeta* __restrict__ meta, const int* __restrict__ ref_slots,
                            const int* __restrict__ act_counts, int n_ref, RefConst* __restrict__ refs)
{
    int r = blockIdx.x * blockDim.x + threadIdx.x;
    if (r >= n_ref) return;
    KfMeta m = meta[ref_slots[r]];
    RefConst rc;
    rc.slot = ref_slots[r];
    rc.fx = m.fx;
    rc.fy = m.fy;
    rc.cx = m.cx;
    rc.cy = m.cy;
    rc.mind = 0.f;
    rc.maxd = 0.f;
    rc.act_count = act_counts[ref_slots[r]];
    refs[r] = rc;
}

__global__ __launch_bounds__(BLOCK) void k_zero_maps(float2* __restrict__ pool, long long plane,
                                                     const int* __restrict__ slots, int n_ref)
{
    long long idx = (long long)blockIdx.x * BLOCK + threadIdx.x;
    if (idx >= plane * n_ref) return;
    int r = (int)(idx / plane);
    long long p = idx - (long long)r * plane;
    pool[(long long)slots[r] * plane + p] = make_float2(0.f, 0.f);
}

#ifndef SDM_K1_WAVES
#define SDM_K1_WAVES 4
#endif
constexpr int K1_PX = 64;
constexpr int K1_WAVES = SDM_K1_WAVES;
constexpr int K1_BLOCK = K1_PX * K1_WAVES;
constexpr int K1_OUTLIER_ROWS = 4;
__host__ __device__ inline size_t k1_lds_bytes(int n)
{
    const size_t nn = (size_t)(n > 0 ? n : 1);
    const size_t cw = (nn + 3) / 4 > (size_t)K1_OUTLIER_ROWS ? (nn + 3) / 4 : (size_t)K1_OUTLIER_ROWS;
    return (sizeof(float2) + sizeof(float)) * (size_t)K1_PX * nn + sizeof(unsigned) * (size_t)K1_PX * cw +
           sizeof(unsigned long long) * K1_BLOCK + sizeof(unsigned long long) * K1_PX + sizeof(unsigned) * K1_PX + 16;
}

constexpr int STATS_WORDS = 16;
struct OpenList {
    unsigned* count;
    unsigned* next;
    unsigned capacity;
    unsigned quota;
    unsigned inplace_min;
    long long* pix;
    unsigned long long* vm;
    float2* hyp;
};

__device__ __forceinline__ void k1_count_all_pairs(const float2* hyp, const float* sgm, unsigned* cnt, unsigned long long vm,
                                                   int n, int p, int w)
{
    for (int i = 0; K1_WAVES * i < n; i++) {
        const int a = K1_WAVES * i + ((i & 1) ? (K1_WAVES - 1 - w) : w);
        if (a >= n || !((vm >> a) & 1ull)) continue;
        const float2 ha = hyp[a * K1_PX + p];
        const float sa = sgm[a * K1_PX + p];
        unsigned c = (sa * sa > 0.0f) ? 1u : 0u;
        for (int bb = a + 1; bb < n; bb++) {
            const float2 hb = hyp[bb * K1_PX + p];
            if (chi_test_lazy(ha, hb, sa, &sgm[bb * K1_PX + p])) {
                c++;
                atomicAdd(&cnt[(bb >> 2) * K1_PX + p], 1u << (8 * (bb & 3)));
            }
        }
        atomicAdd(&cnt[(a >> 2) * K1_PX + p], c << (8 * (a & 3)));
    }
}
__device__ __forceinline__ bool k1_fuse_counted(const float2* hyp, const float* sgm, const unsigned* cnt, unsigned long long vm,
                                                int n, int p, int lambdaN, float2& result)
{
    unsigned best = 0;
    int besta = 0;
    for (int a = 0; a < n; a++) {
        if (!((vm >> a) & 1ull)) continue;
        const unsigned c = (cnt[(a >> 2) * K1_PX + p] >> (8 * (a & 3))) & 0xffu;
        if (c > best) {
            best = c;
            besta = a;
        }
    }
    if ((int)best < lambdaN) return false;
    const float2 ha = hyp[besta * K1_PX + p];
    const float sa = sgm[besta * K1_PX + p];
    float pjsj = 0.f, rsj = 0.f;
    for (int bb = 0; bb < n; bb++) {
        if (!((vm >> bb) & 1ull)) continue;
        const float2 hb = hyp[bb * K1_PX + p];
        const bool in = (bb == besta) ? (sa * sa > 0.0f) : chi_test_lazy(ha, hb, sa, &sgm[bb * K1_PX + p]);
        if (in) fusion_accum(hb.x, sgm[bb * K1_PX + p], pjsj, rsj);
    }
    result = make_float2(pjsj / rsj, sqrtf(1 / rsj));
    return true;
}

#ifndef SDM_K1_EU_MIN
#define SDM_K1_EU_MIN 8
#endif
#ifndef SDM_K1_LB
#define SDM_K1_LB __launch_bounds__(K1_BLOCK) __attribute__((amdgpu_waves_per_eu(SDM_K1_EU_MIN, 8)))
#endif
template <bool STATS, bool MASK>
__global__ SDM_K1_LB void k_search_fuse(const float4* __restrict__ rec, long long plane,
                                                       const RefConst* __restrict__ refs,
                                                       const PairConst* __restrict__ pairs, int n_ref, int n,
                                                       int W, int H, int max_chunks, DevParams prm,
                                                       const unsigned* __restrict__ act, float2* __restrict__ pool,
                                                       unsigned long long* __restrict__ stats, OpenList open_list,
                                                       const unsigned* __restrict__ gmask, int mrow)
{
    extern __shared__ __align__(16) unsigned char smem_raw[];
    float2* hyp = reinterpret_cast<float2*>(smem_raw);
    float* sgm = reinterpret_cast<float*>(hyp + (size_t)n * K1_PX);
    unsigned* cnt = reinterpret_cast<unsigned*>(sgm + (size_t)n * K1_PX);
    const int cnt_words = max((n + 3) >> 2, K1_OUTLIER_ROWS);
    unsigned long long* pmask = reinterpret_cast<unsigned long long*>(cnt + (size_t)cnt_words * K1_PX);
    unsigned long long* set0 = pmask + K1_BLOCK;
    unsigned* cnt0 = reinterpret_cast<unsigned*>(set0 + K1_PX);
    unsigned* xbase = cnt0 + K1_PX;

    const int b = blockIdx.x;
    const int i8 = b >> 3;
    const int cl = i8 / n_ref;
    const int ref = i8 - cl * n_ref;
    const int chunk = cl * 8 + (b & 7);
    if (chunk >= max_chunks) return;
    const RefConst rc = refs[ref];
    if (chunk * K1_PX >= rc.act_count) return;
    const int tid = threadIdx.x, p = tid & (K1_PX - 1);
    const int w = __builtin_amdgcn_readfirstlane(tid >> 6);
    const int t = chunk * K1_PX + p;
    const bool on = t < rc.act_count;
    const float4* __restrict__ rrec = rec + (long long)rc.slot * plane;

    int x = 2, y = 2;
    float pixel = 0.f, grad1 = 0.f, th_pi = 0.f, xp0 = 0.f, xp1 = 0.f;
    if (on) {
        unsigned xy = act[(long long)rc.slot * plane + t];
        x = (int)(xy & 0xffffu);
        y = (int)(xy >> 16);
        float4 r = rrec[y * W + x];
        pixel = (float)(int)(__float_as_uint(r.w) & 0xffu);
        grad1 = r.x;
        th_pi = r.y;
        xp0 = ((float)x - rc.cx) / rc.fx;
        xp1 = ((float)y - rc.cy) / rc.fy;
    }
    SearchStats st = {0, 0, 0};
    MaskStats ms = {0, 0, 0};
    MaskView mv;
    mv.row_pitch = (unsigned)mrow * MASK_WORD_BYTES;
    const PairConst* __restrict__ pcs = pairs + (long long)ref * n;
    const float rcvb[4] = {rc.fx, rc.cx, rc.mind, rc.maxd};
    const float* __restrict__ rcv = rcvb;
    unsigned long long mymask = 0;
    for (int j = w; j < n; j += K1_WAVES) {
        const PairConst* __restrict__ pc = pcs + j;
        const float4* __restrict__ nrec = rec + (long long)pc->nbr_slot * plane;
        float2 h = make_float2(__builtin_inff(), 1.0f);
#if SDM_K1_OPT & 0x1000
        {
            float rho, sigma, bu, bv;
            const float* __restrict__ cv = reinterpret_cast<const float*>(pc);
            bool ok = epipolar_search<STATS, true>(nrec, W, H, cv, rcv, pc->clean, on, x, y, pixel, grad1, th_pi, xp0, xp1, prm,
                                                   rho, sigma, bu, bv, &st);
            if (ok && __float_as_uint(rho) < 0x7f800000u) {
                h = make_float2(rho, sigma);
                mymask |= 1ull << j;
            }
        }
#else
        if (on) {
            float rho, sigma, bu, bv;
            const float* __restrict__ cv = reinterpret_cast<const float*>(pc);
            mv.base = (MASK && gmask) ? reinterpret_cast<const char*>(gmask + (long long)pc->nbr_slot * H * MASK_PLANES * mrow) : nullptr;
            bool ok = epipolar_search<STATS, false, MASK>(nrec, W, H, cv, rcv, pc->clean, true, x, y, pixel, grad1, th_pi, xp0, xp1, prm, rho,
                                             sigma, bu, bv, &st, mv, &ms);
            if (ok && __float_as_uint(rho) < 0x7f800000u) {
                h = make_float2(rho, sigma);
                mymask |= 1ull << j;
            }
        }
#endif
        hyp[j * K1_PX + p] = make_float2(h.x, safe_rcp_sq(h.y));
        sgm[j * K1_PX + p] = h.y;
    }
    for (int q = w; q < cnt_words; q += K1_WAVES) cnt[q * K1_PX + p] = 0u;
    if (w == 0) {
        set0[p] = 0ull;
        cnt0[p] = 0u;
    }
    pmask[tid] = mymask;
    __syncthreads();

    unsigned long long vm = 0;
#pragma unroll
    for (int q = 0; q < K1_WAVES; q++) vm |= pmask[q * K1_PX + p];
#if SDM_ABLATE == 1
    const int nh = 0;
    if (vm == 0x123456789ull) pool[0] = make_float2(1.f, 1.f);
#else
    const int nh = __popcll(vm);
#endif
    const bool go = nh > prm.lambdaN;
    const int a0 = (int)__ffsll((long long)vm) - 1;
    bool self0 = false;
    if (go) {
        const float2 ha = hyp[a0 * K1_PX + p];
        const float sa = sgm[a0 * K1_PX + p];
        self0 = sa * sa > 0.0f;
        unsigned c = 0;
        for (int bb = w; bb < n; bb += K1_WAVES) {
            const float2 hb = hyp[bb * K1_PX + p];
            if (bb != a0 && chi_test_lazy(ha, hb, sa, &sgm[bb * K1_PX + p])) c++;
        }
        if (c) atomicAdd(&cnt0[p], c);
    }
    __syncthreads();
#if SDM_ABLATE == 9
    bool settled = false;
    const bool few = false;
    const unsigned long long S0 = 0ull;
    const int s0 = 0;
#else
    bool settled = go && self0 && (int)cnt0[p] + 1 == nh;
    const bool more = go && !settled && self0;
    unsigned long long S0 = settled ? vm : 0ull;
    if (__builtin_amdgcn_ballot_w64(more) != 0ull) {
        if (more) {
            const float2 ha = hyp[a0 * K1_PX + p];
            const float sa = sgm[a0 * K1_PX + p];
            unsigned long long m = 0;
            for (int bb = w; bb < n; bb += K1_WAVES) {
                const float2 hb = hyp[bb * K1_PX + p];
                if (bb != a0 && chi_test_lazy(ha, hb, sa, &sgm[bb * K1_PX + p])) m |= 1ull << bb;
            }
            if (m) atomicOr(&set0[p], m);
        }
        __syncthreads();
        if (more) S0 = set0[p] | (1ull << a0);
    }
    const int s0 = __popcll(S0);
    const unsigned long long O = vm & ~S0;
    const bool few = more && __popcll(O) <= K1_OUTLIER_ROWS;
    if (__builtin_amdgcn_ballot_w64(few) != 0ull) {
        unsigned* orow = cnt;
        unsigned long long rem = few ? O : 0ull;
        for (int i = 0; i < K1_OUTLIER_ROWS && __builtin_amdgcn_ballot_w64(rem != 0ull) != 0ull; i++) {
            if (rem != 0ull) {
                const int o = (int)__ffsll((long long)rem) - 1;
                rem &= rem - 1ull;
                const float2 ho = hyp[o * K1_PX + p];
                const float so = sgm[o * K1_PX + p];
                unsigned c = (w == 0 && so * so > 0.0f) ? 1u : 0u;
                for (int bb = w; bb < n; bb += K1_WAVES) {
                    const float2 hb = hyp[bb * K1_PX + p];
                    if (bb != o && chi_test_lazy(ho, hb, so, &sgm[bb * K1_PX + p])) c += ((S0 >> bb) & 1ull) ? 0x10001u : 1u;
                }
                if (c) atomicAdd(&orow[i * K1_PX + p], c);
            }
        }
        __syncthreads();
        if (few) {
            bool stands = true;
            const int nO = __popcll(O);
            for (int i = 0; i < K1_OUTLIER_ROWS; i++) {
                const unsigned v = orow[i * K1_PX + p];
                if (i < nO) stands = stands && (v >> 16) == 0u && (int)(v & 0xffffu) <= s0;
            }
            settled = stands;
        }
        __syncthreads();
        for (int q = w; q < K1_OUTLIER_ROWS; q += K1_WAVES) cnt[q * K1_PX + p] = 0u;
    }
#endif
    const bool open = go && !settled;
    const unsigned long long open_mask = __builtin_amdgcn_ballot_w64(open);
    bool deferred = false;
    if (open_mask != 0ull) {
        if (tid == 0) {
            const unsigned cntw = (unsigned)__popcll(open_mask);
            unsigned first = 0xFFFFFFFFu;
            if (cntw < open_list.inplace_min && atomicAdd(&open_list.count[0], cntw) >= open_list.quota) {
                const unsigned base = atomicAdd(&open_list.count[2], cntw);
                if (base <= open_list.capacity && cntw <= open_list.capacity - base)
                    first = base;
                else
                    atomicMin(&open_list.count[1], base);
            }
            xbase[0] = first;
        }
        __syncthreads();
        const unsigned base = xbase[0];
        deferred = base != 0xFFFFFFFFu;
        if (deferred) {
            if (open) {
                const unsigned e = base + (unsigned)__popcll(open_mask & ((1ull << p) - 1ull));
                float2* __restrict__ dst = open_list.hyp + ((size_t)(e >> 6) * n) * K1_PX + (e & 63u);
                for (int j = w; j < n; j += K1_WAVES) dst[(size_t)j * K1_PX] = make_float2(hyp[j * K1_PX + p].x, sgm[j * K1_PX + p]);
                if (w == 0) {
                    open_list.pix[e] = (long long)rc.slot * plane + y * W + x;
                    open_list.vm[e] = vm;
                }
            }
        } else {
            if (open) k1_count_all_pairs(hyp, sgm, cnt, vm, n, p, w);
            __syncthreads();
        }
    }

    unsigned long long n_fused = 0;
    if (w == 0 && on && !(open && deferred)) {
        float2 result = make_float2(0.f, 0.f);
        if (settled) {
            if (s0 >= prm.lambdaN) {
                float pjsj = 0.f, rsj = 0.f;
                for (int bb = 0; bb < n; bb++) {
                    if (!((S0 >> bb) & 1ull)) continue;
                    fusion_accum(hyp[bb * K1_PX + p].x, sgm[bb * K1_PX + p], pjsj, rsj);
                }
                result = make_float2(pjsj / rsj, sqrtf(1 / rsj));
                n_fused = 1;
            }
        } else if (go) {
            n_fused = k1_fuse_counted(hyp, sgm, cnt, vm, n, p, prm.lambdaN, result) ? 1 : 0;
        }
        pool[(long long)rc.slot * plane + y * W + x] = result;
    }
    if (STATS) {
        unsigned long long v[9] = {st.searches, st.candidates, st.gate_pass,
// ... 1392 lines not shown
```

Before: 13730.

## Add lean search-fuse kernel variant when all pairs are host-verified clean

Computes per-pair clean bits on the host (valid theta angles, safe line quotient) and, when every pair is clean and default gates apply, launches a specialized k_search_fuse instantiation that hardcodes the clean path, skips the plan/mask branches and relaxes the waves-per-EU minimum. An optional unroll-3 variant is chosen below a mean-range threshold, which defaults to zero so it is effectively off. Host-side theta_bad mirroring, host-wait counters and debugging APIs are added. The lean path trades the occupancy hint and extra kernel instantiations for less branching and register pressure, and relies on the host bits matching the device ones.

After: 13730, median of 2. About the same (+0.0%).

```diff
diff --git a/include/sdm_c.h b/include/sdm_c.h
--- a/include/sdm_c.h
+++ b/include/sdm_c.h
@@ -202,6 +202,14 @@
 int sdm_enable_stats(sdm_ctx *ctx, int on);
 int sdm_get_stats(sdm_ctx *ctx, sdm_stats *out, int reset);
 int sdm_set_scan_mode(sdm_ctx *ctx, int mode);
+#define SDM_K1_AUTO 0
+#define SDM_K1_GENERAL 1
+#define SDM_K1_LEAN 2
+#define SDM_K1_MASK 3
+int sdm_set_k1_variant(sdm_ctx *ctx, int variant);
+int sdm_get_k1_variant(sdm_ctx *ctx, int *last);
+int sdm_host_waits(sdm_ctx *ctx, long long *count, int reset);
+int sdm_pair_clean_bits(sdm_ctx *ctx, int capacity, int *host_bits, int *device_bits, int *n_pairs);
 int sdm_set_ingest_overlap(sdm_ctx *ctx, int on);
 #define SDM_STAGE_SEARCH_FUSE 0
 #define SDM_STAGE_INTRA 1
diff --git a/orb-slam-free-space-carving_amd/binding.py b/orb-slam-free-space-carving_amd/binding.py
--- a/orb-slam-free-space-carving_amd/binding.py
+++ b/orb-slam-free-space-carving_amd/binding.py
@@ -137,6 +137,10 @@
     ("sdm_enable_stats", C.c_int, [_ctx, C.c_int]),
     ("sdm_get_stats", C.c_int, [_ctx, C.POINTER(Stats), C.c_int]),
     ("sdm_set_scan_mode", C.c_int, [_ctx, C.c_int]),
+    ("sdm_set_k1_variant", C.c_int, [_ctx, C.c_int]),
+    ("sdm_get_k1_variant", C.c_int, [_ctx, C.POINTER(C.c_int)]),
+    ("sdm_host_waits", C.c_int, [_ctx, C.POINTER(C.c_longlong), C.c_int]),
+    ("sdm_pair_clean_bits", C.c_int, [_ctx, C.c_int, C.POINTER(C.c_int), C.POINTER(C.c_int), C.POINTER(C.c_int)]),
     ("sdm_get_params", C.c_int, [_ctx, C.POINTER(Params)]),
     ("sdm_set_ingest_overlap", C.c_int, [_ctx, C.c_int]),
     ("sdm_selftest", C.c_int, [_ctx, C.c_int, C.POINTER(C.c_ulonglong)]),
@@ -806,6 +810,30 @@
     def set_scan_mode(self, mode):
         self._check(self.lib.sdm_set_scan_mode(self.ctx, int(mode)))
 
+    K1_VARIANTS = ("none", "general", "lean", "mask")
+
+    def set_k1_variant(self, variant):
+        self._check(self.lib.sdm_set_k1_variant(self.ctx, int(variant)))
+
+    def k1_variant(self):
+        v = C.c_int(0)
+        self._check(self.lib.sdm_get_k1_variant(self.ctx, C.byref(v)))
+        return self.K1_VARIANTS[v.value]
+
+    def host_waits(self, reset=True):
+        v = C.c_longlong(0)
+        self._check(self.lib.sdm_host_waits(self.ctx, C.byref(v), 1 if reset else 0))
+        return int(v.value)
+
+    def pair_clean_bits(self):
+        n = C.c_int(0)
+        self._check(self.lib.sdm_pair_clean_bits(self.ctx, 0, None, None, C.byref(n)))
+        host = np.zeros(n.value, np.int32)
+        dev = np.zeros(n.value, np.int32)
+        ip = C.POINTER(C.c_int)
+        self._check(self.lib.sdm_pair_clean_bits(self.ctx, n.value, host.ctypes.data_as(ip), dev.ctypes.data_as(ip), C.byref(n)))
+        return host, dev
+
     def enable_stats(self, on=True):
         self._check(self.lib.sdm_enable_stats(self.ctx, 1 if on else 0))
 
diff --git a/orb-slam-free-space-carving_amd/csrc/sdm_device.h b/orb-slam-free-space-carving_amd/csrc/sdm_device.h
--- a/orb-slam-free-space-carving_amd/csrc/sdm_device.h
+++ b/orb-slam-free-space-carving_amd/csrc/sdm_device.h
@@ -453,11 +453,11 @@
 #endif
 }
 
-__device__ __forceinline__ bool line_quot_safe(const float* F)
+__host__ __device__ __forceinline__ bool line_quot_safe(const float* F)
 {
     bool ok = true;
     for (int i = 0; i < 9; i++) {
-        const unsigned u = __float_as_uint(F[i]), mag = u & 0x7FFFFFFFu;
+        const unsigned u = __builtin_bit_cast(unsigned, F[i]), mag = u & 0x7FFFFFFFu;
         ok = ok && (u == 0u || (mag >= ((127u - 36u) << 23) && mag <= ((127u + 20u) << 23)));
     }
     return ok;
@@ -582,12 +582,12 @@
     }
 }
 
-template <bool STATS, bool CLEAN>
+template <bool STATS, bool CLEAN, int NB = SCAN_UNROLL>
 __device__ __forceinline__ void scan_segment(const ScanConst& q, int lo, const DevParams& prm, ScanState& S, SearchStats* st)
 {
     float u0f = (float)lo;
-    for (int u0 = lo; u0 <= q.hi; u0 += SCAN_UNROLL, u0f += (float)SCAN_UNROLL)
-        scan_batch<STATS, CLEAN, SCAN_UNROLL>(q, u0, u0f, prm, S, st);
+    for (int u0 = lo; u0 <= q.hi; u0 += NB, u0f += (float)NB)
+        scan_batch<STATS, CLEAN, NB>(q, u0, u0f, prm, S, st);
 }
 
 #ifndef SDM_MASK_MIN_L
@@ -756,7 +756,7 @@
         if (u0 <= q.hi) scan_batch<STATS, CLEAN, 3>(q, u0, u0f, prm, S, st);
 }
 
-template <bool STATS, bool PLAN = false, bool MASK = false>
+template <bool STATS, bool PLAN = false, bool MASK = false, bool LEAN = false, int NB = SCAN_UNROLL>
 __device__ __forceinline__ bool epipolar_search(const float4* __restrict__ nrec, int W, int H,
                                                 const float* __restrict__ cv, const float* __restrict__ rcv, int clean,
                                                 bool on, int x, int y, float pixel, float grad1,
@@ -777,7 +777,7 @@
     float c = (float)x * F[2] + (float)y * F[5] + F[8];
 #if SDM_K1_OPT & 0x8000
     float ab, cb;
-    if (clean & 2) {
+    if (LEAN || (clean & 2)) {
         const float rb = rcp_fast(b);
         ab = quot_fast(a, b, rb);
         cb = quot_fast(c, b, rb);
@@ -837,7 +837,10 @@
     sc.ang_pi_rot = ang_pi_rot;
     sc.gate_lim = gate_lim;
     sc.hi = hi;
-    if (PLAN) {
+    if (LEAN) {
+        static_assert(!LEAN || (!STATS && !PLAN && !MASK), "the lean search has no statistics, no plan and no mask scan");
+        scan_segment<false, true, NB>(sc, lo, prm, S, st);
+    } else if (PLAN) {
         const int Lmax = wave_max_nonneg(max(hi - lo + 1, 0));
         if (Lmax > 0) {
 #if SDM_K1_OPT & 0x02
diff --git a/orb-slam-free-space-carving_amd/csrc/sdm_engine.hip b/orb-slam-free-space-carving_amd/csrc/sdm_engine.hip
--- a/orb-slam-free-space-carving_amd/csrc/sdm_engine.hip
+++ b/orb-slam-free-space-carving_amd/csrc/sdm_engine.hip
@@ -82,6 +82,8 @@
     unsigned grow_launch = 0;
     unsigned k4_lds_pad = 0;
     int* h_act_count = nullptr;
+    int* h_theta_bad = nullptr;
+    std::vector<char> theta_known;
     std::vector<float> act_lambdaG;
     std::vector<char> chk_sparse, xyz_sparse;
     std::vector<float> recon_lambdaG;
@@ -116,6 +118,11 @@
     unsigned* d_gmask = nullptr;
     int mrow = 0;
     int scan_mode = 0;
+    int k1_variant = 0;
+    int k1_last = 0;
+    int k1_last_unroll = 0;
+    float k1_unroll3_below = K1_UNROLL3_BELOW;
+    long long host_waits = 0;
     bool ingest_overlap = false;
     static constexpr int CNT_RING = 16;
     hipEvent_t cnt_ev[CNT_RING] = {};
@@ -133,6 +140,9 @@
     struct TableKey {
         bool valid = false, has_consts = false;
         bool long_ranges = false;
+        bool all_clean = false;
+        float mean_range = 0.0f;
+        std::vector<unsigned char> clean_host;
         int n_ref = 0, n = 0;
         unsigned long long epoch = 0;
         std::vector<int> refs, nbrs;
@@ -368,7 +378,7 @@
     const hipStream_t ks = c->stream;
     hipLaunchKernelGGL(k_prepass_finish, dim3(n_kf), dim3(FIN_BLOCK), 0, ks, c->d_gitems, c->W, c->H, c->geom.ntiles, c->nseg,
                        c->d_part, c->d_seg_mask, c->d_seg_off, c->d_meta, c->d_act_count, c->h_act_count, c->d_theta_bad,
-                       c->d_act_hash, from_images ? 1 : 0);
+                       c->h_theta_bad, c->d_act_hash, from_images ? 1 : 0);
     const int waves = (c->nseg + LIST_SEGS - 1) / LIST_SEGS;
     hipLaunchKernelGGL(k_list_write, dim3((waves + BLOCK / 64 - 1) / (BLOCK / 64), n_kf), dim3(BLOCK), 0, ks, c->d_gitems,
                        c->geom.tiles_x, c->nseg, c->P, c->d_seg_mask, c->d_seg_off, c->d_act);
@@ -416,6 +426,7 @@
 {
     if (c->cnt_done + 1 < c->cnt_next) {
         HIP_TRY(hipEventSynchronize(c->cnt_ev[(c->cnt_next - 1) % sdm_ctx::CNT_RING]));
+        c->host_waits++;
         c->cnt_done = c->cnt_next - 1;
     }
     return SDM_OK;
@@ -428,6 +439,7 @@
     if (g > c->cnt_done) {
         if (c->cnt_next - g >= (unsigned long long)sdm_ctx::CNT_RING) g = c->cnt_next - 1;
         HIP_TRY(hipEventSynchronize(c->cnt_ev[g % sdm_ctx::CNT_RING]));
+        c->host_waits++;
         c->cnt_done = g;
     }
     return SDM_OK;
@@ -446,6 +458,7 @@
     sdm_ctx::TableSet& s = c->sets[c->cur_set];
     if (s.pending) {
         HIP_TRY(hipEventSynchronize(s.free_ev));
+        c->host_waits++;
         s.pending = false;
     }
     return SDM_OK;
@@ -628,13 +641,28 @@
     k.mind.assign(h_mind, h_mind + n_ref);
     k.maxd.assign(h_maxd, h_maxd + n_ref);
     k.long_ranges = false;
+    k.all_clean = false;
+    k.mean_range = 0.0f;
+    k.clean_host.clear();
     if (k.has_consts) {
         double sum = 0.0;
+        bool all_clean = np > 0;
+        k.clean_host.resize(np);
         for (size_t i = 0; i < np; i++) {
-            const KfMeta& m1 = c->h_meta[ref_slots[i / (size_t)n]];
-            const KfMeta& m2 = c->h_meta[nbr_slots[i]];
+            const int s1 = ref_slots[i / (size_t)n], s2 = nbr_slots[i];
+            const KfMeta& m1 = c->h_meta[s1];
+            const KfMeta& m2 = c->h_meta[s2];
             float F[9], R21[9], t21[3];
             pair_geometry(m1, m2, F, R21, t21);
+            {
+                const bool known = c->theta_known[s1] && c->theta_known[s2];
+                const bool angles_ok = known && c->h_theta_bad[s1] == 0 && c->h_theta_bad[s2] == 0;
+                const float pr = h_rot[i];
+                const unsigned char bits = (unsigned char)(((angles_ok && pr >= -360.0f && pr <= 360.0f) ? 1 : 0) |
+                                                           (line_quot_safe(F) ? 2 : 0) | (known ? 0 : 0x80));
+                k.clean_host[i] = bits;
+                all_clean = all_clean && bits == 3;
+            }
             const float d0 = h_mind[i / (size_t)n], d1 = h_maxd[i / (size_t)n];
             float u0 = m1.fx * (R21[2] * d0 + t21[0]) / (R21[8] * d0 + t21[2]) + m1.cx;
             float u1 = m1.fx * (R21[2] * d1 + t21[0]) / (R21[8] * d1 + t21[2]) + m1.cx;
@@ -645,6 +673,8 @@
             sum += (len == len) ? (double)len : (double)cols;
         }
         k.long_ranges = np > 0 && sum / (double)np >= (double)MASK_CALL_MEAN_L;
+        k.mean_range = np > 0 ? (float)(sum / (double)np) : 0.0f;
+        k.all_clean = all_clean;
     }
     HIP_TRY(hipEventRecord(c->sets[victim].free_ev, c->stream));
     c->sets[victim].pending = true;
@@ -669,6 +699,7 @@
 void reset_slot_state(sdm_ctx* c, int slot)
 {
     c->epoch++;
+    c->theta_known[slot] = 0;
     c->has_depth[slot] = 0;
     c->has_chk[slot] = 0;
     c->recon_lambdaG[slot] = std::nanf("");
@@ -810,6 +841,7 @@
     c->chk_sparse.assign(K, 1);
     c->xyz_sparse.assign(K, 1);
     c->slot_cnt.assign(K, 0);
+    c->theta_known.assign(K, 0);
 
     int rc = SDM_OK;
     auto bail = [&](int code) {
@@ -888,6 +920,8 @@
         c->mrow = 2 * (c->geom.tiles_x + 1);
         if ((rc = dev_alloc(&c->d_gmask, (size_t)K * c->H * MASK_PLANES * c->mrow))) return bail(rc);
         if (const char* e = getenv("SDM_SCAN_MODE")) c->scan_mode = std::max(0, std::min(2, atoi(e)));
+        if (const char* e = getenv("SDM_K1_VARIANT")) c->k1_variant = std::max(0, std::min(2, atoi(e)));
+        if (const char* e = getenv("SDM_K1_UNROLL3_BELOW")) c->k1_unroll3_below = (float)atof(e);
         set_dev_params(c);
     }
     if ((rc = dev_alloc(&c->d_im, (size_t)c->P))) return bail(rc);
@@ -908,6 +942,8 @@
     if ((rc = host_alloc(&c->h_f2, (size_t)c->P))) return bail(rc);
     if ((rc = host_alloc(&c->h_act_count, (size_t)K))) return bail(rc);
     memset(c->h_act_count, 0, sizeof(int) * (size_t)K);
+    if ((rc = host_alloc(&c->h_theta_bad, (size_t)K))) return bail(rc);
+    memset(c->h_theta_bad, 0, sizeof(int) * (size_t)K);
 
     if (hipMemsetAsync(c->rec, 0, sizeof(float4) * c->P * K, c->stream) != hipSuccess ||
         hipMemsetAsync(c->pool, 0, sizeof(float2) * c->P * K, c->stream) != hipSuccess ||
@@ -926,7 +962,9 @@
     if (hipFuncSetAttribute((const void*)k_search_fuse<false, false>, hipFuncAttributeMaxDynamicSharedMemorySize, max_lds) != hipSuccess ||
         hipFuncSetAttribute((const void*)k_search_fuse<true, false>, hipFuncAttributeMaxDynamicSharedMemorySize, max_lds) != hipSuccess ||
         hipFuncSetAttribute((const void*)k_search_fuse<false, true>, hipFuncAttributeMaxDynamicSharedMemorySize, max_lds) != hipSuccess ||
-        hipFuncSetAttribute((const void*)k_search_fuse<true, true>, hipFuncAttributeMaxDynamicSharedMemorySize, max_lds) != hipSuccess)
+        hipFuncSetAttribute((const void*)k_search_fuse<true, true>, hipFuncAttributeMaxDynamicSharedMemorySize, max_lds) != hipSuccess ||
+        hipFuncSetAttribute((const void*)k_search_fuse<false, false, true>, hipFuncAttributeMaxDynamicSharedMemorySize, max_lds) != hipSuccess ||
+        hipFuncSetAttribute((const void*)k_search_fuse<false, false, true, 3>, hipFuncAttributeMaxDynamicSharedMemorySize, max_lds) != hipSuccess)
         return bail(fail(SDM_EHIP, "hipFuncSetAttribute(max dynamic LDS) failed"));
     *out = c;
     return SDM_OK;
@@ -991,6 +1029,7 @@
     }
     (void)hipHostFree(c->h_f2);
     (void)hipHostFree(c->h_act_count);
+    (void)hipHostFree(c->h_theta_bad);
     (void)hipFree(c->d_ext);
     (void)hipFree(c->d_ext_stage);
     (void)hipFree(c->d_vox);
@@ -1298,6 +1337,7 @@
         for (int i = 0; i < m; i++) {
             const int slot = slots[i0 + i];
             reset_slot_state(c, slot);
+            c->theta_known[slot] = 1;
             c->h_meta[slot] = B.h_items[i].meta;
             c->act_lambdaG[slot] = c->dprm.lambdaG;
             c->recon_lambdaG[slot] = c->dprm.lambdaG;
@@ -1457,6 +1497,14 @@
 }
 
 static bool all_pipeline_maps(sdm_ctx* c, int n_ref, const int* ref_slots);
+
+static bool lean_eligible(const sdm_ctx* c, bool mask)
+{
+    if (c->k1_variant == SDM_K1_GENERAL || mask || c->stats_on || c->scan_mode == 2) return false;
+    if (!(c->dprm.default_gates && c->dprm.fast_theta_div && c->dprm.closed_ok)) return false;
+    const sdm_ctx::TableKey& k = c->sets[c->cur_set].key;
+    return k.valid && k.has_consts && k.all_clean;
+}
 
 static int launch_search_fuse(sdm_ctx* c, int n_ref, int n, const int* ref_slots)
 {
@@ -1486,8 +1534,14 @@
     const size_t lds_open = (sizeof(float2) + sizeof(float)) * (size_t)K1_PX * n + sizeof(unsigned) * (size_t)K1_PX * ((n + 3) / 4);
     const int grid_open = (int)std::min<unsigned>(c->open_capacity / K1_PX, c->open_grid);
     const bool mask = c->scan_mode == 2 || (c->scan_mode == 0 && c->sets[c->cur_set].key.long_ranges);
+    const bool lean = lean_eligible(c, mask);
+    const bool unroll3 = lean && c->sets[c->cur_set].key.mean_range < c->k1_unroll3_below;
     auto k1 = c->stats_on ? (mask ? k_search_fuse<true, true> : k_search_fuse<true, false>)
-                          : (mask ? k_search_fuse<false, true> : k_search_fuse<false, false>);
+                          : (mask ? k_search_fuse<false, true>
+                                  : (lean ? (unroll3 ? k_search_fuse<false, false, true, 3> : k_search_fuse<false, false, true>)
+                                          : k_search_fuse<false, false>));
+    c->k1_last = lean ? SDM_K1_LEAN : (mask ? SDM_K1_MASK : SDM_K1_GENERAL);
+    c->k1_last_unroll = unroll3 ? 3 : SCAN_UNROLL;
     for_ref_slices(n_ref, blocks_per_ref, K1_BLOCK, [&](int first, int count) {
         hipLaunchKernelGGL(k1, dim3(blocks_per_ref * count), dim3(K1_BLOCK), lds, c->stream, c->rec, c->P, c->d_refs + first,
                            c->d_pairs + (size_t)first * n, count, n, c->W, c->H, max_chunks, c->dprm, c->d_act, c->pool, c->d_stats,
@@ -2924,6 +2978,50 @@
     return SDM_OK;
 }
 
+int sdm_set_k1_variant(sdm_ctx* c, int variant)
+{
+    if (!c) return fail(SDM_EINVAL, "null context");
+    if (variant < 0 || variant > 2) return fail(SDM_EINVAL, "K1 variant must be 0, 1 or 2");
+    c->k1_variant = variant;
+    return SDM_OK;
+}
+
+int sdm_get_k1_variant(sdm_ctx* c, int* last)
+{
+    if (!c || !last) return fail(SDM_EINVAL, "null argument");
+    *last = c->k1_last;
+    return SDM_OK;
+}
+
+int sdm_host_waits(sdm_ctx* c, long long* count, int reset)
+{
+    if (!c || !count) return fail(SDM_EINVAL, "null argument");
+    *count = c->host_waits;
+    if (reset) c->host_waits = 0;
+    return SDM_OK;
+}
+
+int sdm_pair_clean_bits(sdm_ctx* c, int capacity, int* host_bits, int* device_bits, int* n_pairs)
+{
+    if (!c || !n_pairs) return fail(SDM_EINVAL, "null argument");
+    const sdm_ctx::TableKey& k = c->sets[c->cur_set].key;
+    if (!k.valid || !k.has_consts) return fail(SDM_ESTATE, "the last staged call had no search constants");
+    const size_t np = (size_t)k.n_ref * (size_t)k.n;
+    *n_pairs = (int)np;
+    if (!host_bits && !device_bits) return SDM_OK;
+    if ((size_t)capacity < np) return fail(SDM_EINVAL, "buffer too small");
+    HIP_TRY(hipSetDevice(c->cfg.device));
+    if (host_bits)
+        for (size_t i = 0; i < np; i++) host_bits[i] = (int)k.clean_host[i];
+    if (device_bits) {
+        std::vector<PairConst> pcs(np);
+        HIP_TRY(hipStreamSynchronize(c->stream));
+        HIP_TRY(hipMemcpy(pcs.data(), c->d_pairs, sizeof(PairConst) * np, hipMemcpyDeviceToHost));
+        for (size_t i = 0; i < np; i++) device_bits[i] = pcs[i].clean;
+    }
+    return SDM_OK;
+}
+
 int sdm_get_stats(sdm_ctx* c, sdm_stats* out, int reset)
 {
     if (!c || !out) return fail(SDM_EINVAL, "null argument");
diff --git a/orb-slam-free-space-carving_amd/csrc/sdm_ingest.h b/orb-slam-free-space-carving_amd/csrc/sdm_ingest.h
--- a/orb-slam-free-space-carving_amd/csrc/sdm_ingest.h
+++ b/orb-slam-free-space-carving_amd/csrc/sdm_ingest.h
@@ -307,7 +307,7 @@
                                                               const unsigned long long* __restrict__ seg_mask,
                                                               int* __restrict__ seg_off, KfMeta* __restrict__ meta,
                                                               int* __restrict__ act_count, int* __restrict__ host_count,
-                                                              int* __restrict__ theta_bad,
+                                                              int* __restrict__ theta_bad, int* __restrict__ host_theta_bad,
                                                               unsigned long long* __restrict__ act_hash, int full)
 {
     __shared__ unsigned long long red[PART_WORDS][FIN_BLOCK / 64];
@@ -368,6 +368,7 @@
             }
             meta[it.slot] = m;
             theta_bad[it.slot] = tot[3] ? 1 : 0;
+            host_theta_bad[it.slot] = tot[3] ? 1 : 0;
         }
     }
 }
diff --git a/orb-slam-free-space-carving_amd/csrc/sdm_kernels.h b/orb-slam-free-space-carving_amd/csrc/sdm_kernels.h
--- a/orb-slam-free-space-carving_amd/csrc/sdm_kernels.h
+++ b/orb-slam-free-space-carving_amd/csrc/sdm_kernels.h
@@ -286,10 +286,20 @@
 #ifndef SDM_K1_EU_MIN
 #define SDM_K1_EU_MIN 8
 #endif
+#ifndef SDM_K1_LEAN_EU_MIN
+#define SDM_K1_LEAN_EU_MIN 1
+#endif
+#ifndef SDM_K1_UNROLL3_BELOW
+#define SDM_K1_UNROLL3_BELOW 0.0f
+#endif
+constexpr float K1_UNROLL3_BELOW = SDM_K1_UNROLL3_BELOW;
+#ifndef SDM_K1_LEAN_OPT
+#define SDM_K1_LEAN_OPT 0
+#endif
 #ifndef SDM_K1_LB
-#define SDM_K1_LB __launch_bounds__(K1_BLOCK) __attribute__((amdgpu_waves_per_eu(SDM_K1_EU_MIN, 8)))
-#endif
-template <bool STATS, bool MASK>
+#define SDM_K1_LB __launch_bounds__(K1_BLOCK) __attribute__((amdgpu_waves_per_eu(LEAN ? SDM_K1_LEAN_EU_MIN : SDM_K1_EU_MIN, 8)))
+#endif
+template <bool STATS, bool MASK, bool LEAN = false, int UNROLL = SCAN_UNROLL>
 __global__ SDM_K1_LB void k_search_fuse(const float4* __restrict__ rec, long long plane,
                                                        const RefConst* __restrict__ refs,
                                                        const PairConst* __restrict__ pairs, int n_ref, int n,
@@ -340,7 +350,13 @@
     MaskView mv;
     mv.row_pitch = (unsigned)mrow * MASK_WORD_BYTES;
     const PairConst* __restrict__ pcs = pairs + (long long)ref * n;
-    const float rcvb[4] = {rc.fx, rc.cx, rc.mind, rc.maxd};
+    float rfx = rc.fx, rcx = rc.cx, rmind = rc.mind, rmaxd = rc.maxd;
+#if SDM_K1_LEAN_OPT & 1
+    if (LEAN) {
+        asm volatile("" : "+v"(rfx), "+v"(rcx), "+v"(rmind), "+v"(rmaxd));
+    }
+#endif
+    const float rcvb[4] = {rfx, rcx, rmind, rmaxd};
     const float* __restrict__ rcv = rcvb;
     unsigned long long mymask = 0;
     for (int j = w; j < n; j += K1_WAVES) {
@@ -363,8 +379,8 @@
             float rho, sigma, bu, bv;
             const float* __restrict__ cv = reinterpret_cast<const float*>(pc);
             mv.base = (MASK && gmask) ? reinterpret_cast<const char*>(gmask + (long long)pc->nbr_slot * H * MASK_PLANES * mrow) : nullptr;
-            bool ok = epipolar_search<STATS, false, MASK>(nrec, W, H, cv, rcv, pc->clean, true, x, y, pixel, grad1, th_pi, xp0, xp1, prm, rho,
-                                             sigma, bu, bv, &st, mv, &ms);
+            bool ok = epipolar_search<STATS, false, MASK, LEAN, UNROLL>(nrec, W, H, cv, rcv, LEAN ? 3 : pc->clean, true, x, y, pixel, grad1,
+                                                                        th_pi, xp0, xp1, prm, rho, sigma, bu, bv, &st, mv, &ms);
             if (ok && __float_as_uint(rho) < 0x7f800000u) {
                 h = make_float2(rho, sigma);
                 mymask |= 1ull << j;
```
